# cgmb/euler

Hardware: AMD Instinct MI355X
Metric: cells*steps/sec of sim_step() (frames incl. the PCG pressure projection) + pressure-solve HBM GB/s vs roofline (higher is better)
Workload: dtype f64

## Files before the change

euler_amd/__init__.py:

```python
import ctypes as C
import os

import numpy as np

_HERE = os.path.dirname(os.path.abspath(__file__))
LIB_PATH = os.path.join(_HERE, "lib", "libeuler_hip.so")

DOT_AUTO, DOT_SEQUENTIAL, DOT_TREE = 0, 1, 2
PRECOND_IC0, PRECOND_JACOBI, PRECOND_IC0_TILE, PRECOND_IC0_TILE2, PRECOND_IC0_TILE_MG = 0, 1, 2, 3, 4
(OPT_P_STEPS, OPT_TILE_STORE_AS, OPT_TILE_REVERSE, OPT_RESIDENT_CAP, OPT_GRID4_MIN_CELLS, OPT_SLAB_FUSION, OPT_RCCL_SMALL, OPT_RCCL_NO_EXCHANGE, OPT_MARKERS_ROWMAJOR,
 OPT_SA_RUN, OPT_NO_INTERIOR, OPT_BUILD_GATHER, OPT_RESIDENT_FORCE_TIMEOUT, OPT_MG_SPLIT_LEVEL, OPT_MG_SPLIT_ACTIVE, OPT_MARKERS_TWO_PASS, OPT_BUILD_TWO_PASS,
 OPT_VELOCITY_TWO_PASS, OPT_NO_TILE_MAP, OPT_PROFILE_STRIDE) = range(1, 21)
SWEEP_AUTO, SWEEP_BAND, SWEEP_SIMPLE = 0, 1, 2
PCG_F64, PCG_F32 = 0, 1
RESIDENT_AUTO, RESIDENT_OFF = 0, 1
(F_U, F_V, F_UTMP, F_VTMP, F_SOLID, F_SOURCE, F_SINK, F_COUNT, F_PREV_COUNT, F_MARKERS, F_PRECON,
 F_PRESSURE, F_PCG_B, F_PCG_R, F_PCG_Z, F_PCG_S, F_PCG_Q, F_CELLMASK,
 F_DYE_R, F_DYE_G, F_DYE_B, F_DYE_RTMP, F_DYE_GTMP, F_DYE_BTMP, F_MARKER_KEYS) = range(25)
(STAGE_ADVECT_MARKERS, STAGE_REFRESH_COUNTS, STAGE_SOURCES, STAGE_EXTRAPOLATE, STAGE_ADVECT_VELOCITY,
 STAGE_PROJECT) = range(6)
(OP_BUILD_SYSTEM, OP_PRECON_FACTOR, OP_FORWARD_SOLVE, OP_BACKWARD_SOLVE, OP_APPLY_A, OP_DOT_ZR, OP_DOT_ZS,
 OP_INF_NORM_R, OP_UPDATE_PR, OP_UPDATE_SEARCH) = range(10)

_FIELD_DTYPE = {
    F_U: np.float32, F_V: np.float32, F_UTMP: np.float32, F_VTMP: np.float32,
    F_SOLID: np.uint8, F_SOURCE: np.uint8, F_SINK: np.uint8, F_COUNT: np.uint8, F_PREV_COUNT: np.uint8,
    F_MARKERS: np.float32, F_PRECON: np.float64, F_PRESSURE: np.float64, F_PCG_B: np.float64,
    F_PCG_R: np.float64, F_PCG_Z: np.float64, F_PCG_S: np.float64, F_PCG_Q: np.float64, F_CELLMASK: np.uint8,
    F_DYE_R: np.float32, F_DYE_G: np.float32, F_DYE_B: np.float32,
    F_DYE_RTMP: np.float32, F_DYE_GTMP: np.float32, F_DYE_BTMP: np.float32, F_MARKER_KEYS: np.uint32,
}


class EulerError(RuntimeError):
    def __init__(self, code, msg):
        super().__init__("libeuler_hip error %d: %s" % (code, msg))
        self.code = code


class Config(C.Structure):
    _fields_ = [
        ("abi_version", C.c_int32), ("X", C.c_int32), ("Y", C.c_int32), ("device", C.c_int32),
        ("max_iterations", C.c_int32), ("tol", C.c_double), ("dot_mode", C.c_int32), ("precond", C.c_int32),
        ("sweep_mode", C.c_int32), ("max_substeps", C.c_int32), ("frame_time", C.c_float),
        ("viscosity", C.c_float), ("pcg_poll_interval", C.c_int32), ("rainbow", C.c_int32),
        ("precond_tile_records", C.c_int32), ("slab_rank", C.c_int32), ("slab_nranks", C.c_int32),
        ("slab_band_lo", C.c_int32), ("slab_band_hi", C.c_int32), ("pcg_precision", C.c_int32), ("resident", C.c_int32),
    ]


class Stats(C.Structure):
    _fields_ = [
        ("frames", C.c_uint64), ("total_substeps", C.c_uint64), ("total_pcg_iterations", C.c_uint64),
        ("last_substeps", C.c_int32), ("last_pcg_iterations", C.c_int32), ("last_residual", C.c_double),
        ("last_dt", C.c_float), ("n_markers", C.c_uint64), ("source_exhausted", C.c_int32),
        ("rng_state", C.c_uint64), ("marker_dt_events", C.c_uint64), ("marker_multi_events", C.c_uint64),
        ("fluid_cells", C.c_uint64),
    ]


_lib = None

EXPORTS = [
    "euler_config_default", "euler_create", "euler_destroy", "euler_last_error", "euler_abi_version",
    "euler_load_scenario_mem", "euler_load_scenario_file", "euler_load_half_tank", "euler_load_half_tanks", "euler_parse_scenario",
    "euler_seed_markers", "euler_step", "euler_timestep", "euler_substep", "euler_stage", "euler_pcg_op", "euler_set_precond", "euler_set_solver",
    "euler_get_field", "euler_set_field", "euler_set_markers", "euler_set_rng", "euler_get_stats",
    "euler_field_bytes", "euler_render", "euler_render_grids", "euler_render_grids_rgb", "euler_colorize", "euler_profile_enable",
    "euler_profile_class_count", "euler_profile_class_name", "euler_profile_get", "euler_profile_reset",
    "euler_measure_copy_bandwidth", "euler_measure_exchange", "euler_device_name", "euler_hbm_bytes", "euler_sweep_timeline", "euler_save_state", "euler_load_state", "euler_set_comm", "euler_set_stream", "euler_slab_info",
    "euler_rccl_unique_id", "euler_rccl_version", "euler_set_comm_rccl", "euler_comm_calls",
    "euler_p2p_export", "euler_p2p_connect", "euler_p2p_disconnect", "euler_p2p_calls", "euler_resident_info",
    "euler_set_option", "euler_get_option",
]


def load_library():
    global _lib
    if _lib is not None:
        return _lib
    path = os.environ.get("EULER_HIP_LIB", LIB_PATH)
    if not os.path.exists(path):
        raise ImportError(
            "euler_amd: %s is missing. Build it with `python -c 'import __graft_entry__ as g; g.build()'` "
            "or `make -C euler_amd/csrc`. There is no CPU fallback." % LIB_PATH)
    L = C.CDLL(path)
    vp, i32, u64, f32, f64 = C.c_void_p, C.c_int32, C.c_uint64, C.c_float, C.c_double
    sig = {
        "euler_config_default": (C.c_int, [C.POINTER(Config)]),
        "euler_create": (C.c_int, [C.POINTER(Config), C.POINTER(vp)]),
        "euler_destroy": (None, [vp]),
        "euler_last_error": (C.c_char_p, []),
        "euler_abi_version": (C.c_int, []),
        "euler_load_scenario_mem": (C.c_int, [vp, C.c_char_p, i32, i32]),
        "euler_load_scenario_file": (C.c_int, [vp, C.c_char_p, i32]),
        "euler_load_half_tank": (C.c_int, [vp]),
        "euler_load_half_tanks": (C.c_int, [vp, i32]),
        "euler_parse_scenario": (C.c_int, [C.c_char_p, i32, i32, i32, i32, vp, vp, vp, vp]),
        "euler_seed_markers": (C.c_int, [vp, i32, i32, C.POINTER(u64), vp, C.POINTER(u64)]),
        "euler_step": (C.c_int, [vp]),
        "euler_timestep": (C.c_int, [vp, f32, C.POINTER(f32)]),
        "euler_substep": (C.c_int, [vp, f32]),
        "euler_stage": (C.c_int, [vp, i32, f32]),
        "euler_pcg_op": (C.c_int, [vp, i32, f32, f64, C.POINTER(f64)]),
        "euler_set_precond": (C.c_int, [vp, i32, i32]),
        "euler_set_solver": (C.c_int, [vp, i32, f64]),
        "euler_get_field": (C.c_int, [vp, i32, vp, C.c_size_t]),
        "euler_set_field": (C.c_int, [vp, i32, vp, C.c_size_t]),
        "euler_set_markers": (C.c_int, [vp, vp, u64]),
        "euler_set_rng": (C.c_int, [vp, u64, i32]),
        "euler_get_stats": (C.c_int, [vp, C.POINTER(Stats)]),
        "euler_field_bytes": (C.c_size_t, [vp, i32]),
        "euler_render": (C.c_int, [vp, i32, i32, C.c_char_p, i32, C.POINTER(i32)]),
        "euler_render_grids": (C.c_int, [vp, vp, vp, i32, i32, i32, i32, C.c_char_p, i32, C.POINTER(i32)]),
        "euler_render_grids_rgb": (C.c_int, [vp, vp, vp, vp, vp, vp, i32, i32, i32, i32, C.c_char_p, i32, C.POINTER(i32)]),
        "euler_colorize": (C.c_int, [vp]),
        "euler_profile_enable": (C.c_int, [vp, u64]),
        "euler_profile_class_count": (C.c_int, []),
        "euler_profile_class_name": (C.c_char_p, [i32]),
        "euler_profile_get": (C.c_int, [vp, i32, C.POINTER(f64), C.POINTER(u64)]),
        "euler_profile_reset": (C.c_int, [vp]),
        "euler_resident_info": (C.c_int, [vp, C.POINTER(u64)]),
        "euler_measure_copy_bandwidth": (C.c_int, [vp, C.c_size_t, i32, C.POINTER(f64)]),
        "euler_measure_exchange": (C.c_int, [vp, i32, i32, i32, C.POINTER(f64)]),
        "euler_device_name": (C.c_int, [vp, C.c_char_p, i32]),
        "euler_hbm_bytes": (u64, [vp]),
        "euler_sweep_timeline": (C.c_int, [vp, C.POINTER(C.c_uint64), i32]),
        "euler_save_state": (C.c_int, [vp, C.c_char_p]),
        "euler_load_state": (C.c_int, [vp, C.c_char_p]),
        "euler_set_comm": (C.c_int, [vp, vp, i32]),
        "euler_set_stream": (C.c_int, [vp, vp]),
        "euler_slab_info": (C.c_int, [vp, C.POINTER(i32), C.POINTER(i32), C.POINTER(i32)]),
        "euler_rccl_unique_id": (C.c_int, [vp, i32]),
        "euler_rccl_version": (C.c_int, []),
        "euler_set_comm_rccl": (C.c_int, [vp, vp, i32, i32, i32, i32]),
        "euler_comm_calls": (C.c_int, [vp, C.POINTER(u64)]),
        "euler_p2p_export": (C.c_int, [vp, vp, i32]),
        "euler_p2p_connect": (C.c_int, [vp, vp, i32]),
        "euler_p2p_disconnect": (C.c_int, [vp]),
        "euler_p2p_calls": (C.c_int, [vp, C.POINTER(u64)]),
        "euler_set_option": (C.c_int, [vp, i32, C.c_int64]),
        "euler_get_option": (C.c_int, [vp, i32, C.POINTER(C.c_int64)]),
    }
    for name, (res, args) in sig.items():
        fn = getattr(L, name)
        fn.restype = res
        fn.argtypes = args
    _lib = L
    return L


def _check(rc):
    if rc != 0:
        raise EulerError(rc, load_library().euler_last_error().decode(errors="replace"))


def parse_scenario(text, X, Y, upscale=False):
    if isinstance(text, str):
        text = text.encode()
    out = [np.zeros((Y, X), np.uint8) for _ in range(4)]
    _check(load_library().euler_parse_scenario(text, len(text), X, Y, int(upscale), *[a.ctypes.data for a in out]))
    return tuple(out)


def seed_markers(fluid, rng_state=0x9bd185c449534b91):
# ... 284 lines not shown
```

euler_amd/csrc/driver.hip:

```cpp
#include "euler_dev.h"
#include "k_mg.h"

#include <math.h>
#include <stdarg.h>
#include <stdlib.h>
#include <string.h>

#include <vector>

int eu_launch_build_system(euler_sim* S, float dt);
int eu_launch_velocity_update(euler_sim* S, float dt, int finish);
int eu_pressure_current(euler_sim* S);
int eu_unskew(euler_sim* S, const void* skew, void* rowmajor, int elem_bytes);
int eu_unskew_fluid(euler_sim* S, const double* skew, double* rowmajor);
double* eu_current_search_direction(euler_sim* S);
int eu_launch_tile_table(euler_sim* S);
int eu_skew(euler_sim* S, const void* rowmajor, void* skew, int elem_bytes);

static thread_local char g_err[512] = "";

void eu_set_error(const char* fmt, ...) {
  va_list ap;
  va_start(ap, fmt);
  vsnprintf(g_err, sizeof(g_err), fmt, ap);
// ... 69 lines not shown
  if (ms) *ms = S->prof_ms[cls];
  if (launches) *launches = S->prof_launches[cls];
  return rc;
}
extern "C" int euler_profile_reset(euler_sim* S) {
  if (!S) return EULER_EINVAL;
  int rc = eu_prof_flush(S);
  memset(S->prof_ms, 0, sizeof(S->prof_ms));
  memset(S->prof_launches, 0, sizeof(S->prof_launches));
  memset(S->prof_idle, 0, sizeof(S->prof_idle));
  return rc;
}

extern "C" int euler_config_default(euler_config* c) {
  if (!c) return EULER_EINVAL;
  memset(c, 0, sizeof(*c));
  c->abi_version = EULER_ABI_VERSION;
  c->X = 100; c->Y = 40;
  c->device = 0;
  c->max_iterations = 100;
  c->tol = (double)1e-6f;
  c->dot_mode = EULER_DOT_AUTO;
  c->precond = EULER_PRECOND_IC0;
  c->sweep_mode = EULER_SWEEP_AUTO;
  c->max_substeps = 8;
  c->frame_time = 0.1f;
  c->viscosity = 0.f;
  c->pcg_poll_interval = 8;
  return EULER_OK;
}

static int eu_set_tiles(euler_sim* S, int w) {
  if (w <= 0) w = 16;
  if (w != 8 && w != 16 && w != 32) { eu_set_error("precond_tile_records = %d: 8, 16 or 32 (0 = 16)", w); return EULER_EINVAL; }
  S->cfg.precond_tile_records = w;
  S->tile_w = w;
  return EULER_OK;
}

bool eu_resident_eligible(const euler_sim* S) {
  if (S->res_disabled || S->cfg.resident == EULER_RESIDENT_OFF) return false;
  if (S->cfg.precond != EULER_PRECOND_IC0_TILE || S->tile_w != 16 || S->cfg.sweep_mode == EULER_SWEEP_SIMPLE || S->cfg.dot_mode != EULER_DOT_TREE) return false;
  if (S->has_comm || S->slab_on || S->p2p_on) return false;
  const int cap = eu_resident_capacity(const_cast<euler_sim*>(S), S->cfg.pcg_precision == EULER_PCG_F32);
  if (S->cfg.pcg_precision == EULER_PCG_F32) return cap > 0 && S->geom.nbands * (S->geom.T / 16) <= 4 * cap;
  return cap > 0;
}
extern "C" int euler_resident_info(euler_sim* S, uint64_t out[3]) {
  if (!S || !out) return EULER_EINVAL;
  out[0] = eu_resident_eligible(S) ? 1 : 0; out[1] = S->res_solves; out[2] = S->res_fallbacks;
  return EULER_OK;
}

extern "C" int euler_set_option(euler_sim* S, int32_t key, int64_t value) {
  if (!S || key <= 0 || key >= EULER_OPT__COUNT) { eu_set_error("euler_set_option: unknown key %d", (int)key); return EULER_EINVAL; }
  bool ok = true;
  const char* when = nullptr;
  switch (key) {
    case EULER_OPT_P_STEPS: ok = value == 2 || value == 4 || value == 8; break;
    case EULER_OPT_SA_RUN: ok = value == 8 || value == 16 || value == 32;
      if (ok && value != 8 && (S->has_comm || eu_is_two_level(S))) when = "on a handle without a communicator, in the parity or the plain tile-local mode (the others run runs of 8)";
      break;
    case EULER_OPT_RCCL_SMALL: ok = value >= 0 && value <= 2; if (S->rccl) when = "before euler_set_comm_rccl"; break;
    case EULER_OPT_RCCL_NO_EXCHANGE: ok = value == 0 || value == 1; if (S->rccl) when = "before euler_set_comm_rccl"; break;
    case EULER_OPT_SLAB_FUSION: ok = value == 0 || value == 1; if (S->p2p_on) when = "before euler_p2p_connect"; break;
    case EULER_OPT_RESIDENT_CAP: case EULER_OPT_GRID4_MIN_CELLS: case EULER_OPT_RESIDENT_FORCE_TIMEOUT: ok = value >= 0; break;
    case EULER_OPT_MG_SPLIT_LEVEL: ok = value >= -1 && value < 12; break;
    case EULER_OPT_PROFILE_STRIDE: ok = value >= 1 && value <= 1024; break;
    case EULER_OPT_MG_SPLIT_ACTIVE: ok = false; break;
    default: ok = value == 0 || value == 1; break;
  }
  if (!ok) { eu_set_error("euler_set_option: key %d does not take the value %lld", (int)key, (long long)value); return EULER_EINVAL; }
  if (when) { eu_set_error("euler_set_option: key %d must be set %s", (int)key, when); return EULER_ESTATE; }
  HIPCHK(hipStreamSynchronize(S->stream));
  if (key == EULER_OPT_P_STEPS || key == EULER_OPT_SA_RUN) {
    int rcp = eu_pressure_current(S);
    if (rcp) return rcp;
  }
  S->opt[key] = value;
  if (key == EULER_OPT_P_STEPS || key == EULER_OPT_SA_RUN) S->s_ring_n = 0;
  if (key == EULER_OPT_MG_SPLIT_LEVEL) { eu_mg_split_release(S); S->opt[EULER_OPT_MG_SPLIT_ACTIVE] = 0; }
  return EULER_OK;
}
extern "C" int euler_get_option(euler_sim* S, int32_t key, int64_t* value) {
  if (!S || !value || key <= 0 || key >= EULER_OPT__COUNT) { eu_set_error("euler_get_option: unknown key %d", (int)key); return EULER_EINVAL; }
  *value = S->opt[key];
  return EULER_OK;
}

static const char* eu_precond_combination(const euler_sim* S, int precond, int tile_w, int has_comm, int slab_on, int p2p_on) {
  const bool coarse = precond == EULER_PRECOND_IC0_TILE2 || precond == EULER_PRECOND_IC0_TILE_MG;
  if (!coarse) return nullptr;
  if (tile_w != 16 || S->cfg.sweep_mode == EULER_SWEEP_SIMPLE) return "the coarse-correction preconditioners run on tiles of 16 records with the band schedule";
  if (precond == EULER_PRECOND_IC0_TILE2 && (has_comm || slab_on)) return "EULER_PRECOND_IC0_TILE2 runs on one GPU (row slabs: EULER_PRECOND_IC0_TILE_MG)";
  if (precond == EULER_PRECOND_IC0_TILE_MG && has_comm && (!slab_on || p2p_on)) return "EULER_PRECOND_IC0_TILE_MG with several ranks: row-slab handles without mailboxes only";
  return nullptr;
}

extern "C" int euler_set_precond(euler_sim* S, int32_t precond, int32_t tile_records) {
  if (!S || precond < EULER_PRECOND_IC0 || precond > EULER_PRECOND_IC0_TILE_MG) { eu_set_error("euler_set_precond: bad argument"); return EULER_EINVAL; }
  const int w = tile_records <= 0 ? 16 : tile_records;
  if (w != 8 && w != 16 && w != 32) { eu_set_error("precond_tile_records = %d: 8, 16 or 32 (0 = 16)", tile_records); return EULER_EINVAL; }
  if (const char* why = eu_precond_combination(S, precond, w, S->has_comm, S->slab_on, S->p2p_on)) { eu_set_error("euler_set_precond: %s", why); return EULER_EINVAL; }
  if (S->cfg.pcg_precision == EULER_PCG_F32 && (precond != EULER_PRECOND_IC0_TILE || w != 16)) { eu_set_error("euler_set_precond: an EULER_PCG_F32 handle runs EULER_PRECOND_IC0_TILE with tiles of 16 records only"); return EULER_EINVAL; }
  HIPCHK(hipStreamSynchronize(S->stream));
  const bool coarse = precond == EULER_PRECOND_IC0_TILE2 || precond == EULER_PRECOND_IC0_TILE_MG;
  if (coarse) { int rc = eu_coarse_alloc(S, precond == EULER_PRECOND_IC0_TILE_MG); if (rc) return rc; }
  (void)eu_set_tiles(S, w);
  S->cfg.dot_mode = coarse ? EULER_DOT_TREE : S->dot_mode_user;
  if (S->has_comm && S->cfg.dot_mode == EULER_DOT_SEQUENTIAL) S->cfg.dot_mode = EULER_DOT_TREE;
  S->cfg.precond = precond;
  S->lean_ok = 0;
  return EULER_OK;
}

extern "C" int euler_set_solver(euler_sim* S, int32_t max_iterations, double tol) {
  if (!S) return EULER_EINVAL;
  HIPCHK(hipStreamSynchronize(S->stream));
  if (max_iterations > 0) S->cfg.max_iterations = max_iterations;
  if (tol >= 0.0) S->cfg.tol = tol;
  return EULER_OK;
}

static thread_local size_t g_alloc_bytes = 0;
template <typename T>
static int dalloc(T** p, size_t n) {
  HIPCHK(hipMalloc((void**)p, n * sizeof(T)));
  g_alloc_bytes += n * sizeof(T);
  HIPCHK(hipMemset(*p, 0, n * sizeof(T)));
  return EULER_OK;
}
#define DALLOC(p, n) do { int _rc = dalloc(&(p), (n)); if (_rc) { euler_destroy(S); return _rc; } } while (0)

extern "C" void euler_destroy(euler_sim* S) {
  if (!S) return;
  if (S->stream) (void)hipStreamSynchronize(S->stream);
  eu_p2p_release(S);
  eu_rccl_release(S);
  eu_slab_release(S);
  eu_coarse_release(S);
  const size_t wo = S->shifted ? S->win_off : 0;
  for (float* f : {S->u, S->v, S->utmp, S->vtmp}) if (f) (void)hipFree(f + wo);
  for (uint8_t* g : {S->solid, S->source, S->sink, S->count, S->prev_count}) if (g) (void)hipFree(g + wo);
  if (S->count32) (void)hipFree(S->count32);
  if (S->blockedT) (void)hipFree(S->blockedT);
  if (S->tmap) (void)hipFree(S->tmap);
  if (S->uT) (void)hipFree(S->uT);
  if (S->vT) (void)hipFree(S->vT);
  if (S->countT) (void)hipFree(S->countT);
  if (S->solidT) (void)hipFree(S->solidT);
  if (S->sys_m) (void)hipFree(S->sys_m);
  if (S->sys_div) (void)hipFree(S->sys_div);
  void* dev[] = {S->markers[0], S->markers[1], S->keys[0], S->keys[1], S->ms, S->evmask, S->delmask, S->ev_theta, S->ev_delta, S->sel_idx, S->act_idx,
                 S->act_dt, S->cellmask64, S->draws, S->sel.block_sums, S->sc, S->partial, S->red_counter, S->granules, S->ticket, S->sweep_timeline, S->halo_buf, S->band_ranges, S->partial2, S->pair_buf, S->xrows, S->alpha_buf, S->rng_jump, S->chunk_flag, S->chunk_prev, S->chunk_part, S->tile_table, S->chunk_bits, S->chunk_list,
                 S->rowmajor_tmp};
  for (void* p : dev) if (p) (void)hipFree(p);
  for (float* d : S->dye) if (d) (void)hipFree(d + wo);
  const size_t so = S->shifted ? S->skew_off : 0, sl = S->shifted ? (size_t)EU_SKEW_SLACK : 0;
  (void)so; (void)sl;
  for (void* d : S->s_ring_alloc) if (d) (void)hipFree(d);
  for (void* d : S->skew_alloc) if (d) (void)hipFree(d);
  const size_t fb_off = S->shifted ? (size_t)S->ab_lo * S->fb_stride * 64 : 0;
  if (S->fbits_fwd) (void)hipFree(S->fbits_fwd + fb_off);
  if (S->fbits_bwd) (void)hipFree(S->fbits_bwd + fb_off);
  if (S->ms_host) (void)hipHostFree(S->ms_host);
  if (S->sc_host) (void)hipHostFree(S->sc_host);
  if (S->poll_host) (void)hipHostFree(S->poll_host);
  if (S->res_err) (void)hipHostFree(S->res_err);
  if (S->res_gran) (void)hipFree(S->res_gran);
  for (hipEvent_t e : S->poll_event) if (e) (void)hipEventDestroy(e);
  if (S->ev_pool) { for (int k = 0; k < S->ev_cap; ++k) if (S->ev_pool[k]) (void)hipEventDestroy(S->ev_pool[k]); free(S->ev_pool); }
  free(S->ev_cls); free(S->ev_solve); free(S->ev_iter);
  if (S->stream && S->own_stream) (void)hipStreamDestroy(S->stream);
  free(S);
}

extern "C" int euler_create(const euler_config* cfg, euler_sim** out) {
  if (!cfg || !out) { eu_set_error("euler_create: null argument"); return EULER_EINVAL; }
  if (cfg->abi_version != EULER_ABI_VERSION) { eu_set_error("euler_create: ABI version %d != %d", cfg->abi_version, EULER_ABI_VERSION); return EULER_EINVAL; }
  if (cfg->X < 8 || cfg->Y < 8 || (size_t)cfg->X * cfg->Y > (size_t)1 << 30) { eu_set_error("euler_create: grid %dx%d out of range", cfg->X, cfg->Y); return EULER_EINVAL; }
  int ndev = 0;
  hipError_t e = hipGetDeviceCount(&ndev);
  if (e != hipSuccess || ndev == 0) {
    eu_set_error("euler_create: no HIP device (%s); libeuler_hip has no CPU path", e == hipSuccess ? "device count 0" : hipGetErrorString(e));
    return EULER_EHIP;
  }
  if (cfg->device < 0 || cfg->device >= ndev) { eu_set_error("euler_create: device %d of %d", cfg->device, ndev); return EULER_EINVAL; }
  HIPCHK(hipSetDevice(cfg->device));
  hipDeviceProp_t prop;
  HIPCHK(hipGetDeviceProperties(&prop, cfg->device));
  if (strncmp(prop.gcnArchName, "gfx950", 6) != 0) {
    eu_set_error("euler_create: device is %s; this library carries gfx950 code only", prop.gcnArchName);
    return EULER_EHIP;
  }

  euler_sim* S = (euler_sim*)calloc(1, sizeof(euler_sim));
  if (S) { S->opt[EULER_OPT_P_STEPS] = 8; S->opt[EULER_OPT_TILE_REVERSE] = 1; S->opt[EULER_OPT_GRID4_MIN_CELLS] = 1ll << 22; S->opt[EULER_OPT_SA_RUN] = 8; S->opt[EULER_OPT_PROFILE_STRIDE] = 1; }
  if (!S) return EULER_ENOMEM;
  g_alloc_bytes = 0;
  S->cfg = *cfg;
  if (S->cfg.max_iterations <= 0) S->cfg.max_iterations = 100;
  if (S->cfg.max_substeps <= 0) S->cfg.max_substeps = 8;
  if (S->cfg.frame_time <= 0.f) S->cfg.frame_time = 0.1f;
  S->X = cfg->X; S->Y = cfg->Y;
  const size_t C = S->C = (size_t)cfg->X * cfg->Y;
  if (S->cfg.dot_mode == EULER_DOT_AUTO) S->cfg.dot_mode = C <= 65536 ? EULER_DOT_SEQUENTIAL : EULER_DOT_TREE;
  S->dot_mode_user = S->cfg.dot_mode;
  if (S->cfg.sweep_mode == EULER_SWEEP_AUTO) S->cfg.sweep_mode = EULER_SWEEP_BAND;
  S->geom.X = S->X; S->geom.Y = S->Y;
  S->geom.nbands = (S->Y + 63) / 64;
  S->geom.T = (S->X + 63 + 95) / 96 * 96;
  S->geom.TS = (S->geom.T + 31) / 32 * 32 + 64;
  S->geom.S = (size_t)S->geom.nbands * S->geom.TS * 64;
  const int nbands = S->geom.nbands;
  S->slab_on = cfg->slab_nranks >= 1;
  if (S->slab_on) {
    if (cfg->slab_rank < 0 || cfg->slab_rank >= cfg->slab_nranks || cfg->slab_nranks > nbands) {
      eu_set_error("euler_create: slab rank %d of %d for %d bands of 64 rows", cfg->slab_rank, cfg->slab_nranks, nbands);
      free(S); return EULER_EINVAL;
    }
    if (S->cfg.sweep_mode == EULER_SWEEP_SIMPLE) {
      eu_set_error("euler_create: row slabs do not run EULER_SWEEP_SIMPLE");
      free(S); return EULER_EINVAL;
    }
    S->band_lo = (int)((int64_t)nbands * cfg->slab_rank / cfg->slab_nranks);
    S->band_hi = (int)((int64_t)nbands * (cfg->slab_rank + 1) / cfg->slab_nranks);
    if (cfg->slab_band_hi > cfg->slab_band_lo || cfg->slab_band_lo != 0) {
      const int lo = cfg->slab_band_lo, hi = cfg->slab_band_hi;
      const bool first = cfg->slab_rank == 0, last = cfg->slab_rank + 1 == cfg->slab_nranks;
      if (lo < 0 || hi <= lo || hi > nbands || (first && lo != 0) || (last && hi != nbands) || (!first && lo < cfg->slab_rank) ||
          (!last && nbands - hi < cfg->slab_nranks - 1 - cfg->slab_rank)) {
        eu_set_error("euler_create: slab rank %d of %d cannot own bands [%d, %d) of %d (every rank needs a band; the ranges tile the grid in rank order)",
                     cfg->slab_rank, cfg->slab_nranks, lo, hi, nbands);
        free(S); return EULER_EINVAL;
      }
      S->band_lo = lo; S->band_hi = hi;
    }
    if (S->cfg.dot_mode == EULER_DOT_SEQUENTIAL) S->cfg.dot_mode = EULER_DOT_TREE;
  } else { S->band_lo = 0; S->band_hi = nbands; }
  S->row_lo = 64 * S->band_lo; S->row_hi = 64 * S->band_hi < S->Y ? 64 * S->band_hi : S->Y;
  S->win_lo = S->row_lo - EU_GHOST_LO > 0 ? S->row_lo - EU_GHOST_LO : 0;
  S->win_hi = S->row_hi + EU_GHOST_HI < S->Y ? S->row_hi + EU_GHOST_HI : S->Y;
  S->win_off = (size_t)S->win_lo * S->X;
  S->Cw = (size_t)(S->win_hi - S->win_lo) * S->X;
  S->ab_lo = S->band_lo > 0 ? S->band_lo - 1 : 0; S->ab_hi = S->band_hi < nbands ? S->band_hi + 1 : nbands;
  S->skew_off = (size_t)S->ab_lo * S->geom.TS * 64;
  S->Sw = (size_t)(S->ab_hi - S->ab_lo) * S->geom.TS * 64;
  S->e_lo = (size_t)S->band_lo * S->geom.TS * 64; S->e_cnt = (size_t)(S->band_hi - S->band_lo) * S->geom.TS * 64;
  const size_t SS = S->Sw;
  const size_t Cw = S->Cw;
  if (C > ((size_t)1 << 29) || Cw > ((size_t)1 << 28) || (SS + EU_SKEW_SLACK) * 8 >= ((size_t)1 << 32)) {
    eu_set_error("grid %d x %d is larger than the supported maximum (2^28 cells per GPU, 2^29 in all)", cfg->X, cfg->Y);
    free(S);
    return EULER_EINVAL;
  }
#define CREATECHK(call) do { hipError_t _e = (call); if (_e != hipSuccess) { int _rc = eu_hip_fail(_e, #call, __FILE__, __LINE__); euler_destroy(S); return _rc; } } while (0)
  CREATECHK(hipStreamCreateWithFlags(&S->stream, hipStreamNonBlocking));
  S->own_stream = 1;

  DALLOC(S->u, Cw); DALLOC(S->v, Cw); DALLOC(S->utmp, Cw); DALLOC(S->vtmp, Cw);
  DALLOC(S->solid, Cw); DALLOC(S->source, Cw); DALLOC(S->sink, Cw); DALLOC(S->count, Cw); DALLOC(S->prev_count, Cw);
  DALLOC(S->count32, Cw);
  if (!S->slab_on) { DALLOC(S->blockedT, Cw); DALLOC(S->uT, Cw); DALLOC(S->vT, Cw); DALLOC(S->countT, Cw); DALLOC(S->solidT, Cw); }
  eu_state_replaced(S);
  DALLOC(S->sys_m, Cw); DALLOC(S->sys_div, Cw);
  if (S->cfg.rainbow) for (float*& d : S->dye) DALLOC(d, Cw);
  S->max_markers = 4 * C;
  if (S->slab_on) { const size_t cap = 6 * (size_t)(S->row_hi - S->row_lo) * S->X + 65536; if (cap < S->max_markers) S->max_markers = cap; }
  DALLOC(S->markers[0], S->max_markers); DALLOC(S->markers[1], S->max_markers);
  if (S->slab_on) { DALLOC(S->keys[0], S->max_markers); DALLOC(S->keys[1], S->max_markers); }
  DALLOC(S->ms, 1);
  const size_t mwords = (S->max_markers + 63) / 64;
  DALLOC(S->evmask, mwords);
  if (!S->slab_on) DALLOC(S->delmask, mwords);
  if (!S->slab_on) {
    S->tmap_nx = (S->X + 63) / 64 + 1; S->tmap_n = S->tmap_nx * ((S->Y + 63) / 64 + 2);
    DALLOC(S->tmap, 3 * (size_t)S->tmap_n);
  }
  DALLOC(S->ev_theta, S->max_markers); DALLOC(S->ev_delta, S->max_markers);
  S->sel_cap = S->max_markers;
  DALLOC(S->sel_idx, S->sel_cap);
  DALLOC(S->act_idx, S->max_markers); DALLOC(S->act_dt, S->max_markers);
  DALLOC(S->cellmask64, (Cw + 63) / 64 + 1);
  S->sel.capacity_blocks = (mwords + 2047) / 2048 + 1;
  DALLOC(S->sel.block_sums, S->sel.capacity_blocks);
  {
    const size_t stagger = (size_t)EU_ARRAY_STAGGER / 8 * 8;
    int k = 0;
    for (double** d : {&S->b, &S->p, &S->r, &S->z, &S->s, &S->s2, &S->q, &S->precon}) {
      DALLOC(*d, SS + EU_SKEW_SLACK + 8 * stagger / 8);
      S->skew_alloc[k] = *d;
      *d += (size_t)k * stagger / 8;
      ++k;
    }
    DALLOC(S->cellmask, SS + EU_SKEW_SLACK);
    S->skew_alloc[8] = S->cellmask;
  }
  S->fb_stride = 12 * (((S->geom.T + 7) / 8 + 11) / 12) + 4;
  DALLOC(S->fbits_fwd, (size_t)(S->ab_hi - S->ab_lo) * S->fb_stride * 64);
  DALLOC(S->fbits_bwd, (size_t)(S->ab_hi - S->ab_lo) * S->fb_stride * 64);
  DALLOC(S->sc, 1);
  DALLOC(S->band_ranges, (size_t)S->geom.nbands);
  { int rc = eu_set_tiles(S, S->cfg.precond_tile_records); if (rc) { euler_destroy(S); return rc; } }
  S->red_blocks = (int)eu_blocks(S->e_cnt, EU_RED_ELEMS, 2048);
  DALLOC(S->partial, (size_t)S->red_blocks > 2048 ? (size_t)S->red_blocks : 2048);
  DALLOC(S->partial2, 2048);
  DALLOC(S->pair_buf, 2 * 64);
// ... 704 lines not shown
```

euler_amd/csrc/euler_dev.h:

```cpp
#pragma once

#include <hip/hip_runtime.h>
#include <stdint.h>
#include <stdio.h>

#include "euler.h"
#include "euler_host.h"

#define EU_H 1.0f
#define EU_RHO 1.0f
#define EU_G (-10.0f)

#define CM_FLUID 0x01
#define CM_RIGHT 0x02
#define CM_UP    0x04
#define CM_LEFT  0x08
#define CM_DOWN  0x10
#define CM_DIAG_SHIFT 5
#define CM_INTERIOR 0x9F
#define EU_CHUNK_INTERIOR 0x80000000u

enum {
  KC_TIMESTEP = 0, KC_MARKER_ADVECT, KC_MARKER_EVENTS, KC_MARKER_BIN, KC_MARKER_COMPACT, KC_SOURCES,
  KC_SELECT, KC_EXTRAPOLATE, KC_ADVECT_VELOCITY, KC_BUILD_SYSTEM, KC_PRECON_FACTOR,
  KC_FORWARD_SOLVE, KC_BACKWARD_SOLVE, KC_APPLY_A, KC_DOT, KC_UPDATE_PR, KC_UPDATE_SEARCH,
  KC_REDUCE_FINAL, KC_VELOCITY_UPDATE, KC_JACOBI, KC_MISC, KC_PRECOND_TILE, KC_COARSE_CYCLE, KC_RESIDENT, KC__COUNT
};

struct PcgScalars {
  double sigma, zs, sigma_new, alpha, beta, rnorm;
  double tol;
  double comm_val;
  double comm_val2;
  double* comm_slot;
  double alpha_prev;
  double alpha_hist[8];
  int nonzero;
  int done;
  int iters;
  int max_iters;
  unsigned int n_chunks, pad_;
  void** p2p_boxes;
  int* p2p_error;
  int p2p_rank, p2p_n;
  unsigned int p2p_seq, p2p_halo_seq;
};

struct MarkerState {
  unsigned long long n;
  unsigned long long max_markers;
  unsigned long long rng_state;
  int exhausted;
  unsigned int n_events;
  unsigned int n_actual;
  unsigned int n_deleted;
  unsigned int n_append;
  unsigned long long n0_append;
  unsigned long long total_dt_events, multi_events;
  float dt_final;
  float dt;
  unsigned int max_u2_bits, max_v2_bits;
  unsigned int dt_ticket;
  int error;
  unsigned long long n_loc;
  unsigned int n_rm;
  unsigned int n_del_glob;
  unsigned int n_recv;
  unsigned int src_k_lo;
  unsigned long long rng0;
};

#define EU_SKEW_SLACK (64 * 64)
#ifndef EU_ARRAY_STAGGER
#define EU_ARRAY_STAGGER 0
#endif
#ifndef EU_RED_ELEMS
#define EU_RED_ELEMS (256 * 16)
#endif
struct SkewGeom {
  int X, Y, nbands, T, TS;
  size_t S;
};
static inline __host__ __device__ size_t skew_index(const SkewGeom& g, int x, int y) {
  const int l = y & 63, t = x + l;
  return ((size_t)(y >> 6) * g.TS + (size_t)(t & ~1)) * 64 + 2 * l + (t & 1);
}
static inline __host__ __device__ void skew_decode(const SkewGeom& g, size_t e, int& band, int& t, int& l) {
  const size_t per_band = (size_t)g.TS * 64;
  band = (int)(e / per_band);
  const size_t r = e % per_band;
  l = (int)((r & 127) >> 1);
  t = (int)((r >> 7) << 1) + (int)(r & 1);
}

struct SelectScratch {
  unsigned int* block_sums;
  unsigned int* total;
  size_t capacity_blocks;
};

struct euler_sim {
  euler_config cfg;
  int X, Y;
  size_t C;
  hipStream_t stream;
  int loaded;
  long long opt[32];
  int dot_mode_user;

  float *u, *v, *utmp, *vtmp;
  uint8_t *solid, *source, *sink, *count, *prev_count;
  unsigned int* count32;
  int p_pending;
  int maxsq_state;
  int uv_clean;
  int uv_zb;
  int count32_dirty;
  int prebin_valid;
  unsigned long long* delmask;
  uint8_t* tmap;
  int tmap_nx, tmap_n;
  int tmap_valid;
  int utmp_clean;
  int countT_clean;
  uint8_t* blockedT;
  int blocked_dirty;
  float *uT, *vT; uint8_t *countT, *solidT;
  int solidT_dirty;
  float* dye[6];
  float2* markers[2];
  int cur;
  size_t max_markers;
  unsigned long long n_markers_host;
  size_t n_source_cells;
  MarkerState* ms;
  MarkerState* ms_host;
  unsigned long long* evmask;
  float* ev_theta;
  float* ev_delta;
  unsigned int* sel_idx;
  size_t sel_cap;
  unsigned int* act_idx; float* act_dt;
  unsigned long long* cellmask64;
  float* draws;
  SelectScratch sel;

  SkewGeom geom;
  double *b, *p, *r, *z, *s, *q, *precon;
  double* s2;
  void* skew_alloc[9];
  uint8_t* cellmask;
  uint8_t* sys_m; float* sys_div;
  unsigned int* fbits_fwd; unsigned int* fbits_bwd;
  int fb_stride;
  int4* band_ranges;
  int coarse_m, coarse_shift, coarse_nx, coarse_ny, coarse_n;
  int *cc_diag, *cc_right, *cc_up;
  int* cc_pinned;
  double* cc_sten;
  int cc_n;
  double* cc_fac;
  double* cc_inv;
  double* cc_part;
  double* cc_y;
  double* cc_null;
  int mg_levels, mg_nx[12], mg_ny[12];
  size_t mg_off[12], mg_cells;
  double* mg_a;
  unsigned long long* mg_a0i;
  double *mg_rhs, *mg_x;
  double* mg_wd;
  uint8_t* mg_inner0; double mg_ic[9];
  double* mg_part;
  double* mg_dot;
  double* mg_null0;
  double* mg_m0;
  void* mg_split;
  double* mg_xbuf; int mg_xslot;
  unsigned long long* res_gran;
  unsigned long long res_tag;
  int* res_err;
  int res_disabled;
  unsigned int res_last_chunks;
  int res_have_last, res_skip_once;
  unsigned long long res_solves, res_fallbacks;
  int pcg_fields_resident;
  int tile_w;
  double* s_ring[8];
  void* s_ring_alloc[8];
  double* s_base[2];
  int s_ring_n;
  int s_launched;
  int s_none;
  int s_stale;
  const double* tile_as_override;
  double* partial2;
  struct RngJump* rng_jump;
  uint8_t* chunk_flag;
  uint8_t* chunk_prev;
  uint8_t* chunk_part;
  size_t hbm_bytes;
  int lean_ok;
  double* tile_table;
  unsigned long long* chunk_bits;
  unsigned int* chunk_list;
  size_t chunk_words, chunk_cap;
  double* xrows;
  size_t xrow_len;
  int gs_cur;
  double* alpha_buf;
  double* pair_buf;
  double* rowmajor_tmp;
  PcgScalars* sc;
  PcgScalars* sc_host;
  PcgScalars* poll_host;
  hipEvent_t poll_event[2];
  double* partial;
  unsigned int* red_counter;
  int red_blocks;
  unsigned long long* granules;
  int gran_stride;
  unsigned int* ticket;
  unsigned int ticket_base;
  unsigned int epoch;
  unsigned long long* sweep_timeline;

  float interp_lim[4];

  euler_stats stats;

  euler_comm_ops comm;
  int has_comm, couple;
  int band_lo, band_hi;
  size_t e_lo, e_cnt;
  double* halo_buf;
  int own_stream;
  int slab_on, shifted;
  int row_lo, row_hi, win_lo, win_hi;
  size_t win_off, Cw, skew_off, Sw;
  int ab_lo, ab_hi;
  unsigned int* keys[2];
  euler_comm_ops bulk;
  struct SlabScratch* slab;
  int part_lo[64], part_hi[64];
  void* rccl;
  void* p2p;
  int p2p_on;

  uint64_t prof_mask;
  uint64_t prof_open;
  unsigned int prof_seq[32];
  double prof_ms[KC__COUNT];
  uint64_t prof_launches[KC__COUNT];
  uint64_t prof_idle[KC__COUNT];
  hipEvent_t* ev_pool; int* ev_cls; int* ev_solve; int* ev_iter; int ev_used, ev_cap;
  int solve_seq;
  int prof_iter;
  int solve_iters[256];
};

void eu_set_error(const char* fmt, ...);
int eu_hip_fail(hipError_t e, const char* what, const char* file, int line);
#define HIPCHK(call) do { hipError_t _e = (call); if (_e != hipSuccess) return eu_hip_fail(_e, #call, __FILE__, __LINE__); } while (0)

void eu_prof_begin(euler_sim* S, int cls);
void eu_prof_end(euler_sim* S, int cls);
int  eu_prof_flush(euler_sim* S);

#define LAUNCH(S, CLS, KERNEL, GRID, BLOCK, ...)                                   \
  do {                                                                             \
    eu_prof_begin((S), (CLS));                                                     \
    hipLaunchKernelGGL(KERNEL, GRID, BLOCK, 0, (S)->stream, __VA_ARGS__);          \
    eu_prof_end((S), (CLS));                                                       \
  } while (0)

static inline unsigned eu_blocks(size_t n, unsigned per_block, unsigned cap = 0x7fffffffu) {
  size_t b = (n + per_block - 1) / per_block;
  if (b < 1) b = 1;
  if (b > cap) b = cap;
  return (unsigned)b;
}

__device__ __forceinline__ size_t eu_xcd_block() {
  const unsigned int b = blockIdx.x, full = gridDim.x & ~7u;
  return b < full ? (size_t)(b & 7) * (full >> 3) + (b >> 3) : (size_t)b;
}

#define EU_GHOST_LO 1
#define EU_GHOST_HI 2
int  eu_slab_alloc(euler_sim* S);
size_t eu_slab_bytes(const euler_sim* S);
void eu_slab_release(euler_sim* S);
int  eu_slab_substep(euler_sim* S, float dt);
int  eu_slab_stage(euler_sim* S, int stage, float dt);
int  eu_slab_timestep(euler_sim* S, float frame_time_left);
int  eu_slab_after_load(euler_sim* S);
int  eu_slab_check_partition(euler_sim* S);
int  eu_slab_exchange_uv(euler_sim* S);
int  eu_slab_exchange_dye(euler_sim* S);
int  eu_slab_render(euler_sim* S, int wx, int wy, char* out, int cap, int* len);
int  eu_slab_after_restore(euler_sim* S);
int  eu_slab_error_sync(euler_sim* S);
int  eu_slab_same_everywhere(euler_sim* S, const double* vals, int n, int* same);
int  eu_slab_status_sync(euler_sim* S, int local_rc, int* worst);
static inline void eu_state_replaced(euler_sim* S) {
  S->blocked_dirty = 1; S->solidT_dirty = 1;
  S->prebin_valid = 0;
  if (S->maxsq_state == 2) S->maxsq_state = 1;
  S->p_pending = 0;
  S->uv_clean = 0; S->uv_zb = 0;
  S->tmap_valid = 0; S->utmp_clean = 0; S->countT_clean = 0;
}
static inline bool eu_tile_map_on(const euler_sim* S) { return S->tmap && S->tmap_valid && !S->slab_on && S->opt[EULER_OPT_NO_TILE_MAP] == 0; }
int eu_launch_timestep(euler_sim* S, float frame_time_left);
int eu_launch_advect_markers(euler_sim* S, float dt);
int eu_launch_refresh_counts(euler_sim* S);
int eu_launch_sources(euler_sim* S);
int eu_launch_extrapolate(euler_sim* S);
int eu_launch_advect_velocity(euler_sim* S, float dt);
int eu_launch_diffuse(euler_sim* S, float dt);
int eu_launch_project(euler_sim* S, float dt);
int eu_resident_capacity(euler_sim* S, int f32);
int eu_launch_resident(euler_sim* S, unsigned int n_chunks);
bool eu_resident_eligible(const euler_sim* S);
int eu_launch_colorize(euler_sim* S);
int eu_launch_dye_extrapolate(euler_sim* S);
int eu_launch_dye_sources(euler_sim* S);
int eu_launch_dye_advect(euler_sim* S, float dt);
int eu_launch_pcg_op(euler_sim* S, int op, float dt, double a, double* out);
int eu_ordered_select(euler_sim* S, const unsigned long long* mask, size_t nwords, unsigned int* out_idx,
                      unsigned int* out_total);
int eu_sync_marker_state(euler_sim* S);
void eu_rccl_release(euler_sim* S);
void eu_p2p_release(euler_sim* S);
int eu_p2p_halo_skewed(euler_sim* S, double* s_skewed);
void eu_p2p_xgran(euler_sim* S, int backward, const unsigned long long** in, unsigned long long** out);
int  eu_p2p_has_neighbour_arrays(const euler_sim* S);
void eu_p2p_neighbour_arrays(euler_sim* S, const double** z_dn, const double** s_dn, const double** z_up, const double** s_up);
int eu_install_comm(euler_sim* S, const euler_comm_ops* ops, int32_t coupling, int allow_single);
static inline bool eu_is_tile(const euler_sim* S) { return S->cfg.precond == EULER_PRECOND_IC0_TILE || S->cfg.precond == EULER_PRECOND_IC0_TILE2 || S->cfg.precond == EULER_PRECOND_IC0_TILE_MG; }
static inline bool eu_is_two_level(const euler_sim* S) { return S->cfg.precond == EULER_PRECOND_IC0_TILE2 || S->cfg.precond == EULER_PRECOND_IC0_TILE_MG; }
static inline bool eu_is_mg(const euler_sim* S) { return S->cfg.precond == EULER_PRECOND_IC0_TILE_MG; }
int  eu_coarse_alloc(euler_sim* S, bool mg);
void eu_coarse_release(euler_sim* S);
int  eu_launch_coarse_setup(euler_sim* S);
int  eu_launch_coarse_consistent(euler_sim* S);
int  eu_launch_coarse_solve(euler_sim* S, int fin_op, int force);
int  eu_launch_coarse_search_init(euler_sim* S);
int  eu_coarse_comm_slots(euler_sim* S);
int  eu_launch_coarse_pre(euler_sim* S, int force);
int  eu_launch_coarse_scatter(euler_sim* S);
int  eu_launch_coarse_add_row(euler_sim* S, double* row, int yrow);

#ifdef __HIPCC__

// ... 186 lines not shown
```

euler_amd/csrc/k_pcg.hip:

```cpp
#include "euler_dev.h"
#include "k_mg.h"

#include <stdlib.h>
#include <cmath>
#include <type_traits>
#include <vector>

#define RED_THREADS 1024
typedef double sw_d2 __attribute__((ext_vector_type(2)));

__device__ __forceinline__ bool pcg_idle(const PcgScalars* sc) { return sc->done || !sc->nonzero; }

#define DPP_WAVE_SHL1 0x130
#define DPP_WAVE_SHR1 0x138

template <int CTRL>
__device__ __forceinline__ double wave_shift_inject(double v, double edge) {
  const int lo = __builtin_amdgcn_update_dpp(__double2loint(edge), __double2loint(v), CTRL, 0xf, 0xf, false);
  const int hi = __builtin_amdgcn_update_dpp(__double2hiint(edge), __double2hiint(v), CTRL, 0xf, 0xf, false);
  return __hiloint2double(hi, lo);
}

enum { FIN_SIGMA_INIT = 0, FIN_ALPHA, FIN_RNORM, FIN_BETA, FIN_STORE_ONLY, FIN_TO_COMM };
#define FIN_VIA_P2P 0x100
// ... 80 lines not shown
  return l == 0 ? ((edges & 1) && band == 0) : ((edges & 2) && band == nb_local - 1);
}

template <bool EDGES>
__global__ __launch_bounds__(RED_THREADS) void k_dot_partial(const double* __restrict__ a, const double* __restrict__ b,
                                                             const uint8_t* __restrict__ mask, size_t S,
                                                             double* __restrict__ partial, PcgScalars* sc, int force,
                                                             unsigned int* counter, int fin_op, int TS, int nb_local, int edges) {
  if (!force && pcg_idle(sc)) return;
  const size_t chunk = (((S + gridDim.x - 1) / gridDim.x) + 1) & ~(size_t)1;
  const size_t lo = (size_t)blockIdx.x * chunk, hi = lo + chunk < S ? lo + chunk : S;
  double t = 0.0;
  for (size_t i = lo + 2 * (size_t)threadIdx.x; i < hi; i += 2 * RED_THREADS) {
    const unsigned int mm = *reinterpret_cast<const unsigned short*>(mask + i);
    if (!((mm | (mm >> 8)) & CM_FLUID)) continue;
    const sw_d2 av = *reinterpret_cast<const sw_d2*>(a + i), bv = *reinterpret_cast<const sw_d2*>(b + i);
    if (mm & CM_FLUID) t += av.x * bv.x;
    if ((mm >> 8) & CM_FLUID) t += av.y * bv.y;
    if (EDGES && slab_edge_row(i, (int)((i & 127) >> 1), TS, nb_local, edges)) {
      if (mm & CM_FLUID) st_system(a + i, av.x);
      if ((mm >> 8) & CM_FLUID) st_system(a + i + 1, av.y);
    }
  }
  if (EDGES) asm volatile("s_waitcnt vmcnt(0)" ::: "memory");
  t = block_sum(t);
  block_finish<false>(t, partial, counter, sc, fin_op);
}

#define SEQ_TILE 4096
__global__ __launch_bounds__(256) void k_dot_sequential(const double* __restrict__ a, const double* __restrict__ b,
                                                        const uint8_t* __restrict__ mask, SkewGeom g, PcgScalars* sc,
                                                        int op, int force) {
  if (!force && pcg_idle(sc)) return;
  __shared__ double prod[2][SEQ_TILE];
  __shared__ unsigned long long any[2][SEQ_TILE / 64];
  const size_t C = (size_t)g.X * g.Y;
  const int ntiles = (int)((C + SEQ_TILE - 1) / SEQ_TILE);
  const int wave = threadIdx.x >> 6, lane = threadIdx.x & 63;
  double total = 0.0;
  for (int tile = -1; tile < ntiles; ++tile) {
    if (wave > 0 && tile + 1 < ntiles) {
      const int buf = (tile + 1) & 1;
      const size_t base = (size_t)(tile + 1) * SEQ_TILE;
      for (int grp = wave - 1; grp < SEQ_TILE / 64; grp += 3) {
        const size_t c = base + (size_t)grp * 64 + lane;
        bool f = false;
        double pr = 0.0;
        if (c < C) {
          const size_t i = skew_index(g, (int)(c % g.X), (int)(c / g.X));
          f = (mask[i] & CM_FLUID) != 0;
          if (f) pr = a[i] * b[i];
        }
        prod[buf][grp * 64 + lane] = pr;
        const unsigned long long bal = __ballot(f);
        if (lane == 0) any[buf][grp] = bal;
      }
    }
    if (threadIdx.x == 0 && tile >= 0) {
      const int buf = tile & 1;
      for (int grp = 0; grp < SEQ_TILE / 64; ++grp) {
        if (any[buf][grp] == 0ull) continue;
        const double* pp = &prod[buf][grp * 64];
        double v[64];
#pragma unroll
        for (int k = 0; k < 64; ++k) v[k] = pp[k];
#pragma unroll
        for (int k = 0; k < 64; ++k) total += v[k];
      }
    }
    __syncthreads();
  }
  if (threadIdx.x == 0) pcg_scalar_step(sc, op, total);
}

__global__ __launch_bounds__(RED_THREADS) void k_apply_a(const double* __restrict__ s, double* __restrict__ z,
                                                         const uint8_t* __restrict__ mask, SkewGeom g,
                                                         double* __restrict__ partial, PcgScalars* sc, int force,
                                                         unsigned int* counter, int fin_op) {
  if (!force && pcg_idle(sc)) return;
  const size_t S = g.S;
  const size_t chunk = (((S + gridDim.x - 1) / gridDim.x) + 127) & ~(size_t)127;
  const size_t lo = (size_t)blockIdx.x * chunk, hi = lo + chunk < S ? lo + chunk : S;
  double t = 0.0;
  for (size_t i = lo + 2 * (size_t)threadIdx.x; i < hi; i += 2 * RED_THREADS) {
    const unsigned int mm = *reinterpret_cast<const unsigned short*>(mask + i);
    const unsigned int m0 = mm & 0xff, m1 = mm >> 8;
    if (!((m0 | m1) & CM_FLUID)) continue;
    const sw_d2 c = *reinterpret_cast<const sw_d2*>(s + i);
    const int l = (int)((i & 127) >> 1);
    sw_d2 o = {0.0, 0.0};
    if (m0 & CM_FLUID) {
      double v = (double)(int)(m0 >> CM_DIAG_SHIFT) * c.x;
      v = v - ((m0 & CM_RIGHT) ? c.y : 0.0);
      if (m0 & CM_UP) {
        size_t up = i + 3;
        if (l == 63) { int band, tt, ll; skew_decode(g, i, band, tt, ll); up = skew_index(g, tt - 63, 64 * (band + 1)); }
        v = v - s[up];
      } else {
        v = v - 0.0;
      }
      v = v - ((m0 & CM_LEFT) ? s[i - 127] : 0.0);
      if (m0 & CM_DOWN) {
        size_t dn = i - 129;
        if (l == 0) { int band, tt, ll; skew_decode(g, i, band, tt, ll); dn = skew_index(g, tt, 64 * band - 1); }
        v = v - s[dn];
      } else {
        v = v - 0.0;
      }
      o.x = v;
      t += v * c.x;
    }
    if (m1 & CM_FLUID) {
      double v = (double)(int)(m1 >> CM_DIAG_SHIFT) * c.y;
      v = v - ((m1 & CM_RIGHT) ? s[i + 128] : 0.0);
      if (m1 & CM_UP) {
        size_t up = i + 130;
        if (l == 63) { int band, tt, ll; skew_decode(g, i + 1, band, tt, ll); up = skew_index(g, tt - 63, 64 * (band + 1)); }
        v = v - s[up];
      } else {
        v = v - 0.0;
      }
      v = v - ((m1 & CM_LEFT) ? c.x : 0.0);
      if (m1 & CM_DOWN) {
        size_t dn = i - 2;
        if (l == 0) { int band, tt, ll; skew_decode(g, i + 1, band, tt, ll); dn = skew_index(g, tt, 64 * band - 1); }
        v = v - s[dn];
      } else {
        v = v - 0.0;
      }
      o.y = v;
      t += v * c.y;
    }
    if ((m0 & m1) & CM_FLUID) *reinterpret_cast<sw_d2*>(z + i) = o;
    else if (m0 & CM_FLUID) z[i] = o.x;
    else z[i + 1] = o.y;
  }
  t = block_sum(t);
  if (fin_op >= 0) block_finish<false>(t, partial, counter, sc, fin_op);
}

struct SlabNeighbours {
  const double *z_dn, *s_dn, *z_up, *s_up;
  int nb_local;
  const double *zrow_dn, *srow_dn, *zrow_up, *srow_up;
  double *snew_dn, *snew_up;
};
__device__ __forceinline__ double ld_system(const double* p) {
  double v;
  asm volatile("global_load_dwordx2 %0, %1, off sc0 sc1\n\ts_waitcnt vmcnt(0)" : "=v"(v) : "v"(p) : "memory");
  return v;
}

#define SA_THREADS 256
struct SaPair { sw_d2 z, so; double ez0, es0, ez1, es1; };

__device__ __forceinline__ double pick3(int t, int tb1, int tb2, double v0, double v1, double v2) {
  double v = v0;
  v = t >= tb1 ? v1 : v;
  v = t >= tb2 ? v2 : v;
  return v;
}
struct CoarseRef { const double* y; int shift, nx, ny, band0; };
__device__ __forceinline__ double pick4(int q, double v0, double v1, double v2, double v3) {
  double v = v0;
  v = q >= 1 ? v1 : v;
  v = q >= 2 ? v2 : v;
  v = q >= 3 ? v3 : v;
  return v;
}
struct SaHist { const double* s[6]; };
template <int SLAB, int PMODE, int SA_RUN, int COARSE = 0, bool STORE = true>
__global__ __launch_bounds__(SA_THREADS, (COARSE == 2 && PMODE == 1 && SLAB == 0) ? 4 : 1) void k_search_apply(const double* __restrict__ s_old, const double* __restrict__ z,
                                                             double* __restrict__ s_new, double* __restrict__ out,
                                                             const uint8_t* __restrict__ mask, SkewGeom g,
                                                             double* __restrict__ partial, PcgScalars* sc, int force,
                                                             unsigned int* counter, int fin_op, SlabNeighbours nbr,
                                                             double* __restrict__ p, double* s_new_base, double* s_old_base,
                                                             const unsigned int* __restrict__ chunk_list,
                                                             CoarseRef cref, SaHist hist) {
  __shared__ double s_cy[COARSE == 2 ? SA_THREADS / 64 : 1][COARSE == 2 ? MG_NI + 1 : 1][64];
  __shared__ double s_ce[COARSE == 2 ? SA_THREADS / 64 : 1][COARSE == 2 ? MG_NI + 1 : 1][64];
  if (!force && pcg_idle(sc)) return;
  const double beta = sc->beta;
  (void)s_new_base; (void)s_old_base;
  constexpr int NPA = PMODE >= 2 ? PMODE : 2;
  double al[NPA] = {};
  if (PMODE >= 2) {
    const int k = sc->iters;
#pragma unroll
    for (int j = 0; j < NPA; ++j) al[j] = sc->alpha_hist[(k - NPA + j) & 7];
  }
  const int lane = threadIdx.x & 63;
  const int TS = g.TS, npairs = TS / 2;
  const int nb_local = (int)(g.S / ((size_t)TS * 64));
  const int cpb = (npairs + SA_RUN - 1) / SA_RUN, total = nb_local * cpb;
  const int n_waves = gridDim.x * (SA_THREADS / 64);
  const bool edge_lane = lane == 0 || lane == 63;
  double t = 0.0;
  const bool listed = chunk_list != nullptr;
  const int ntb16 = g.T / 16;
  const int todo = listed ? (int)sc->n_chunks : total;
  typedef std::integral_constant<bool, true> yes_t;
  typedef std::integral_constant<bool, false> no_t;
  for (int i = blockIdx.x * (SA_THREADS / 64) + (threadIdx.x >> 6); i < todo; i += n_waves) {
    int c = i, per = cpb;
    bool interior = false;
    if (listed) { const unsigned int ent = chunk_list[i]; interior = (ent & EU_CHUNK_INTERIOR) != 0; c = (int)(ent & ~EU_CHUNK_INTERIOR); per = ntb16; }
    const int lb = c / per, P0 = (c % per) * SA_RUN, P1 = P0 + SA_RUN < npairs ? P0 + SA_RUN : npairs;
    const size_t bbase = (size_t)lb * TS * 64 + 2 * lane;
    auto run = [&](auto full_tag) {
      constexpr bool FULL = decltype(full_tag)::value;
      unsigned int mm[SA_RUN];
      unsigned int any = 0;
#pragma unroll
      for (int j = 0; j < SA_RUN; ++j) {
        if (FULL) mm[j] = CM_INTERIOR | (CM_INTERIOR << 8);
        else mm[j] = P0 + j < P1 ? (unsigned int)*reinterpret_cast<const unsigned short*>(mask + bbase + (size_t)(P0 + j) * 128) : 0u;
        any |= mm[j];
      }
      if (!FULL && !listed && !__ballot(((any | (any >> 8)) & CM_FLUID) != 0)) return;
      const bool up_remote = SLAB == 1 && nbr.z_up && lb + 1 == nb_local, dn_remote = SLAB == 1 && nbr.z_dn && lb == 0;
      const double* ez = lane == 0 ? (dn_remote ? nbr.z_dn : z) : (up_remote ? nbr.z_up : z);
      const double* es = lane == 0 ? (dn_remote ? nbr.s_dn : s_old) : (up_remote ? nbr.s_up : s_old);
      const bool remote = lane == 0 ? dn_remote : up_remote;
      const long long e0_base = lane == 0 ? ((long long)(lb - 1) * TS + 62) * 64 + 127 : ((long long)(lb + 1) * TS - 64) * 64 + 1;
      const long long e1_base = lane == 0 ? ((long long)(lb - 1) * TS + 64) * 64 + 126 : ((long long)(lb + 1) * TS - 62) * 64;
      const unsigned int vbit = lane == 0 ? CM_DOWN : CM_UP;
      const bool ghost = SLAB == 2 && (lane == 0 ? (nbr.zrow_dn != nullptr && lb == 0) : (nbr.zrow_up != nullptr && lb + 1 == nb_local));
      const double* gz = lane == 0 ? nbr.zrow_dn : nbr.zrow_up;
      const double* gs = lane == 0 ? nbr.srow_dn : nbr.srow_up;
      double* gsn = lane == 0 ? nbr.snew_dn : nbr.snew_up;
      const int gcol = lane == 0 ? 0 : -63;
      double cy0 = 0.0, cy1 = 0.0, cy2 = 0.0, ce0 = 0.0, ce1 = 0.0, ce2 = 0.0;
      double (*cyv)[64] = s_cy[COARSE == 2 ? threadIdx.x >> 6 : 0];
      double (*cev)[64] = s_ce[COARSE == 2 ? threadIdx.x >> 6 : 0];
      int ctb1 = 0x7fffffff, ctb2 = 0x7fffffff, cJb = 0;
      (void)cJb;
      if (COARSE == 2) {
        cJb = (2 * (P0 - 1) - lane - MG_G0 / 2) >> MG_LOG;
        ctb1 = MG_G0 * (cJb + 1) + lane + MG_G0 / 2;
        const int row = (cref.band0 + lb) * 64 + lane;
        const int hi_ = cref.nx - 1;
        int i0, i1;
        double fy;
        mg_cell_w(row, cref.ny, i0, i1, fy);
        const double* y0 = cref.y + (size_t)i0 * cref.nx;
        const double* y1 = cref.y + (size_t)i1 * cref.nx;
#pragma unroll
        for (int q = 0; q <= MG_NI; ++q) { const int c = cJb + q < 0 ? 0 : (cJb + q < hi_ ? cJb + q : hi_); cyv[q][lane] = mg_rows(y0[c], y1[c], fy); }
#pragma unroll
        for (int q = 0; q <= MG_NI; ++q) cev[q][lane] = 0.0;
        if (edge_lane) {
          const int re = row + (lane == 0 ? -1 : 1);
          if (re >= 0 && re < MG_G0 * cref.ny) {
            mg_cell_w(re, cref.ny, i0, i1, fy);
            y0 = cref.y + (size_t)i0 * cref.nx; y1 = cref.y + (size_t)i1 * cref.nx;
#pragma unroll
            for (int q = 0; q <= MG_NI; ++q) { const int c = cJb + q < 0 ? 0 : (cJb + q < hi_ ? cJb + q : hi_); cev[q][lane] = mg_rows(y0[c], y1[c], fy); }
          }
        }
      }
      auto p0y = [&](int t, double (*av)[64]) __attribute__((always_inline)) {
        const double f = (double)((t - lane - MG_G0 / 2) & (MG_G0 - 1)) * (1.0 / MG_G0);
        int m = t >= ctb1 ? ((t - ctb1) >> MG_LOG) + 1 : 0;
        m = m < MG_NI - 1 ? m : MG_NI - 1;
        return mg_lerp_x(av[m][lane], av[m + 1][lane], f);
      };
      if (COARSE == 1) {
        const int xa = 2 * (P0 - 1) - lane, Ja = (xa > 0 ? xa : 0) >> cref.shift;
        const int row = (cref.band0 + lb) * 64 + lane;
        const size_t I = (size_t)(row >> cref.shift) * cref.nx;
        ctb1 = ((Ja + 1) << cref.shift) + lane;
        ctb2 = ((Ja + 2) << cref.shift) + lane;
        cy0 = Ja < cref.nx ? cref.y[I + Ja] : 0.0;
        cy1 = Ja + 1 < cref.nx ? cref.y[I + Ja + 1] : 0.0;
        cy2 = Ja + 2 < cref.nx ? cref.y[I + Ja + 2] : 0.0;
        if (edge_lane) {
          const int re = row + (lane == 0 ? -1 : 1);
          const bool inside = re >= 0 && (re >> cref.shift) < cref.ny;
          const size_t Ie = (size_t)((inside ? re : row) >> cref.shift) * cref.nx;
          ce0 = (inside && Ja < cref.nx) ? cref.y[Ie + Ja] : 0.0;
          ce1 = (inside && Ja + 1 < cref.nx) ? cref.y[Ie + Ja + 1] : 0.0;
          ce2 = (inside && Ja + 2 < cref.nx) ? cref.y[Ie + Ja + 2] : 0.0;
        }
      }
      auto load_pair = [&](int P, SaPair& d, unsigned int m) __attribute__((always_inline)) {
        d.ez0 = d.es0 = d.ez1 = d.es1 = 0.0;
        if (P < 0 || P >= npairs) { d.z = sw_d2{0.0, 0.0}; d.so = sw_d2{0.0, 0.0}; return; }
        d.z = *reinterpret_cast<const sw_d2*>(z + bbase + (size_t)P * 128);
        d.so = *reinterpret_cast<const sw_d2*>(s_old + bbase + (size_t)P * 128);
        if (edge_lane) {
          if ((m & CM_FLUID) && (m & vbit)) {
            const long long k = e0_base + (long long)P * 128;
            if (SLAB == 2 && ghost) { d.ez0 = gz[2 * P + gcol]; d.es0 = gs[2 * P + gcol]; }
            else if (SLAB == 1 && remote) { d.ez0 = ld_system(ez + k); d.es0 = ld_system(es + k); } else { d.ez0 = ez[k]; d.es0 = es[k]; }
          }
          if (((m >> 8) & CM_FLUID) && ((m >> 8) & vbit)) {
            const long long k = e1_base + (long long)P * 128;
            if (SLAB == 2 && ghost) { d.ez1 = gz[2 * P + 1 + gcol]; d.es1 = gs[2 * P + 1 + gcol]; }
            else if (SLAB == 1 && remote) { d.ez1 = ld_system(ez + k); d.es1 = ld_system(es + k); } else { d.ez1 = ez[k]; d.es1 = es[k]; }
          }
          if (COARSE == 1) {
            d.ez0 = d.ez0 + pick3(2 * P, ctb1, ctb2, ce0, ce1, ce2);
            d.ez1 = d.ez1 + pick3(2 * P + 1, ctb1, ctb2, ce0, ce1, ce2);
          }
          if (COARSE == 2) {
            d.ez0 = d.ez0 + p0y(2 * P, cev);
            d.ez1 = d.ez1 + p0y(2 * P + 1, cev);
          }
        }
        if (COARSE == 1) {
          d.z.x = d.z.x + pick3(2 * P, ctb1, ctb2, cy0, cy1, cy2);
          d.z.y = d.z.y + pick3(2 * P + 1, ctb1, ctb2, cy0, cy1, cy2);
        }
        if (COARSE == 2) {
          d.z.x = d.z.x + p0y(2 * P, cyv);
          d.z.y = d.z.y + p0y(2 * P + 1, cyv);
        }
      };
      auto sprime = [&](const SaPair& d) __attribute__((always_inline)) { return sw_d2{d.z.x + beta * d.so.x, d.z.y + beta * d.so.y}; };
      SaPair A, B, Cn;
      load_pair(P0 - 1, A, 0u);
      load_pair(P0, B, mm[0]);
      load_pair(P0 + 1, Cn, SA_RUN > 1 ? mm[1] : 0u);
      double prev_y = sprime(A).y;
      sw_d2 cur = sprime(B);
#pragma unroll
      for (int j = 0; j < SA_RUN; ++j) {
        const int P = P0 + j;
        if (P < P1) {
          SaPair D;
          load_pair(P + 2 <= P1 ? P + 2 : -1, D, j + 2 < SA_RUN ? mm[j + 2] : 0u);
          const unsigned int m0 = mm[j] & 0xff, m1 = mm[j] >> 8;
          const sw_d2 nxt = sprime(Cn);
          const double e0 = B.ez0 + beta * B.es0, e1 = B.ez1 + beta * B.es1;
          if (SLAB == 2 && ghost && edge_lane) {
            if ((mm[j] & CM_FLUID) && (mm[j] & vbit)) gsn[2 * P + gcol] = e0;
            if (((mm[j] >> 8) & CM_FLUID) && ((mm[j] >> 8) & vbit)) gsn[2 * P + 1 + gcol] = e1;
          }
          const double dn0 = wave_shift_inject<DPP_WAVE_SHR1>(prev_y, e0), up0 = wave_shift_inject<DPP_WAVE_SHL1>(cur.y, e0);
          const double dn1 = wave_shift_inject<DPP_WAVE_SHR1>(cur.x, e1), up1 = wave_shift_inject<DPP_WAVE_SHL1>(nxt.x, e1);
          if ((m0 | m1) & CM_FLUID) {
            const size_t i = bbase + (size_t)P * 128;
            sw_d2 cc = B.so, o = {0.0, 0.0};
            if (PMODE >= 2) {
              sw_d2 pv = *reinterpret_cast<const sw_d2*>(p + i);
              constexpr int NP = PMODE >= 2 ? PMODE : 2;
              sw_d2 sv[NP];
              sv[0] = *reinterpret_cast<const sw_d2*>(s_new + i);
#pragma unroll
              for (int j = 1; j < NP - 1; ++j) sv[j] = *reinterpret_cast<const sw_d2*>(hist.s[j - 1] + i);
              sv[NP - 1] = B.so;
#pragma unroll
              for (int j = 0; j < NP; ++j) {
                if (m0 & CM_FLUID) pv.x = pv.x + sv[j].x * al[j];
                if (m1 & CM_FLUID) pv.y = pv.y + sv[j].y * al[j];
              }
              *reinterpret_cast<sw_d2*>(p + i) = pv;
            }
            if (m0 & CM_FLUID) cc.x = cur.x;
            if (m1 & CM_FLUID) cc.y = cur.y;
            if (m0 & CM_FLUID) {
              double v = (double)(int)(m0 >> CM_DIAG_SHIFT) * cc.x;
              v = v - ((m0 & CM_RIGHT) ? cc.y : 0.0);
              v = v - ((m0 & CM_UP) ? up0 : 0.0);
              v = v - ((m0 & CM_LEFT) ? prev_y : 0.0);
              v = v - ((m0 & CM_DOWN) ? dn0 : 0.0);
              o.x = v;
              t += v * cc.x;
            }
            if (m1 & CM_FLUID) {
              double v = (double)(int)(m1 >> CM_DIAG_SHIFT) * cc.y;
              v = v - ((m1 & CM_RIGHT) ? nxt.x : 0.0);
              v = v - ((m1 & CM_UP) ? up1 : 0.0);
              v = v - ((m1 & CM_LEFT) ? cc.x : 0.0);
              v = v - ((m1 & CM_DOWN) ? dn1 : 0.0);
              o.y = v;
              t += v * cc.y;
            }
            if ((m0 & m1) & CM_FLUID) *reinterpret_cast<sw_d2*>(s_new + i) = cc;
            else if (m0 & CM_FLUID) s_new[i] = cc.x;
            else s_new[i + 1] = cc.y;
            if (STORE) {
              if ((m0 & m1) & CM_FLUID) *reinterpret_cast<sw_d2*>(out + i) = o;
              else if (m0 & CM_FLUID) out[i] = o.x;
              else out[i + 1] = o.y;
            }
            if (SLAB == 1 && slab_edge_row(i, lane, TS, nb_local, (nbr.z_dn ? 1 : 0) | (nbr.z_up ? 2 : 0))) {
              if (m0 & CM_FLUID) st_system(s_new + i, cc.x);
              if (m1 & CM_FLUID) st_system(s_new + i + 1, cc.y);
            }
          }
          prev_y = cur.y; cur = nxt;
          B = Cn; Cn = D;
        }
      }
    };
    if (SA_RUN == 8 && interior) run(yes_t()); else run(no_t());
  }
  if (SLAB == 1) asm volatile("s_waitcnt vmcnt(0)" ::: "memory");
  t = block_sum<SA_THREADS>(t);
  if (fin_op >= 0) block_finish<false, SA_THREADS>(t, partial, counter, sc, fin_op);
}

__global__ __launch_bounds__(RED_THREADS) void k_update_pr(double* __restrict__ p, double* __restrict__ r,
                                                           const double* __restrict__ s, const double* __restrict__ z,
                                                           const uint8_t* __restrict__ mask, size_t S,
                                                           double* __restrict__ partial, PcgScalars* sc, int force,
                                                           double alpha_arg, unsigned int* counter, int fin_op) {
  if (!force && pcg_idle(sc)) return;
  const double alpha = force ? alpha_arg : sc->alpha;
  const double nalpha = -alpha;
  const size_t chunk = (((S + gridDim.x - 1) / gridDim.x) + 1) & ~(size_t)1;
  const size_t lo = (size_t)blockIdx.x * chunk, hi = lo + chunk < S ? lo + chunk : S;
  double mx = 0.0;
  for (size_t i = lo + 2 * (size_t)threadIdx.x; i < hi; i += 2 * RED_THREADS) {
    const unsigned int mm = *reinterpret_cast<const unsigned short*>(mask + i);
    const bool f0 = (mm & CM_FLUID) != 0, f1 = ((mm >> 8) & CM_FLUID) != 0;
    if (!(f0 | f1)) continue;
    const sw_d2 sv = *reinterpret_cast<const sw_d2*>(s + i), zv = *reinterpret_cast<const sw_d2*>(z + i);
    sw_d2 pv = *reinterpret_cast<const sw_d2*>(p + i), rv = *reinterpret_cast<const sw_d2*>(r + i);
    if (f0) { pv.x = pv.x + sv.x * alpha; rv.x = rv.x + zv.x * nalpha; const double a = fabs(rv.x); if (a > mx) mx = a; }
    if (f1) { pv.y = pv.y + sv.y * alpha; rv.y = rv.y + zv.y * nalpha; const double a = fabs(rv.y); if (a > mx) mx = a; }
    *reinterpret_cast<sw_d2*>(p + i) = pv;
    *reinterpret_cast<sw_d2*>(r + i) = rv;
  }
  mx = block_max(mx);
  if (fin_op >= 0) block_finish<true>(mx, partial, counter, sc, fin_op);
}

__global__ __launch_bounds__(RED_THREADS) void k_inf_norm(const double* __restrict__ r, const uint8_t* __restrict__ mask,
                                                          size_t S, double* __restrict__ partial) {
  const size_t chunk = (S + gridDim.x - 1) / gridDim.x;
  const size_t lo = (size_t)blockIdx.x * chunk, hi = lo + chunk < S ? lo + chunk : S;
  double mx = 0.0;
  for (size_t i = lo + threadIdx.x; i < hi; i += RED_THREADS)
    if (mask[i] & CM_FLUID) { const double a = fabs(r[i]); if (a > mx) mx = a; }
  mx = block_max(mx);
  if (threadIdx.x == 0) partial[blockIdx.x] = mx;
}

template <bool COPY>
__global__ __launch_bounds__(256) void k_update_search(double* __restrict__ s, const double* __restrict__ z,
                                                       const uint8_t* __restrict__ mask, size_t S, const PcgScalars* sc,
                                                       int force, double beta_arg) {
  if (!force && pcg_idle(sc)) return;
  const double beta = force ? beta_arg : sc->beta;
  for (size_t i = 2 * ((size_t)blockIdx.x * blockDim.x + threadIdx.x); i < S; i += 2 * (size_t)gridDim.x * blockDim.x) {
    const sw_d2 zv = *reinterpret_cast<const sw_d2*>(z + i);
    if (COPY) { *reinterpret_cast<sw_d2*>(s + i) = zv; continue; }
    const unsigned int mm = *reinterpret_cast<const unsigned short*>(mask + i);
    const bool f0 = (mm & CM_FLUID) != 0, f1 = ((mm >> 8) & CM_FLUID) != 0;
// ... 340 lines not shown
  };

  auto await = [&](const unsigned int* cnt, int target) {
    ++stalls;
    for (unsigned int spins = 0; (int)lds_get(cnt) < target;) {
      if (lds_get(&sh.abort)) break;
      if (++spins > SW_SPIN_LIMIT) { if (lane == 0) atomicExch(a.error, 2); lds_put(&sh.abort, 1u); break; }
      __builtin_amdgcn_s_sleep(1);
    }
    SW_COMPILER_FENCE();
  };

  unsigned long long t_first = 0;
  double qq = 0.0;
  auto sweep = [&](auto hp_c, auto pb_c) {
    constexpr bool HP = decltype(hp_c)::value;
    constexpr bool PB = decltype(pb_c)::value;
    fetch_block(opA);
    if (DIST >= 2) fetch_block(opB);
    if (DIST >= 3) fetch_block(opC);
    double own = CONST;
    qq = 0.0;
    double out = CONST;
    double beA[SW_BLK], beB[SW_BLK];
    auto read_boundary = [&](int rel, double (&be)[SW_BLK]) {
      const double* slot = sh.bnd[rel & (SW_BND_RING - 1)];
#pragma unroll
      for (int j = 0; j < SW_BLK; ++j) be[j] = HP ? slot[j] : CONST;
    };
    if (PB) sh.pub[(SW_BLK * B0 - 1) & (SW_RING - 1)][lane] = CONST;
    if (HP) await(&sh.dep_done, 1);
    read_boundary(0, beA);
    t_first = wall_clock64();

    auto run_block = [&](int blk, Operands& cur, Operands& nxt, double (&be)[SW_BLK], double (&be_next)[SW_BLK]) {
      const int rel = blk - B0;
      fetch_block(nxt);
      unsigned long long prog = 0;
      if (HP || PB) prog = __hip_atomic_load(reinterpret_cast<const unsigned long long*>(&sh.dep_done), __ATOMIC_RELAXED, __HIP_MEMORY_SCOPE_WORKGROUP);
      __builtin_amdgcn_sched_barrier(0);
      double* ring = &sh.pub[(SW_BLK * blk) & (SW_RING - 1)][lane];
      double prev_carry = CONST, prev_res = 0.0;
      auto step = [&](auto jc) {
        constexpr int j = decltype(jc)::value;
        constexpr int P = j >> 1;
        constexpr bool ODD = ((j & 1) != 0) != BWD;
        if constexpr (OP != SW_FACTOR && (j & 1) == 0) {
          constexpr int N0 = (3 - P) * LOADS_PER_PAIR + DIST * LOADS + P, N = N0 < 63 ? N0 : 63;
          asm volatile("s_waitcnt vmcnt(%3)" : "+v"(cur.in[P]), "+v"(cur.pre[P]), "+v"(cur.fb) : "n"(N) : "memory");
        }
        const double nbv = wave_shift_inject<CTRL>(out, be[j]);
        const double cin = ODD ? cur.in[P].y : cur.in[P].x, cpre = ODD ? cur.pre[P].y : cur.pre[P].x;
        const int cm = OP == SW_FACTOR ? ((cur.m[P] >> (ODD ? 8 : 0)) & 0xff) : ((int)(cur.fb << (31 - j)) >> 31);
        double res, carry;
        if (OP == SW_FACTOR) {
          const double aa = (double)(cm >> CM_DIAG_SHIFT);
          const double cl = -1.0 * own, cb = -1.0 * nbv;
          double e = aa - cl * cl - cb * cb;
          if (e < 0.25 * aa) e = (aa != 0.0) ? aa : 1.0;
          res = (cm & CM_FLUID) ? 1.0 / sqrt(e) : cpre;
          carry = res;
        } else if (OP == SW_FORWARD) {
          const double t = cin - own - nbv;
          const double qv = t * cpre;
          res = __hiloint2double(__double2hiint(qv) & cm, __double2loint(qv) & cm);
          carry = -1.0 * cpre * res;
          qq = __builtin_fma(res, res, qq);
        } else {
          const int fr = (int)(cur.fb << (23 - j)) >> 31, fu = (int)(cur.fb << (15 - j)) >> 31;
          const double kr = __hiloint2double((int)0xBFF00000 & fr, 0) * cpre, ku = __hiloint2double((int)0xBFF00000 & fu, 0) * cpre;
          const double t = cin - kr * own - ku * nbv;
          const double zv = t * cpre;
          res = __hiloint2double(__double2hiint(zv) & cm, __double2loint(zv) & cm);
          carry = res;
        }
        if (j & 1) *reinterpret_cast<sw_d2*>(p_out + P * PSTEP) = BWD ? sw_d2{res, prev_res} : sw_d2{prev_res, res};
        prev_res = res;
        own = carry;
        out = carry;
        if (PB && (j & 1)) { ring[(j - 1) * 64] = prev_carry; ring[j * 64] = carry; }
        prev_carry = carry;
      };
      step(std::integral_constant<int, 0>()); step(std::integral_constant<int, 1>()); step(std::integral_constant<int, 2>());
      step(std::integral_constant<int, 3>());
      step(std::integral_constant<int, 4>()); step(std::integral_constant<int, 5>());
      if (HP) {
        if (__builtin_expect(rel + 1 < NBLK && (int)(unsigned int)prog < rel + 2, 0)) await(&sh.dep_done, rel + 2);
        read_boundary(rel + 1, be_next);
        if (SW_TRACE_HANDOFF && blk + 1 == SW_TRACE_CB && lane == 0) a.timeline[(size_t)ord * 8 + 7] = wall_clock64();
      }
      step(std::integral_constant<int, 6>()); step(std::integral_constant<int, 7>());
      __builtin_amdgcn_sched_barrier(0);
      p_out += 4 * PSTEP;
      if (HP || PB) { SW_COMPILER_FENCE(); lds_put(&sh.comp_done, (unsigned int)(rel + 1)); }
      if (SW_TRACE_HANDOFF && blk == SW_TRACE_CB + 8 && lane == 0) a.timeline[(size_t)ord * 8 + 4] = wall_clock64();
      if (PB && __builtin_expect(rel + 1 < NBLK && (int)(unsigned int)(prog >> 32) < rel - 5, 0)) await(&sh.pub_done, rel - 5);
    };

    for (int blk = B0; blk < B1; blk += 4) {
      if (DIST == 3) {
        run_block(blk, opA, opD, beA, beB);
        run_block(blk + 1, opB, opA, beB, beA);
        run_block(blk + 2, opC, opB, beA, beB);
        run_block(blk + 3, opD, opC, beB, beA);
      } else {
        run_block(blk, opA, opB, beA, beB);
        run_block(blk + 1, opB, opA, beB, beA);
        run_block(blk + 2, opA, opB, beA, beB);
        run_block(blk + 3, opB, opA, beB, beA);
      }
    }
    asm volatile("s_waitcnt vmcnt(0)" ::: "memory");
  };
  typedef std::integral_constant<bool, true> yes_t;
  typedef std::integral_constant<bool, false> no_t;
  if (has_prev) { if (publish) sweep(yes_t(), yes_t()); else sweep(yes_t(), no_t()); }
  else          { if (publish) sweep(no_t(), yes_t()); else sweep(no_t(), no_t()); }
  if (OP == SW_FORWARD && a.fin_qq >= 0) sweep_qq_arrive(a, ord, qq);
  if (lane == 0) {
    unsigned long long* tl = a.timeline + (size_t)ord * 8;
    tl[0] = t_entry; tl[1] = t_first; tl[2] = wall_clock64(); tl[3] = ((unsigned long long)(B1 - B0) << 32) | stalls;
  }
}


#define PT_THREADS 256
struct TileArgs {
  SkewGeom g;
  const uint8_t* mask;
  double* pre;
  double* r;
  const double* as;
  double* z;
  int band_lo, nb_local;
  int rupd;
  int sweeps;
  int fin_dot;
  int via;
  double* part_max; double* part_dot;
  unsigned int* counter;
  const unsigned int* list;
  const double* table;
  PcgScalars* sc;
  int force;
  double alpha_arg;
  double* pair_slot;
  double *zsend_lo, *zsend_hi;
  int edge_lo, edge_hi;
  int reverse;
  double* cpart;
  int cshift;
  int cmode, cnx, cny;
  const double *gs_lo, *gs_hi;
};

__device__ __forceinline__ void tile_block_reduce(double& mx, double& sm) {
  __shared__ double s_mx[PT_THREADS / 64], s_sm[PT_THREADS / 64];
  mx = eu_wave_max(mx);
  sm = eu_wave_sum(sm);
  __syncthreads();
  if ((threadIdx.x & 63) == 0) { s_mx[threadIdx.x >> 6] = mx; s_sm[threadIdx.x >> 6] = sm; }
  __syncthreads();
  if (threadIdx.x == 0) {
    mx = s_mx[0]; sm = s_sm[0];
    for (int k = 1; k < PT_THREADS / 64; ++k) { mx = s_mx[k] > mx ? s_mx[k] : mx; sm += s_sm[k]; }
  }
}

__device__ __forceinline__ double factor_step(double aa, double own, double nbv) {
  const double cl = -1.0 * own, cb = -1.0 * nbv;
  double e = aa - cl * cl - cb * cb;
  if (e < 0.25 * aa) e = (aa != 0.0) ? aa : 1.0;
  return 1.0 / sqrt(e);
}

__global__ __launch_bounds__(64) void k_tile_table(double* __restrict__ tab) {
  const int lane = threadIdx.x & 63;
  double own = 0.0, out = 0.0;
  sw_d2 pp[8];
#pragma unroll
  for (int j = 0; j < 16; ++j) {
    const double nbv = wave_shift_inject<DPP_WAVE_SHR1>(out, 0.0);
    const double res = factor_step(4.0, own, nbv);
    own = res; out = res;
    if (j & 1) pp[j >> 1].y = res; else pp[j >> 1].x = res;
  }
#pragma unroll
  for (int P = 0; P < 8; ++P) reinterpret_cast<sw_d2*>(tab)[P * 64 + lane] = pp[P];
}
int eu_launch_tile_table(euler_sim* S) {
  hipLaunchKernelGGL(k_tile_table, dim3(1), dim3(64), 0, S->stream, S->tile_table);
  return EULER_OK;
}

template <int CTRL>
__device__ __forceinline__ double dpp_move(double v) {
  const int lo = __builtin_amdgcn_update_dpp(0, __double2loint(v), CTRL, 0xf, 0xf, true);
  const int hi = __builtin_amdgcn_update_dpp(0, __double2hiint(v), CTRL, 0xf, 0xf, true);
  return __hiloint2double(hi, lo);
}
__device__ __forceinline__ double group_sum(double v) {
  v = v + dpp_move<0xB1>(v);
  v = v + dpp_move<0x4E>(v);
  if (MG_LG == 8) v = v + dpp_move<0x141>(v);
  return v;
}

template <int W>
__global__ __launch_bounds__(PT_THREADS) void k_factor_tile(TileArgs a) {
  if (!a.force && pcg_idle(a.sc)) return;
  const int lane = threadIdx.x & 63;
  const int ntb = a.g.T / W, total = a.nb_local * ntb;
  const int n_waves = gridDim.x * (PT_THREADS / 64);
  for (int tile = blockIdx.x * (PT_THREADS / 64) + (threadIdx.x >> 6); tile < total; tile += n_waves) {
    const int band = a.band_lo + tile / ntb, k = tile % ntb;
    const size_t base = ((size_t)band * a.g.TS + (size_t)k * W) * 64 + 2 * lane;
    unsigned int mm[W / 2];
    unsigned int any = 0;
#pragma unroll
    for (int P = 0; P < W / 2; ++P) { mm[P] = *reinterpret_cast<const unsigned short*>(a.mask + base + P * 128); any |= mm[P]; }
    if (!__ballot(((any | (any >> 8)) & CM_FLUID) != 0)) continue;
    sw_d2 pp[W / 2];
#pragma unroll
    for (int P = 0; P < W / 2; ++P) pp[P] = *reinterpret_cast<const sw_d2*>(a.pre + base + P * 128);
    double own = 0.0, out = 0.0;
#pragma unroll
    for (int j = 0; j < W; ++j) {
      const int cm = (int)((mm[j >> 1] >> ((j & 1) * 8)) & 0xff);
      const double cpre = (j & 1) ? pp[j >> 1].y : pp[j >> 1].x;
      const double nbv = wave_shift_inject<DPP_WAVE_SHR1>(out, 0.0);
      const double aa = (double)(cm >> CM_DIAG_SHIFT);
      const double res = (cm & CM_FLUID) ? factor_step(aa, own, nbv) : cpre;
      own = res; out = res;
      if (j & 1) pp[j >> 1].y = res; else pp[j >> 1].x = res;
    }
#pragma unroll
    for (int P = 0; P < W / 2; ++P) *reinterpret_cast<sw_d2*>(a.pre + base + P * 128) = pp[P];
  }
}

#ifndef PT_RECOMP_BLOCKS
#define PT_RECOMP_BLOCKS 1
#endif
template <int W, bool RECOMP = false, int CMODE = 0>
__global__ __launch_bounds__(PT_THREADS, RECOMP ? PT_RECOMP_BLOCKS : 1) void k_precond_tile(TileArgs a) {
  if (!a.force && pcg_idle(a.sc)) return;
  const int lane = threadIdx.x & 63;
  const int ntb = a.g.T / W, total = a.nb_local * ntb;
  const int n_waves = gridDim.x * (PT_THREADS / 64);
  const double nalpha = -(a.force ? a.alpha_arg : a.sc->alpha);
  double mx = 0.0, dsum = 0.0;
  const bool listed = W == 16 && a.list != nullptr;
  const int todo = listed ? (int)a.sc->n_chunks : total;
  constexpr int TABP = W == 16 ? 8 : 1;
  __shared__ sw_d2 s_tab[TABP][64];
  __shared__ double s_cpart[CMODE == 2 ? PT_THREADS / 64 : 1][CMODE == 2 ? 16 * 2 * MG_NSLOT : 1];
  (void)s_cpart;
  const bool have_tab = W == 16 && listed && a.table != nullptr;
  if (have_tab) {
    for (int k = threadIdx.x; k < TABP * 64; k += PT_THREADS) (&s_tab[0][0])[k] = reinterpret_cast<const sw_d2*>(a.table)[k];
    __syncthreads();
  }
  typedef std::integral_constant<bool, true> yes_t;
  typedef std::integral_constant<bool, false> no_t;
  for (int i = blockIdx.x * (PT_THREADS / 64) + (threadIdx.x >> 6); i < todo; i += n_waves) {
    const int ii = a.reverse ? todo - 1 - i : i;
    const unsigned int ent = listed ? a.list[ii] : (unsigned int)ii;
    const bool interior = have_tab && (ent & EU_CHUNK_INTERIOR) != 0;
    const int tile = (int)(listed ? ent & ~EU_CHUNK_INTERIOR : ent);
    const int band = a.band_lo + tile / ntb, k = tile % ntb;
    const size_t base = ((size_t)band * a.g.TS + (size_t)k * W) * 64 + 2 * lane;
    auto run = [&](auto full_tag) {
      constexpr bool FULL = decltype(full_tag)::value;
      unsigned int mm[W / 2];
      unsigned int any = 0;
#pragma unroll
      for (int P = 0; P < W / 2; ++P) {
        mm[P] = FULL ? (unsigned int)(CM_INTERIOR | (CM_INTERIOR << 8)) : (unsigned int)*reinterpret_cast<const unsigned short*>(a.mask + base + P * 128);
        any |= mm[P];
      }
      if (!FULL && !listed && !__ballot(((any | (any >> 8)) & CM_FLUID) != 0)) return;
      sw_d2 rr[W / 2], qq[W / 2], pp[W / 2];
#pragma unroll
      for (int P = 0; P < W / 2; ++P) {
        rr[P] = *reinterpret_cast<const sw_d2*>(a.r + base + P * 128);
        if (RECOMP && a.rupd) continue;
        if (!a.sweeps) pp[P] = sw_d2{0.0, 0.0};
        else if (FULL) pp[P] = s_tab[P < TABP ? P : 0][lane];
        else pp[P] = *reinterpret_cast<const sw_d2*>(a.pre + base + P * 128);
        if (!RECOMP && a.rupd) qq[P] = *reinterpret_cast<const sw_d2*>(a.as + base + P * 128);
      }
      if (RECOMP && a.rupd) {
        const int npairs = a.g.TS / 2, P0 = k * (W / 2);
        sw_d2 ss[W / 2 + 2];
#pragma unroll
        for (int P = -1; P <= W / 2; ++P)
          ss[P + 1] = (P0 + P >= 0 && P0 + P < npairs) ? *reinterpret_cast<const sw_d2*>(a.as + base + (long long)P * 128) : sw_d2{0.0, 0.0};
        double ev = 0.0;
        if (lane < 16) {
          const int x = k * W + lane;
          if (x < a.g.X) {
            if (a.gs_lo && band == a.band_lo) ev = a.gs_lo[x];
            else if (band > 0) ev = a.as[skew_index(a.g, x, 64 * band - 1)];
          }
        } else if (lane >= 48) {
          const int x = k * W + lane - 48 - 63;
          if (x >= 0 && x < a.g.X) {
            if (a.gs_hi && band == a.band_lo + a.nb_local - 1) ev = a.gs_hi[x];
            else if (band + 1 < a.g.nbands) ev = a.as[skew_index(a.g, x, 64 * (band + 1))];
          }
        }
        const int ev_lo = __double2loint(ev), ev_hi = __double2hiint(ev);
#pragma unroll
        for (int P = 0; P < W / 2; ++P) {
          const unsigned int m0 = mm[P] & 0xff, m1 = mm[P] >> 8;
          const sw_d2 cc = ss[P + 1];
          const double prev_y = ss[P].y, nxt_x = ss[P + 2].x;
          const double d0 = __hiloint2double(__builtin_amdgcn_readlane(ev_hi, 2 * P), __builtin_amdgcn_readlane(ev_lo, 2 * P));
          const double d1 = __hiloint2double(__builtin_amdgcn_readlane(ev_hi, 2 * P + 1), __builtin_amdgcn_readlane(ev_lo, 2 * P + 1));
          const double u0 = __hiloint2double(__builtin_amdgcn_readlane(ev_hi, 48 + 2 * P), __builtin_amdgcn_readlane(ev_lo, 48 + 2 * P));
          const double u1 = __hiloint2double(__builtin_amdgcn_readlane(ev_hi, 49 + 2 * P), __builtin_amdgcn_readlane(ev_lo, 49 + 2 * P));
          const double dn0 = wave_shift_inject<DPP_WAVE_SHR1>(prev_y, d0), up0 = wave_shift_inject<DPP_WAVE_SHL1>(cc.y, u0);
          const double dn1 = wave_shift_inject<DPP_WAVE_SHR1>(cc.x, d1), up1 = wave_shift_inject<DPP_WAVE_SHL1>(nxt_x, u1);
          double v = (double)(int)(m0 >> CM_DIAG_SHIFT) * cc.x;
          v = v - ((m0 & CM_RIGHT) ? cc.y : 0.0);
          v = v - ((m0 & CM_UP) ? up0 : 0.0);
          v = v - ((m0 & CM_LEFT) ? prev_y : 0.0);
          v = v - ((m0 & CM_DOWN) ? dn0 : 0.0);
          if (m0 & CM_FLUID) { rr[P].x = rr[P].x + v * nalpha; const double w = fabs(rr[P].x); if (w > mx) mx = w; }
          v = (double)(int)(m1 >> CM_DIAG_SHIFT) * cc.y;
          v = v - ((m1 & CM_RIGHT) ? nxt_x : 0.0);
          v = v - ((m1 & CM_UP) ? up1 : 0.0);
          v = v - ((m1 & CM_LEFT) ? cc.x : 0.0);
          v = v - ((m1 & CM_DOWN) ? dn1 : 0.0);
          if (m1 & CM_FLUID) { rr[P].y = rr[P].y + v * nalpha; const double w = fabs(rr[P].y); if (w > mx) mx = w; }
          *reinterpret_cast<sw_d2*>(a.r + base + P * 128) = rr[P];
        }
      }
      if (!RECOMP && a.rupd) {
#pragma unroll
        for (int P = 0; P < W / 2; ++P) {
          if (mm[P] & CM_FLUID) { rr[P].x = rr[P].x + qq[P].x * nalpha; const double v = fabs(rr[P].x); if (v > mx) mx = v; }
          if ((mm[P] >> 8) & CM_FLUID) { rr[P].y = rr[P].y + qq[P].y * nalpha; const double v = fabs(rr[P].y); if (v > mx) mx = v; }
          *reinterpret_cast<sw_d2*>(a.r + base + P * 128) = rr[P];
        }
      }
      if (!a.sweeps) return;
      if (W == 16 && CMODE == 2) {
        const int quad = lane >> 2, G = (lane + 4) >> 3;
        const int uy = 64 * band + lane - MG_G0 / 2, I0 = uy >> MG_LOG;
        double wy1 = (double)(uy & (MG_G0 - 1)), wy0 = (double)MG_G0 - wy1;
        if (I0 < 0) { wy0 = 0.0; wy1 = (double)MG_G0; }
        if (I0 >= a.cny - 1) { wy0 = (double)MG_G0; wy1 = 0.0; }
        const int x0 = 16 * k - lane - MG_G0 / 2, Jb = x0 >> MG_LOG, tbase = MG_G0 * Jb - x0;
        const int Jq = 2 * k - G - 1;
        double sg_s[MG_NSEG], sg_t[MG_NSEG];
#pragma unroll
        for (int m = 0; m < MG_NSEG; ++m) { sg_s[m] = 0.0; sg_t[m] = 0.0; }
#pragma unroll
        for (int j = 0; j < W; ++j) {
          const int cm = (int)((mm[j >> 1] >> ((j & 1) * 8)) & 0xff);
          const double rv = (cm & CM_FLUID) ? ((j & 1) ? rr[j >> 1].y : rr[j >> 1].x) : 0.0;
          const double jv = rv * (double)j;
#pragma unroll
          for (int m = 0; m < MG_NSEG; ++m) {
            const bool in = (m == 0 || j >= tbase + MG_G0 * m) && (m == MG_NSEG - 1 || j < tbase + MG_G0 * (m + 1));
            sg_s[m] += in ? rv : 0.0; sg_t[m] += in ? jv : 0.0;
          }
        }
        double cn[MG_NSEG + 1];
#pragma unroll
        for (int m = 0; m <= MG_NSEG; ++m) cn[m] = 0.0;
#pragma unroll
        for (int m = 0; m < MG_NSEG; ++m) {
          double u1 = sg_t[m] + (double)(-tbase - MG_G0 * m) * sg_s[m], u0 = (double)MG_G0 * sg_s[m] - u1;
          if (Jb + m < 0) { u0 = 0.0; u1 = (double)MG_G0 * sg_s[m]; }
          if (Jb + m >= a.cnx - 1) { u0 = (double)MG_G0 * sg_s[m]; u1 = 0.0; }
          cn[m] += u0; cn[m + 1] += u1;
        }
        const bool shifted = Jb != Jq;
        wy0 *= 1.0 / (MG_G0 * MG_G0); wy1 *= 1.0 / (MG_G0 * MG_G0);
        double* sp = s_cpart[threadIdx.x >> 6];
#pragma unroll
        for (int q = 0; q < MG_NSLOT; ++q) {
          const double lo = cn[q], hi = q >= 1 ? cn[q - 1] : 0.0;
          const double cs = shifted ? hi : lo;
          const double p0 = group_sum(wy0 * cs), p1 = group_sum(wy1 * cs);
          if ((lane & 3) == 0) { sp[quad * 2 * MG_NSLOT + q] = p0; sp[quad * 2 * MG_NSLOT + MG_NSLOT + q] = p1; }
        }
        __builtin_amdgcn_fence(__ATOMIC_RELEASE, "wavefront");
        __builtin_amdgcn_wave_barrier();
        {
          double* cp = a.cpart + ((size_t)(tile / ntb) * MG_NGRP * ntb + (size_t)k) * (2 * MG_NSLOT);
#pragma unroll
          for (int u = 0; u < (MG_PART + 63) / 64; ++u) {
            const int e = lane + 64 * u;
            if (e < MG_PART) {
              const int g = e / (2 * MG_NSLOT), w = e % (2 * MG_NSLOT);
              const double va = g > 0 ? sp[(2 * g - 1) * 2 * MG_NSLOT + w] : 0.0, vb = g < 8 ? sp[(2 * g) * 2 * MG_NSLOT + w] : 0.0;
              cp[((size_t)g * ntb) * (2 * MG_NSLOT) + w] = va + vb;
            }
          }
        }
        __builtin_amdgcn_fence(__ATOMIC_ACQUIRE, "wavefront");
        __builtin_amdgcn_wave_barrier();
      } else if (W == 16 && CMODE == 1) {
        const int xl = k * W - 63, J0 = (xl > 0 ? xl : 0) >> a.cshift;
        double c0 = 0.0, c1 = 0.0, c2 = 0.0;
#pragma unroll
        for (int j = 0; j < W; ++j) {
          const int cm = (int)((mm[j >> 1] >> ((j & 1) * 8)) & 0xff);
          const double rv = (cm & CM_FLUID) ? ((j & 1) ? rr[j >> 1].y : rr[j >> 1].x) : 0.0;
          const int x = k * W + j - lane;
          const int b = ((x > 0 ? x : 0) >> a.cshift) - J0;
          c0 += b == 0 ? rv : 0.0; c1 += b == 1 ? rv : 0.0; c2 += b == 2 ? rv : 0.0;
        }
        c0 = eu_wave_sum(c0); c1 = eu_wave_sum(c1); c2 = eu_wave_sum(c2);
        if (lane == 0) { double* cp = a.cpart + (size_t)tile * 3; cp[0] = c0; cp[1] = c1; cp[2] = c2; }
      }
      if (RECOMP && a.rupd) {
        asm volatile("" ::: "memory");
#pragma unroll
        for (int P = 0; P < W / 2; ++P) pp[P] = FULL ? s_tab[P < TABP ? P : 0][lane] : *reinterpret_cast<const sw_d2*>(a.pre + base + P * 128);
      }
      double own = -0.0, out = -0.0;
#pragma unroll
      for (int j = 0; j < W; ++j) {
        const int cm = (int)((mm[j >> 1] >> ((j & 1) * 8)) & 0xff);
        const double cin = (j & 1) ? rr[j >> 1].y : rr[j >> 1].x, cpre = (j & 1) ? pp[j >> 1].y : pp[j >> 1].x;
        const double nbv = wave_shift_inject<DPP_WAVE_SHR1>(out, -0.0);
        const double t = cin - own - nbv;
        const double qv = t * cpre;
        const double res = (cm & CM_FLUID) ? qv : 0.0;
        const double carry = -1.0 * cpre * res;
        own = carry; out = carry;
        if (j & 1) qq[j >> 1].y = res; else qq[j >> 1].x = res;
      }
      own = 0.0; out = 0.0;
#pragma unroll
      for (int j = W - 1; j >= 0; --j) {
        const int cm = (int)((mm[j >> 1] >> ((j & 1) * 8)) & 0xff);
        const double cin = (j & 1) ? qq[j >> 1].y : qq[j >> 1].x, cpre = (j & 1) ? pp[j >> 1].y : pp[j >> 1].x;
        const double crr = (j & 1) ? rr[j >> 1].y : rr[j >> 1].x;
        const double nbv = wave_shift_inject<DPP_WAVE_SHL1>(out, 0.0);
        const double kr = ((cm & CM_RIGHT) ? -1.0 : 0.0) * cpre, ku = ((cm & CM_UP) ? -1.0 : 0.0) * cpre;
        const double t = cin - kr * own - ku * nbv;
        const double zv = t * cpre;
        const double res = (cm & CM_FLUID) ? zv : 0.0;
        own = res; out = res;
        if (cm & CM_FLUID) dsum += res * crr;
        if (j & 1) qq[j >> 1].y = res; else qq[j >> 1].x = res;
      }
#pragma unroll
      for (int P = 0; P < W / 2; ++P) *reinterpret_cast<sw_d2*>(a.z + base + P * 128) = qq[P];
      if (band == a.edge_lo || band == a.edge_hi) {
        const bool lo = band == a.edge_lo && lane == 0, hi = band == a.edge_hi && lane == 63;
#pragma unroll
        for (int j = 0; j < W; ++j) {
          const double zv = (j & 1) ? qq[j >> 1].y : qq[j >> 1].x;
          const int x_lo = k * W + j, x_hi = k * W + j - 63;
          if (lo && x_lo < a.g.X) a.zsend_lo[x_lo] = zv;
          if (hi && x_hi >= 0 && x_hi < a.g.X) a.zsend_hi[x_hi] = zv;
        }
      }
    };
    if (W == 16 && interior) run(yes_t()); else run(no_t());
  }
  tile_block_reduce(mx, dsum);
  __shared__ int am_last;
  if (threadIdx.x == 0) {
    __hip_atomic_store(reinterpret_cast<unsigned long long*>(&a.part_max[blockIdx.x]), (unsigned long long)__double_as_longlong(mx), __ATOMIC_RELAXED, __HIP_MEMORY_SCOPE_AGENT);
    __hip_atomic_store(reinterpret_cast<unsigned long long*>(&a.part_dot[blockIdx.x]), (unsigned long long)__double_as_longlong(dsum), __ATOMIC_RELAXED, __HIP_MEMORY_SCOPE_AGENT);
    asm volatile("s_waitcnt vmcnt(0)" ::: "memory");
    const unsigned int t = __hip_atomic_fetch_add(a.counter, 1u, __ATOMIC_RELAXED, __HIP_MEMORY_SCOPE_AGENT);
    am_last = t == gridDim.x - 1;
  }
  __syncthreads();
  if (!am_last) return;
  double vmax = 0.0, vsum = 0.0;
  for (unsigned int i = threadIdx.x; i < gridDim.x; i += PT_THREADS) {
    const double m = __longlong_as_double((long long)__hip_atomic_load(reinterpret_cast<unsigned long long*>(&a.part_max[i]), __ATOMIC_RELAXED, __HIP_MEMORY_SCOPE_AGENT));
    const double d = __longlong_as_double((long long)__hip_atomic_load(reinterpret_cast<unsigned long long*>(&a.part_dot[i]), __ATOMIC_RELAXED, __HIP_MEMORY_SCOPE_AGENT));
    vmax = m > vmax ? m : vmax; vsum += d;
  }
  tile_block_reduce(vmax, vsum);
  if (a.via == FIN_VIA_P2P) {
    if (a.rupd) vmax = p2p_allreduce_block<true>(a.sc, vmax);
    if (a.fin_dot >= 0) vsum = p2p_allreduce_block<false>(a.sc, vsum);
  }
  if (threadIdx.x == 0) {
    if (a.via == FIN_TO_COMM) { a.pair_slot[0] = vmax; a.pair_slot[1] = vsum; }
    else {
      if (a.rupd) pcg_scalar_step(a.sc, FIN_RNORM, vmax);
      if (a.fin_dot >= 0 && !(a.rupd && a.sc->done)) pcg_scalar_step(a.sc, a.fin_dot, vsum);
    }
    __hip_atomic_store(a.counter, 0u, __ATOMIC_RELAXED, __HIP_MEMORY_SCOPE_AGENT);
  }
}

struct SRing { const double* s[8]; int n, steps; };
__global__ __launch_bounds__(256) void k_finish_p(double* __restrict__ p, const uint8_t* __restrict__ mask, size_t e_lo, size_t S,
                                                  const PcgScalars* sc, SRing ring) {
  if (!sc->nonzero || sc->iters == 0) return;
  const int n_it = sc->iters;
  const int from = n_it - 1 >= ring.steps ? (n_it - 1) / ring.steps * ring.steps : 0;
  const int cnt = n_it - from;
  double al[8];
  const double* sp[8];
#pragma unroll
  for (int j = 0; j < 8; ++j) { const int it = from + (j < cnt ? j : 0); al[j] = sc->alpha_hist[it & 7]; sp[j] = ring.s[it % ring.n] + e_lo; }
  for (size_t i = 2 * ((size_t)blockIdx.x * blockDim.x + threadIdx.x); i < S; i += 2 * (size_t)gridDim.x * blockDim.x) {
    const unsigned int mm = *reinterpret_cast<const unsigned short*>(mask + i);
    const bool f0 = (mm & CM_FLUID) != 0, f1 = ((mm >> 8) & CM_FLUID) != 0;
    if (!(f0 | f1)) continue;
    sw_d2 pv = *reinterpret_cast<const sw_d2*>(p + i);
#pragma unroll
    for (int j = 0; j < 8; ++j) {
      if (j < cnt) {
        const sw_d2 sv = *reinterpret_cast<const sw_d2*>(sp[j] + i);
        if (f0) pv.x = pv.x + sv.x * al[j];
        if (f1) pv.y = pv.y + sv.y * al[j];
      }
    }
    *reinterpret_cast<sw_d2*>(p + i) = pv;
  }
}

int eu_launch_finish_p(euler_sim* S) {
  if (S->s_ring_n <= 0) return EULER_OK;
  SRing ring;
  for (int k = 0; k < 8; ++k) ring.s[k] = S->s_ring[k < S->s_ring_n ? k : 0];
  ring.n = S->s_ring_n; ring.steps = S->s_ring_n;
  LAUNCH(S, KC_UPDATE_PR, k_finish_p, dim3(eu_blocks(S->e_cnt, 256 * 4, 4096)), dim3(256), S->p + S->e_lo, S->cellmask + S->e_lo, S->e_lo, S->e_cnt, S->sc, ring);
  return EULER_OK;
}

static SweepArgs make_sweep_args(euler_sim* S, int op, int force) {
  SweepArgs a;
  a.g = S->geom;
  a.mask = S->cellmask; a.fbits_fwd = S->fbits_fwd; a.fbits_bwd = S->fbits_bwd; a.fb_stride = S->fb_stride; a.pre = S->precon;
  a.in = op == SW_FORWARD ? S->r : S->q;
  a.out = op == SW_FORWARD ? S->q : S->z;
  a.granules = S->granules; a.gran_stride = S->gran_stride; a.ticket = S->ticket;
  a.xg_in = nullptr; a.xg_out = nullptr;
  a.ranges = S->band_ranges;
  a.band_lo = S->band_lo; a.nb_local = S->band_hi - S->band_lo; a.couple = S->has_comm && S->couple;
  a.ticket_base = S->ticket_base; a.epoch = S->epoch;
  a.sc = S->sc; a.force = force; a.error = &S->ms->error;
  a.timeline = S->sweep_timeline;
  a.tile_w = eu_is_tile(S) ? S->tile_w : 0;
  a.fin_qq = -1; a.qq_partial = S->partial; a.qq_counter = S->red_counter; a.sc_w = S->sc;
  return a;
}

__global__ __launch_bounds__(1024) void k_band_ranges(const uint8_t* __restrict__ count, int X, int Y, int T, int4* __restrict__ ranges, int band0) {
  __shared__ int s_lo, s_hi;
  const int band = band0 + blockIdx.x;
  if (threadIdx.x == 0) { s_lo = 0x7fffffff; s_hi = -1; }
  __syncthreads();
  int lo = 0x7fffffff, hi = -1;
  const int rows = Y - band * 64 < 64 ? Y - band * 64 : 64;
  for (int x = threadIdx.x; x < X; x += 1024) {
    for (int l0 = 0; l0 < rows; l0 += 8) {
      uint8_t c[8];
#pragma unroll
      for (int k = 0; k < 8; ++k) c[k] = l0 + k < rows ? count[(size_t)(band * 64 + l0 + k) * X + x] : (uint8_t)0;
#pragma unroll
      for (int k = 0; k < 8; ++k)
        if (c[k]) { const int t = x + l0 + k; lo = t < lo ? t : lo; hi = t > hi ? t : hi; }
    }
  }
  if (hi >= 0) { atomicMin(&s_lo, lo); atomicMax(&s_hi, hi); }
  __syncthreads();
  if (threadIdx.x == 0) {
    int4 r = make_int4(0, 0, 0, 0);
    if (s_hi >= 0) {
      const int f0 = s_lo / 32 * 32, f1 = (s_hi + 2 + 31) / 32 * 32;
      const int b0 = (T - 1 - s_hi) / 32 * 32, b1 = (T - 1 - s_lo + 2 + 31) / 32 * 32;
      r = make_int4(f0 / 8, f1 / 8, b0 / 8, b1 / 8);
    }
    ranges[band] = r;
  }
}
__global__ __launch_bounds__(256) void k_pack_fbits(const uint8_t* __restrict__ cellmask, SkewGeom g, unsigned int* __restrict__ fwd,
                                                    unsigned int* __restrict__ bwd, int fb_stride, int band_lo, int nb_local) {
  const size_t i = (size_t)blockIdx.x * 256 + threadIdx.x;
  if (i >= (size_t)nb_local * fb_stride * 64) return;
  const int lane = (int)(i & 63);
  const int gi = (int)((i >> 6) % fb_stride), band = band_lo + (int)((i >> 6) / fb_stride);
  const uint8_t* base = cellmask + (size_t)band * g.TS * 64 + 2 * lane;
  unsigned int wf = 0, wb = 0;
#pragma unroll
  for (int j = 0; j < 8; ++j) {
    const int tf = 8 * gi + j, tb = g.T - 1 - 8 * gi - j;
    if (tf < g.T && (base[(size_t)(tf & ~1) * 64 + (tf & 1)] & CM_FLUID)) wf |= 1u << j;
    if (tb >= 0) {
      const unsigned int m = base[(size_t)(tb & ~1) * 64 + (tb & 1)];
      if (m & CM_FLUID) wb |= 1u << j;
      if (m & CM_RIGHT) wb |= 1u << (8 + j);
      if (m & CM_UP) wb |= 1u << (16 + j);
    }
  }
  const size_t o = ((size_t)band * fb_stride + gi) * 64 + lane;
  fwd[o] = wf; bwd[o] = wb;
}
int eu_launch_band_ranges(euler_sim* S) {
  if (eu_is_tile(S)) return EULER_OK;
  const bool nbrs = S->has_comm && S->couple && !S->slab_on;
  const int b0 = nbrs && S->band_lo > 0 ? S->band_lo - 1 : S->band_lo, b1 = nbrs && S->band_hi < S->geom.nbands ? S->band_hi + 1 : S->band_hi;
  LAUNCH(S, KC_BUILD_SYSTEM, k_band_ranges, dim3(b1 - b0), dim3(1024), S->count, S->X, S->Y, S->geom.T, S->band_ranges, b0);
  const int nbl = S->band_hi - S->band_lo;
  const size_t n = (size_t)nbl * S->fb_stride * 64;
  LAUNCH(S, KC_BUILD_SYSTEM, k_pack_fbits, dim3((unsigned)((n + 255) / 256)), dim3(256), S->cellmask, S->geom, S->fbits_fwd, S->fbits_bwd,
         S->fb_stride, S->band_lo, nbl);
  return EULER_OK;
}

__global__ void k_scalar_epilogue(PcgScalars* sc, int op, int force) {
  if (!force && pcg_idle(sc)) return;
  pcg_scalar_step(sc, op, sc->comm_val);
}
__global__ void k_nonzero_to_comm(PcgScalars* sc) { sc->comm_val = sc->nonzero ? 1.0 : 0.0; }
__global__ void k_nonzero_from_comm(PcgScalars* sc) { sc->nonzero = sc->comm_val != 0.0; }

__global__ __launch_bounds__(256) void k_pack_row(const double* __restrict__ skew, double* __restrict__ row, SkewGeom g, int band, int lane) {
  const int x = blockIdx.x * 256 + threadIdx.x;
  if (x < g.X) row[x] = skew[skew_index(g, x, band * 64 + lane)];
}
__global__ __launch_bounds__(256) void k_unpack_row(double* __restrict__ skew, const double* __restrict__ row, SkewGeom g, int band, int lane) {
  const int x = blockIdx.x * 256 + threadIdx.x;
  if (x < g.X) skew[skew_index(g, x, band * 64 + lane)] = row[x];
}

template <bool PACK>
__global__ __launch_bounds__(256) void k_halo_rows2(double* a, double* b, double* lo, double* hi, SkewGeom g, int band_lo, int band_hi,
                                                    int has_lo, int has_hi) {
  const int x = blockIdx.x * 256 + threadIdx.x;
  if (x >= g.X) return;
  const int side = blockIdx.y >> 1, vec = blockIdx.y & 1;
  if (side == 0 ? !has_lo : !has_hi) return;
  double* arr = vec ? b : a;
  double* buf = (side ? hi : lo) + (size_t)vec * g.X;
  const int y = PACK ? (side ? 64 * band_hi - 1 : 64 * band_lo) : (side ? 64 * band_hi : 64 * band_lo - 1);
  double* e = arr + skew_index(g, x, y);
  if (PACK) buf[x] = *e; else *e = buf[x];
}

#define COMM_CALL(expr) do { if ((expr) != 0) { eu_set_error("communicator callback failed: %s", #expr); return EULER_ECOMM; } } while (0)

static inline bool tile_fused(const euler_sim* S);
static inline bool ghost_mode(const euler_sim* S) { return S->has_comm && !S->p2p_on && tile_fused(S); }
enum { XR_ZSEND_LO = 0, XR_ZSEND_HI, XR_ZRECV_LO, XR_ZRECV_HI, XR_GS_LO0, XR_GS_LO1, XR_GS_HI0, XR_GS_HI1 };
static inline double* xrow(const euler_sim* S, int k) { return S->xrows + (size_t)k * S->xrow_len; }
static int comm_exchange(euler_sim* S, double* send_lo, double* send_hi, double* recv_lo, double* recv_hi, int count, double* small, int nsmall) {
  if (S->bulk.exchange) {
    COMM_CALL(S->bulk.exchange(S->bulk.ctx, send_lo, send_hi, recv_lo, recv_hi, count, small, nsmall));
    return EULER_OK;
  }
  if (count > 0) COMM_CALL(S->bulk.halo(S->bulk.ctx, send_lo, send_hi, recv_lo, recv_hi, count));
  if (nsmall > 0) {
    int64_t off[64], cnt[64];
    for (int r = 0; r < S->bulk.nranks && r < 64; ++r) { off[r] = (int64_t)8 * nsmall * r; cnt[r] = (int64_t)8 * nsmall; }
    COMM_CALL(S->bulk.allgather(S->bulk.ctx, small, off, cnt));
  }
  return EULER_OK;
}
__global__ void k_alpha_fold(PcgScalars* sc, const double* __restrict__ vals, int R, int force) {
  if (!force && pcg_idle(sc)) return;
  double v = 0.0;
  for (int r = 0; r < R; ++r) v += vals[r];
  pcg_scalar_step(sc, FIN_ALPHA, v);
}

static int comm_allreduce_scalar(euler_sim* S, int is_max) {
  COMM_CALL(S->comm.allreduce(S->comm.ctx, &S->sc->comm_val, 1, is_max));
  return EULER_OK;
}
static int comm_finish(euler_sim* S, int fin_op, int is_max, int force) {
  if (S->p2p_on) return EULER_OK;
  if (fin_op == FIN_ALPHA && ghost_mode(S)) {
    int rc = comm_exchange(S, nullptr, nullptr, nullptr, nullptr, 0, S->alpha_buf, 1);
    if (rc) return rc;
    hipLaunchKernelGGL(k_alpha_fold, dim3(1), dim3(1), 0, S->stream, S->sc, S->alpha_buf, S->comm.nranks, force);
    return EULER_OK;
  }
  int rc = comm_allreduce_scalar(S, is_max);
  if (rc) return rc;
  hipLaunchKernelGGL(k_scalar_epilogue, dim3(1), dim3(1), 0, S->stream, S->sc, fin_op, force);
  return EULER_OK;
}
static inline int fin_or_comm(const euler_sim* S, int fin_op) {
  return S->has_comm ? (S->p2p_on ? (fin_op | FIN_VIA_P2P) : (int)FIN_TO_COMM) : fin_op;
}

static int comm_halo_s(euler_sim* S) {
  if (S->p2p_on) return eu_p2p_halo_skewed(S, S->s);
  const int X = S->X, nbk = (X + 255) / 256;
  double *send_lo = S->halo_buf, *send_hi = S->halo_buf + X, *recv_lo = S->halo_buf + 2 * X, *recv_hi = S->halo_buf + 3 * X;
  const bool has_lo = S->band_lo > 0, has_hi = S->band_hi < S->geom.nbands;
  if (has_lo) hipLaunchKernelGGL(k_pack_row, dim3(nbk), dim3(256), 0, S->stream, S->s, send_lo, S->geom, S->band_lo, 0);
  if (has_hi) hipLaunchKernelGGL(k_pack_row, dim3(nbk), dim3(256), 0, S->stream, S->s, send_hi, S->geom, S->band_hi - 1, 63);
  COMM_CALL(S->comm.halo(S->comm.ctx, send_lo, send_hi, recv_lo, recv_hi, X));
  if (has_lo) hipLaunchKernelGGL(k_unpack_row, dim3(nbk), dim3(256), 0, S->stream, S->s, recv_lo, S->geom, S->band_lo - 1, 63);
  if (has_hi) hipLaunchKernelGGL(k_unpack_row, dim3(nbk), dim3(256), 0, S->stream, S->s, recv_hi, S->geom, S->band_hi, 0);
  return EULER_OK;
}

template <int OP>
static int launch_sweep(euler_sim* S, int cls, int force, int fin_qq = -1) {
  if (S->cfg.sweep_mode != EULER_SWEEP_SIMPLE) {
    constexpr bool BWD = OP == SW_BACKWARD;
    const int nb = S->geom.nbands, nbl = S->band_hi - S->band_lo;
    const bool chain = S->has_comm && S->couple;
    const int64_t row_bytes = (int64_t)S->gran_stride * 2 * 8;
    const int g_first = BWD ? nb - S->band_hi : S->band_lo, g_last = g_first + nbl - 1;
    const int r = S->comm.rank, prev_rank = BWD ? r + 1 : r - 1, next_rank = BWD ? r - 1 : r + 1;
    S->epoch += 1;
    if (chain && S->p2p_on) {
      SweepArgs a = make_sweep_args(S, OP, force);
      eu_p2p_xgran(S, BWD ? 1 : 0, &a.xg_in, &a.xg_out);
      LAUNCH(S, cls, (k_sweep_skew<OP, true>), dim3(nbl), dim3(192), a);
      S->ticket_base += (unsigned)nbl;
      return EULER_OK;
    }
    if (chain && g_first > 0)
      COMM_CALL(S->comm.chain(S->comm.ctx, S->granules + (size_t)(g_first - 1) * S->gran_stride * 2, row_bytes, prev_rank, r));
    SweepArgs a = make_sweep_args(S, OP, force);
    a.fin_qq = fin_qq;
    LAUNCH(S, cls, k_sweep_skew<OP>, dim3(nbl), dim3(192), a);
    S->ticket_base += (unsigned)nbl;
    if (chain && g_last + 1 < nb)
      COMM_CALL(S->comm.chain(S->comm.ctx, S->granules + (size_t)g_last * S->gran_stride * 2, row_bytes, r, next_rank));
  } else {
    SweepArgs a = make_sweep_args(S, OP, force);
    LAUNCH(S, cls, k_sweep_simple<OP>, dim3(1), dim3(1024), a);
  }
  return EULER_OK;
}

#define LOC(ptr) ((ptr) + S->e_lo)
static inline int loc_red_blocks(const euler_sim* S) { return (int)eu_blocks(S->e_cnt, EU_RED_ELEMS, 2048); }

static int launch_dot(euler_sim* S, const double* a, const double* b, int fin_op, int force) {
  if (S->cfg.dot_mode == EULER_DOT_SEQUENTIAL && !S->has_comm) {
    LAUNCH(S, KC_DOT, k_dot_sequential, dim3(1), dim3(256), a, b, S->cellmask, S->geom, S->sc, fin_op, force);
  } else {
    const int edges = (a == S->z && S->has_comm && eu_p2p_has_neighbour_arrays(S)) ? ((S->band_lo > 0 ? 1 : 0) | (S->band_hi < S->geom.nbands ? 2 : 0)) : 0;
    if (edges)
      LAUNCH(S, KC_DOT, k_dot_partial<true>, dim3(loc_red_blocks(S)), dim3(RED_THREADS), LOC(a), LOC(b), LOC(S->cellmask), S->e_cnt,
             S->partial, S->sc, force, S->red_counter, fin_or_comm(S, fin_op), S->geom.TS, S->band_hi - S->band_lo, edges);
    else
      LAUNCH(S, KC_DOT, k_dot_partial<false>, dim3(loc_red_blocks(S)), dim3(RED_THREADS), LOC(a), LOC(b), LOC(S->cellmask), S->e_cnt,
             S->partial, S->sc, force, S->red_counter, fin_or_comm(S, fin_op), 0, 0, 0);
    if (S->has_comm) return comm_finish(S, fin_op, 0, force);
  }
  return EULER_OK;
}

static inline bool tile_fused(const euler_sim* S) { return eu_is_tile(S) && S->cfg.sweep_mode != EULER_SWEEP_SIMPLE; }
static inline int sa_run(const euler_sim* S);
static inline bool tile_recompute(const euler_sim* S) {
  if (S->opt[EULER_OPT_TILE_STORE_AS] || sa_run(S) != 8) return false;
  if (!tile_fused(S)) return !S->has_comm && S->cfg.dot_mode != EULER_DOT_SEQUENTIAL;
  if (S->tile_w != 16) return false;
  if (S->has_comm) return ghost_mode(S);
  return S->cfg.dot_mode != EULER_DOT_SEQUENTIAL;
}
__global__ void k_pair_fold(PcgScalars* sc, const double* __restrict__ pairs, int stride, int R, int rupd, int fin_dot, int force) {
  if (!force && pcg_idle(sc)) return;
  double vmax = 0.0, vsum = 0.0;
  for (int r = 0; r < R; ++r) { vmax = pairs[(size_t)stride * r] > vmax ? pairs[(size_t)stride * r] : vmax; vsum += pairs[(size_t)stride * r + 1]; }
  if (rupd) pcg_scalar_step(sc, FIN_RNORM, vmax);
  if (fin_dot >= 0 && !(rupd && sc->done)) pcg_scalar_step(sc, fin_dot, vsum);
}
static TileArgs make_tile_args(euler_sim* S, int force) {
  TileArgs a;
  a.g = S->geom; a.mask = S->cellmask; a.pre = S->precon; a.r = S->r; a.as = S->tile_as_override ? S->tile_as_override : S->q; a.z = S->z;
  a.band_lo = S->band_lo; a.nb_local = S->band_hi - S->band_lo;
  a.rupd = 0; a.sweeps = 1; a.fin_dot = -1;
  a.via = S->has_comm ? (S->p2p_on ? (int)FIN_VIA_P2P : (int)FIN_TO_COMM) : 0;
  a.part_max = S->partial; a.part_dot = S->partial2; a.counter = S->red_counter; a.sc = S->sc; a.force = force; a.alpha_arg = 0.0;
  a.pair_slot = S->pair_buf + 2 * (S->has_comm ? S->comm.rank : 0);
  a.list = !force ? S->chunk_list : nullptr;
  a.table = S->tile_table;
  a.zsend_lo = a.zsend_hi = nullptr; a.edge_lo = a.edge_hi = -1;
  a.reverse = S->opt[EULER_OPT_TILE_REVERSE] != 0;
  a.cpart = nullptr; a.cshift = 0; a.cmode = 0; a.cnx = a.cny = 0;
  a.gs_lo = a.gs_hi = nullptr;
  if (ghost_mode(S)) {
    if (S->band_lo > 0) { a.zsend_lo = xrow(S, XR_ZSEND_LO); a.edge_lo = S->band_lo; }
    if (S->band_hi < S->geom.nbands) { a.zsend_hi = xrow(S, XR_ZSEND_HI); a.edge_hi = S->band_hi - 1; }
  }
  return a;
}
static inline unsigned tile_blocks(const euler_sim* S) {
  const size_t tiles = (size_t)(S->band_hi - S->band_lo) * (S->geom.T / S->tile_w);
  return eu_blocks(tiles, PT_THREADS / 64, 2048);
}
static int launch_factor_tile(euler_sim* S, int force) {
  const TileArgs a = make_tile_args(S, force);
  switch (S->tile_w) {
    case 8: LAUNCH(S, KC_PRECON_FACTOR, k_factor_tile<8>, dim3(tile_blocks(S)), dim3(PT_THREADS), a); break;
    case 32: LAUNCH(S, KC_PRECON_FACTOR, k_factor_tile<32>, dim3(tile_blocks(S)), dim3(PT_THREADS), a); break;
    default: LAUNCH(S, KC_PRECON_FACTOR, k_factor_tile<16>, dim3(tile_blocks(S)), dim3(PT_THREADS), a); break;
  }
  return EULER_OK;
}
static int launch_precond_tile(euler_sim* S, int rupd, int sweeps, int fin_dot, int force, double alpha, bool r_only = false) {
  const bool seq = S->cfg.dot_mode == EULER_DOT_SEQUENTIAL && !S->has_comm;
  TileArgs a = make_tile_args(S, force);
  a.rupd = rupd; a.sweeps = sweeps; a.fin_dot = (seq || !sweeps) ? -1 : fin_dot; a.alpha_arg = alpha;
  const bool two_level = eu_is_two_level(S) && sweeps && !r_only && !force && a.list != nullptr;
  const int fin_real = a.fin_dot;
  if (two_level) {
    const bool mg = eu_is_mg(S);
    a.cpart = mg ? S->mg_part : S->cc_part; a.cshift = mg ? 0 : S->coarse_shift;
    a.cmode = mg ? 2 : 1; a.cnx = mg ? S->mg_nx[0] : 0; a.cny = mg ? S->mg_ny[0] : 0;
    if (a.fin_dot >= 0) a.fin_dot = FIN_STORE_ONLY;
  }
  double* xsmall = S->pair_buf;
  int nsmall = 2;
  bool split = false;
  if (two_level && a.via == FIN_TO_COMM) {
    split = eu_is_mg(S) && ghost_mode(S) && eu_mg_split(S);
    nsmall = eu_coarse_comm_slots(S);
    if (nsmall < 0) return EULER_ENOMEM;
    xsmall = S->mg_xbuf;
    a.pair_slot = xsmall + (size_t)S->comm.rank * nsmall;
    if (split) {
      if (a.zsend_lo) a.zsend_lo = eu_mg_split_msg(S, 0);
      if (a.zsend_hi) a.zsend_hi = eu_mg_split_msg(S, 1);
    }
  }
  const int w = r_only ? 16 : S->tile_w, cls = r_only ? KC_UPDATE_PR : KC_PRECOND_TILE;
  const unsigned nblk = eu_blocks((size_t)(S->band_hi - S->band_lo) * (S->geom.T / w), PT_THREADS / 64, 2048);
  const bool recomp = rupd && !force && tile_recompute(S) && (r_only ? S->tile_as_override == S->q : !S->tile_as_override);
  if (recomp) {
    a.as = S->s;
    if (ghost_mode(S)) {
      if (S->band_lo > 0) a.gs_lo = xrow(S, XR_GS_LO0 + S->gs_cur);
      if (S->band_hi < S->geom.nbands) a.gs_hi = xrow(S, XR_GS_HI0 + S->gs_cur);
    }
  }
  switch (w) {
    case 8: LAUNCH(S, cls, k_precond_tile<8>, dim3(nblk), dim3(PT_THREADS), a); break;
    case 32: LAUNCH(S, cls, k_precond_tile<32>, dim3(nblk), dim3(PT_THREADS), a); break;
    default:
      if (a.cmode == 2) { if (recomp) LAUNCH(S, cls, (k_precond_tile<16, true, 2>), dim3(nblk), dim3(PT_THREADS), a); else LAUNCH(S, cls, (k_precond_tile<16, false, 2>), dim3(nblk), dim3(PT_THREADS), a); }
      else if (a.cmode == 1) { if (recomp) LAUNCH(S, cls, (k_precond_tile<16, true, 1>), dim3(nblk), dim3(PT_THREADS), a); else LAUNCH(S, cls, (k_precond_tile<16, false, 1>), dim3(nblk), dim3(PT_THREADS), a); }
      else if (recomp) LAUNCH(S, cls, (k_precond_tile<16, true>), dim3(nblk), dim3(PT_THREADS), a);
      else LAUNCH(S, cls, k_precond_tile<16>, dim3(nblk), dim3(PT_THREADS), a);
      break;
  }
  if (two_level && a.via != FIN_TO_COMM) { int rc = eu_launch_coarse_solve(S, fin_real, force); if (rc) return rc; }
  if (seq && sweeps && fin_dot >= 0)
    LAUNCH(S, KC_DOT, k_dot_sequential, dim3(1), dim3(256), S->z, S->r, S->cellmask, S->geom, S->sc, fin_dot, force);
  if (a.via == FIN_TO_COMM) {
    const int R = S->comm.nranks;
    const bool rows = ghost_mode(S) && !force;
    int rc = !two_level ? EULER_OK : split ? eu_mg_split_pre(S) : eu_launch_coarse_pre(S, force);
    if (rc) return rc;
    if (split) rc = comm_exchange(S, eu_mg_split_msg(S, 0), eu_mg_split_msg(S, 1), eu_mg_split_msg(S, 2), eu_mg_split_msg(S, 3), eu_mg_split_count(S), xsmall, nsmall);
    else rc = comm_exchange(S, xrow(S, XR_ZSEND_LO), xrow(S, XR_ZSEND_HI), xrow(S, XR_ZRECV_LO), xrow(S, XR_ZRECV_HI), rows ? S->X : 0, xsmall, nsmall);
    if (rc) return rc;
    hipLaunchKernelGGL(k_pair_fold, dim3(1), dim3(1), 0, S->stream, S->sc, xsmall, nsmall, R, rupd, a.fin_dot, force);
    if (split) {
      if ((rc = eu_mg_split_mid(S, fin_real, force, xrow(S, XR_ZRECV_LO), xrow(S, XR_ZRECV_HI)))) return rc;
      if ((rc = comm_exchange(S, nullptr, nullptr, nullptr, nullptr, 0, eu_mg_split_gc(S), 1 + MG_NULL_MAX))) return rc;
      return eu_mg_split_fold(S, fin_real, force);
    }
    if (two_level) { rc = eu_launch_coarse_scatter(S); if (rc) return rc; rc = eu_launch_coarse_solve(S, fin_real, force); if (rc) return rc; }
  }
  return EULER_OK;
}

static int comm_halo_two(euler_sim* S, double* a, double* b) {
  if (S->p2p_on) { int rc = eu_p2p_halo_skewed(S, a); return rc ? rc : eu_p2p_halo_skewed(S, b); }
  const int X = S->X, nbk = (X + 255) / 256;
  double *send_lo = S->halo_buf, *send_hi = S->halo_buf + 2 * X, *recv_lo = S->halo_buf + 4 * X, *recv_hi = S->halo_buf + 6 * X;
  const int has_lo = S->band_lo > 0, has_hi = S->band_hi < S->geom.nbands;
  hipLaunchKernelGGL(k_halo_rows2<true>, dim3(nbk, 4), dim3(256), 0, S->stream, a, b, send_lo, send_hi, S->geom, S->band_lo, S->band_hi, has_lo, has_hi);
  COMM_CALL(S->comm.halo(S->comm.ctx, send_lo, send_hi, recv_lo, recv_hi, 2 * X));
  hipLaunchKernelGGL(k_halo_rows2<false>, dim3(nbk, 4), dim3(256), 0, S->stream, a, b, recv_lo, recv_hi, S->geom, S->band_lo, S->band_hi, has_lo, has_hi);
  return EULER_OK;
}

static inline bool dot_rides_in_sweep(const euler_sim* S) {
  return S->cfg.precond == EULER_PRECOND_IC0 && S->cfg.sweep_mode != EULER_SWEEP_SIMPLE && !S->has_comm && S->cfg.dot_mode != EULER_DOT_SEQUENTIAL;
}
static int launch_precondition(euler_sim* S, int force, int fin_dot = -1) {
  if (S->cfg.precond == EULER_PRECOND_JACOBI) {
    LAUNCH(S, KC_JACOBI, k_jacobi, dim3(eu_blocks(S->e_cnt, 256 * 4, 4096)), dim3(256), LOC(S->r), LOC(S->z), LOC(S->cellmask),
           S->e_cnt, S->sc, force);
    return fin_dot >= 0 ? launch_dot(S, S->z, S->r, fin_dot, force) : EULER_OK;
  }
  const bool ride = fin_dot >= 0 && dot_rides_in_sweep(S);
  int rc = launch_sweep<SW_FORWARD>(S, KC_FORWARD_SOLVE, force, ride ? fin_dot : -1);
  if (rc) return rc;
  if ((rc = launch_sweep<SW_BACKWARD>(S, KC_BACKWARD_SOLVE, force))) return rc;
  return fin_dot >= 0 && !ride ? launch_dot(S, S->z, S->r, fin_dot, force) : EULER_OK;
}

static int launch_apply_a_and_alpha(euler_sim* S, int force) {
  const bool seq = S->cfg.dot_mode == EULER_DOT_SEQUENTIAL && !S->has_comm;
  if (S->has_comm && ghost_mode(S) && !force) {
    const int X = S->X, nbk = (X + 255) / 256;
    const bool coarse = eu_is_two_level(S);
    if (S->band_lo > 0) {
      HIPCHK(hipMemcpyAsync(xrow(S, XR_GS_LO0), xrow(S, XR_ZRECV_LO), (size_t)X * 8, hipMemcpyDeviceToDevice, S->stream));
      if (coarse) { int rc = eu_launch_coarse_add_row(S, xrow(S, XR_GS_LO0), 64 * S->band_lo - 1); if (rc) return rc; }
      hipLaunchKernelGGL(k_unpack_row, dim3(nbk), dim3(256), 0, S->stream, S->s, xrow(S, XR_GS_LO0), S->geom, S->band_lo - 1, 63);
    }
    if (S->band_hi < S->geom.nbands) {
      HIPCHK(hipMemcpyAsync(xrow(S, XR_GS_HI0), xrow(S, XR_ZRECV_HI), (size_t)X * 8, hipMemcpyDeviceToDevice, S->stream));
      if (coarse) { int rc = eu_launch_coarse_add_row(S, xrow(S, XR_GS_HI0), 64 * S->band_hi); if (rc) return rc; }
      hipLaunchKernelGGL(k_unpack_row, dim3(nbk), dim3(256), 0, S->stream, S->s, xrow(S, XR_GS_HI0), S->geom, S->band_hi, 0);
    }
    S->gs_cur = 0;
  } else if (S->has_comm) { int rc = comm_halo_s(S); if (rc) return rc; }
  SkewGeom gl = S->geom;
  gl.S = S->e_cnt;
  double* out = tile_fused(S) ? S->q : S->z;
  LAUNCH(S, KC_APPLY_A, k_apply_a, dim3(loc_red_blocks(S)), dim3(RED_THREADS), LOC(S->s), LOC(out), LOC(S->cellmask), gl,
         S->partial, S->sc, force, S->red_counter, seq ? -1 : fin_or_comm(S, FIN_ALPHA));
  if (seq)
    LAUNCH(S, KC_DOT, k_dot_sequential, dim3(1), dim3(256), out, S->s, S->cellmask, S->geom, S->sc, (int)FIN_ALPHA, force);
  if (S->has_comm) return comm_finish(S, FIN_ALPHA, 0, force);
  return EULER_OK;
}

static inline unsigned sa_blocks(const euler_sim* S, int run) {
  const size_t runs = (size_t)(S->band_hi - S->band_lo) * ((S->geom.TS / 2 + run - 1) / run);
  return eu_blocks(runs, SA_THREADS / 64, 2048);
}
static inline int sa_run(const euler_sim* S) {
  if (S->opt[EULER_OPT_SA_RUN] != 8 && !S->has_comm && !eu_is_two_level(S)) return (int)S->opt[EULER_OPT_SA_RUN];
  return 8;
}
static inline int p_steps(const euler_sim* S) {
  if (S->p2p_on || sa_run(S) != 8) return 2;
  return (int)S->opt[EULER_OPT_P_STEPS];
}
static int ring_begin(euler_sim* S) {
  const int n = p_steps(S);
  if (!S->s_base[0]) { S->s_base[0] = S->s; S->s_base[1] = S->s2; }
  if (n > 2) { S->s = S->s_base[0]; S->s2 = S->s_base[1]; }
  else if (S->s != S->s_base[0] && S->s != S->s_base[1]) { S->s = S->s_base[0]; S->s2 = S->s_base[1]; }
  else if (S->s2 != S->s_base[0] && S->s2 != S->s_base[1]) S->s2 = S->s == S->s_base[0] ? S->s_base[1] : S->s_base[0];
  S->s_ring[0] = S->s; S->s_ring[1] = S->s2;
  for (int k = 2; k < n; ++k) {
    if (!S->s_ring_alloc[k]) {
      const size_t elems = S->Sw + EU_SKEW_SLACK;
      if (hipMalloc(&S->s_ring_alloc[k], elems * sizeof(double)) != hipSuccess) {
        (void)hipGetLastError();
        S->s_ring_alloc[k] = nullptr;
        for (int j = 2; j < k; ++j) if (S->s_ring_alloc[j]) { (void)hipFree(S->s_ring_alloc[j]); S->s_ring_alloc[j] = nullptr; S->hbm_bytes -= elems * sizeof(double); }
        S->opt[EULER_OPT_P_STEPS] = 2;
        return ring_begin(S);
      }
      S->hbm_bytes += elems * sizeof(double);
      HIPCHK(hipMemsetAsync(S->s_ring_alloc[k], 0, elems * sizeof(double), S->stream));
    }
    S->s_ring[k] = static_cast<double*>(S->s_ring_alloc[k]) + EU_SKEW_SLACK - S->skew_off;
  }
  S->s_ring_n = n;
  S->s_launched = 0;
  return EULER_OK;
}
double* eu_current_search_direction(euler_sim* S) {
  if (S->s_ring_n < 2 || S->s_launched <= 0) return S->s;
  (void)hipStreamSynchronize(S->stream);
  const int ran = S->sc_host->nonzero ? S->sc_host->iters : 0;
  if (ran <= 0 || ran > S->s_launched) return S->s;
  return S->s_ring[(ran - 1) % S->s_ring_n];
}
static int launch_search_apply_and_alpha(euler_sim* S, int it) {
  const bool seq = S->cfg.dot_mode == EULER_DOT_SEQUENTIAL && !S->has_comm;
  SlabNeighbours nbr = {nullptr, nullptr, nullptr, nullptr, S->band_hi - S->band_lo, nullptr, nullptr, nullptr, nullptr, nullptr, nullptr};
  const bool direct = S->has_comm && eu_p2p_has_neighbour_arrays(S);
  const bool ghost = ghost_mode(S);
  if (ghost) {
    const int c = S->gs_cur;
    if (S->band_lo > 0) { nbr.zrow_dn = xrow(S, XR_ZRECV_LO); nbr.srow_dn = xrow(S, XR_GS_LO0 + c); nbr.snew_dn = xrow(S, XR_GS_LO0 + (c ^ 1)); }
    if (S->band_hi < S->geom.nbands) { nbr.zrow_up = xrow(S, XR_ZRECV_HI); nbr.srow_up = xrow(S, XR_GS_HI0 + c); nbr.snew_up = xrow(S, XR_GS_HI0 + (c ^ 1)); }
    S->gs_cur = c ^ 1;
  } else if (direct) {
    eu_p2p_neighbour_arrays(S, &nbr.z_dn, &nbr.s_dn, &nbr.z_up, &nbr.s_up);
    if (nbr.z_dn) { nbr.z_dn += S->e_lo; nbr.s_dn += S->e_lo; }
    if (nbr.z_up) { nbr.z_up += S->e_lo; nbr.s_up += S->e_lo; }
  } else if (S->has_comm) {
    int rc = comm_halo_two(S, S->z, S->s);
    if (rc) return rc;
  }
  SkewGeom gl = S->geom;
  gl.S = S->e_cnt;
  const int steps = S->s_ring_n;
  const int pmode = (it >= steps && it % steps == 0) ? steps : 1;
  SaHist hist = {{nullptr, nullptr, nullptr, nullptr, nullptr, nullptr}};
  for (int j = 1; j + 1 < steps; ++j) hist.s[j - 1] = LOC(S->s_ring[j]);
  const int run = sa_run(S);
  const int fin = S->has_comm ? fin_or_comm(S, FIN_ALPHA) : (seq ? -1 : (int)FIN_ALPHA);
  double* pp = LOC(S->p);
  const bool store = !tile_recompute(S);
  const bool mg = eu_is_mg(S);
  const CoarseRef cref = {mg ? S->mg_x : S->cc_y, mg ? 0 : S->coarse_shift, mg ? S->mg_nx[0] : S->coarse_nx, mg ? S->mg_ny[0] : S->coarse_ny, S->band_lo};
#define SA_LAUNCH_CS(SLABF, PM, RUNV, CF, ST)                                                                                                \
  LAUNCH(S, KC_APPLY_A, (k_search_apply<SLABF, PM, RUNV, CF, ST>), dim3(sa_blocks(S, RUNV)), dim3(SA_THREADS), LOC(S->s), LOC(S->z), LOC(S->s2), \
         LOC(S->q), LOC(S->cellmask), gl, S->partial, S->sc, 0, S->red_counter, fin, nbr, pp, S->s2, S->s, (RUNV) == 8 ? S->chunk_list : (const unsigned int*)nullptr, cref, hist)
#define SA_LAUNCH_C(SLABF, PM, RUNV, CF) do { if ((RUNV) == 8 && !store) SA_LAUNCH_CS(SLABF, PM, RUNV, CF, ((RUNV) != 8)); else SA_LAUNCH_CS(SLABF, PM, RUNV, CF, true); } while (0)
#define SA_LAUNCH(SLABF, PM, RUNV) SA_LAUNCH_C(SLABF, PM, RUNV, 0)
#define SA_RUNS(SLABF, PM) do { if (run == 8) SA_LAUNCH(SLABF, PM, 8); else if (run == 16) SA_LAUNCH(SLABF, PM, 16); else SA_LAUNCH(SLABF, PM, 32); } while (0)
  if (eu_is_two_level(S) && tile_fused(S) && ghost) {
    if (pmode == 8) SA_LAUNCH_C(2, 8, 8, 2); else if (pmode == 4) SA_LAUNCH_C(2, 4, 8, 2); else if (pmode == 2) SA_LAUNCH_C(2, 2, 8, 2); else SA_LAUNCH_C(2, 1, 8, 2);
  } else if (eu_is_two_level(S) && tile_fused(S)) {
    if (mg) { if (pmode == 8) SA_LAUNCH_C(0, 8, 8, 2); else if (pmode == 4) SA_LAUNCH_C(0, 4, 8, 2); else if (pmode == 2) SA_LAUNCH_C(0, 2, 8, 2); else SA_LAUNCH_C(0, 1, 8, 2); }
    else { if (pmode == 8) SA_LAUNCH_C(0, 8, 8, 1); else if (pmode == 4) SA_LAUNCH_C(0, 4, 8, 1); else if (pmode == 2) SA_LAUNCH_C(0, 2, 8, 1); else SA_LAUNCH_C(0, 1, 8, 1); }
  } else if (ghost) {
    if (pmode == 8) SA_LAUNCH(2, 8, 8); else if (pmode == 4) SA_LAUNCH(2, 4, 8); else if (pmode == 2) SA_LAUNCH(2, 2, 8); else SA_LAUNCH(2, 1, 8);
  } else if (direct) {
    if (pmode == 2) { if (run == 8) SA_LAUNCH(1, 2, 8); else SA_LAUNCH(1, 2, 32); }
    else if (pmode == 1) { if (run == 8) SA_LAUNCH(1, 1, 8); else SA_LAUNCH(1, 1, 32); }
    else { if (run == 8) SA_LAUNCH(1, 0, 8); else SA_LAUNCH(1, 0, 32); }
  } else {
    if (pmode == 8) SA_LAUNCH(0, 8, 8); else if (pmode == 4) SA_LAUNCH(0, 4, 8); else if (pmode == 2) SA_RUNS(0, 2); else if (pmode == 1) SA_RUNS(0, 1); else SA_RUNS(0, 0);
  }
#undef SA_RUNS
#undef SA_LAUNCH
#undef SA_LAUNCH_C
#undef SA_LAUNCH_CS
  S->s = S->s_ring[it % steps]; S->s2 = S->s_ring[(it + 1) % steps];
  S->s_launched = it + 1;
  if (seq)
    LAUNCH(S, KC_DOT, k_dot_sequential, dim3(1), dim3(256), S->q, S->s, S->cellmask, S->geom, S->sc, (int)FIN_ALPHA, 0);
  if (S->has_comm) return comm_finish(S, FIN_ALPHA, 0, 0);
  return EULER_OK;
}

int eu_launch_build_system(euler_sim* S, float dt);
int eu_launch_velocity_update(euler_sim* S, float dt, int finish);

__global__ void k_pcg_reset(PcgScalars* sc, double tol, int max_iters) {
  sc->sigma = sc->zs = sc->sigma_new = sc->alpha = sc->alpha_prev = sc->beta = sc->rnorm = 0.0;
  sc->tol = tol; sc->nonzero = 0; sc->done = 0; sc->iters = 0; sc->max_iters = max_iters;
}

int eu_launch_project(euler_sim* S, float dt) {
  S->s_launched = 0;
  S->p_pending = 0;
  S->pcg_fields_resident = 0;
  const PcgScalars prev_solve = *S->sc_host;
  S->solve_iters[S->solve_seq & 255] = S->sc_host->nonzero ? S->sc_host->iters : -1;
  if (S->solve_seq > 0) { S->res_last_chunks = S->sc_host->n_chunks; S->res_have_last = 1; }
  S->solve_seq += 1;
  const int pred_iters = (S->sc_host->nonzero && S->sc_host->done && S->sc_host->iters < S->cfg.max_iterations) ? S->sc_host->iters : 0;
  const bool drain_poll = S->p2p_on && !(S->sc_host->nonzero && !S->sc_host->done && S->sc_host->iters >= S->cfg.max_iterations);
  S->prof_iter = -1;
  int rc;
  LAUNCH(S, KC_MISC, k_pcg_reset, dim3(1), dim3(1), S->sc, S->cfg.tol, S->cfg.max_iterations);
  eu_launch_build_system(S, dt);
  if (S->has_comm) {
    hipLaunchKernelGGL(k_nonzero_to_comm, dim3(1), dim3(1), 0, S->stream, S->sc);
    if ((rc = comm_allreduce_scalar(S, 1))) return rc;
    hipLaunchKernelGGL(k_nonzero_from_comm, dim3(1), dim3(1), 0, S->stream, S->sc);
  }
  const bool res_skip = S->res_skip_once != 0;
  S->res_skip_once = 0;
  if (!res_skip && eu_resident_eligible(S)) {
    const unsigned int cap_chunks = 4u * (unsigned int)eu_resident_capacity(S, S->cfg.pcg_precision == EULER_PCG_F32);
    unsigned int guess = S->res_last_chunks;
    if (!S->res_have_last) {
      HIPCHK(hipMemcpyAsync(S->sc_host, S->sc, sizeof(PcgScalars), hipMemcpyDeviceToHost, S->stream));
      HIPCHK(hipStreamSynchronize(S->stream));
      guess = S->sc_host->n_chunks;
    }
    if (guess + guess / 16 + 8 <= cap_chunks || S->cfg.pcg_precision == EULER_PCG_F32) {
      S->prof_iter = -2;
      if ((rc = eu_launch_resident(S, cap_chunks))) return rc;
      HIPCHK(hipMemcpyAsync(S->sc_host, S->sc, sizeof(PcgScalars), hipMemcpyDeviceToHost, S->stream));
      HIPCHK(hipStreamSynchronize(S->stream));
      S->res_last_chunks = S->sc_host->n_chunks; S->res_have_last = 1;
      const int err = *S->res_err;
      if (err == 0) {
        if (S->sc_host->nonzero) { S->res_solves += 1; S->pcg_fields_resident = 1; }
        if ((rc = eu_launch_velocity_update(S, dt, 0))) return rc;
        return EULER_OK;
      }
      *S->res_err = 0;
      if (S->cfg.pcg_precision == EULER_PCG_F32 && err == 2) { eu_set_error("EULER_PCG_F32: the solve's active chunks do not fit the resident solver"); return EULER_EHIP; }
      if (err != 2) { S->res_fallbacks += 1; S->res_disabled = 1; }
      S->solve_seq -= 1;
      S->lean_ok = 0;
      S->res_skip_once = 1;
      *S->sc_host = prev_solve;
      return eu_launch_project(S, dt);
    }
  }
  const bool tile = tile_fused(S);
  const bool two_level = tile && eu_is_two_level(S);
  if (two_level && S->has_comm && !(eu_is_mg(S) && ghost_mode(S) && S->slab_on)) {
    eu_set_error("coarse-correction preconditioners with several ranks: EULER_PRECOND_IC0_TILE_MG on row slabs without mailboxes only");
    return EULER_EINVAL;
  }
  if (two_level && (rc = eu_launch_coarse_setup(S))) return rc;
  if (two_level && (rc = eu_launch_coarse_consistent(S))) return rc;
  if (tile) {
    if ((rc = launch_factor_tile(S, 0))) return rc;
    if ((rc = launch_precond_tile(S, 0, 1, FIN_SIGMA_INIT, 0, 0.0))) return rc;
  } else {
  if (S->cfg.precond != EULER_PRECOND_JACOBI && (rc = launch_sweep<SW_FACTOR>(S, KC_PRECON_FACTOR, 0))) return rc;
  if ((rc = launch_precondition(S, 0, FIN_SIGMA_INIT))) return rc;
  }
  if ((rc = ring_begin(S))) return rc;
  const bool fold0 = two_level && eu_is_mg(S) && !S->has_comm && S->cfg.dot_mode != EULER_DOT_SEQUENTIAL && sa_run(S) == 8;
  if (fold0) {
    const PcgScalars& ps = prev_solve;
    if (ps.nonzero && !(std::isfinite(ps.alpha) && std::isfinite(ps.beta) && std::isfinite(ps.rnorm) && std::isfinite(ps.sigma) && std::isfinite(ps.zs)))
      for (int k = 0; k < S->s_ring_n; ++k) HIPCHK(hipMemsetAsync(S->s_ring[k] + S->skew_off, 0, S->Sw * sizeof(double), S->stream));
  }
  else if (two_level) { if ((rc = eu_launch_coarse_search_init(S))) return rc; }
  else
  LAUNCH(S, KC_UPDATE_SEARCH, k_update_search<true>, dim3(eu_blocks(S->e_cnt, 256 * 4, 4096)), dim3(256), LOC(S->s), LOC(S->z),
         LOC(S->cellmask), S->e_cnt, S->sc, 0, 0.0);
  if (S->has_comm && eu_p2p_has_neighbour_arrays(S)) {
    const int y0 = S->band_lo > 0 ? 64 * S->band_lo : -1, y1 = S->band_hi < S->geom.nbands ? 64 * S->band_hi - 1 : -1;
    LAUNCH(S, KC_UPDATE_SEARCH, k_publish_edge_rows, dim3((S->X + 255) / 256, 2), dim3(256), S->s, S->geom, y0, y1, S->sc);
  }
  if (S->s_ring_n == 2) HIPCHK(hipMemsetAsync(LOC(S->s2), 0, S->e_cnt * sizeof(double), S->stream));
  S->s_stale = 1;
  HIPCHK(hipMemcpyAsync(S->sc_host, S->sc, sizeof(PcgScalars), hipMemcpyDeviceToHost, S->stream));
  HIPCHK(hipStreamSynchronize(S->stream));
  const int poll = S->cfg.pcg_poll_interval > 0 ? S->cfg.pcg_poll_interval : 8;
  const int max_it = S->cfg.max_iterations;
  int it = 0, chunk = 0;
  bool stop = !S->sc_host->nonzero;
  S->s_none = stop ? 1 : 0;
  while (it < max_it && !stop) {
    int chunk_end = it + poll;
    if (!drain_poll && pred_iters > 0 && it < pred_iters + poll && chunk_end > pred_iters - 2) {
      const int lo = pred_iters - 2 < chunk_end ? pred_iters - 2 : chunk_end;
      chunk_end = lo > it + 2 ? lo : it + 2;
    }
    if (chunk_end > max_it) chunk_end = max_it;
    for (; it < chunk_end; ++it) {
      S->prof_iter = it;
      const bool fused = it > 0 || fold0;
      if (it == 0 && fold0) { S->s = S->s_ring[S->s_ring_n - 1]; S->s2 = S->s_ring[0]; }
      if ((rc = fused ? launch_search_apply_and_alpha(S, it) : launch_apply_a_and_alpha(S, 0))) return rc;
      if (tile) {
        S->prof_iter = it;
        if ((rc = launch_precond_tile(S, 1, it + 1 < max_it, FIN_BETA, 0, 0.0))) return rc;
        continue;
      }
      S->tile_as_override = fused ? S->q : S->z;
      rc = launch_precond_tile(S, 1, 0, -1, 0, 0.0, true);
      S->tile_as_override = nullptr;
      if (rc) return rc;
      if (it + 1 < max_it) {
        S->prof_iter = it + 1;
        if ((rc = launch_precondition(S, 0, FIN_BETA))) return rc;
      }
    }
    if (it < max_it && drain_poll) {
      HIPCHK(hipMemcpyAsync(S->sc_host, S->sc, sizeof(PcgScalars), hipMemcpyDeviceToHost, S->stream));
      HIPCHK(hipStreamSynchronize(S->stream));
      stop = S->sc_host->done != 0;
    } else
    if (it < max_it) {
      const int slot = chunk & 1;
      if (chunk > 0) {
        HIPCHK(hipEventSynchronize(S->poll_event[slot ^ 1]));
        stop = S->poll_host[slot ^ 1].done != 0;
      }
      HIPCHK(hipMemcpyAsync(&S->poll_host[slot], S->sc, sizeof(PcgScalars), hipMemcpyDeviceToHost, S->stream));
      HIPCHK(hipEventRecord(S->poll_event[slot], S->stream));
      ++chunk;
    }
  }
  S->prof_iter = -2;
  const bool finish_in_update = !S->has_comm && !S->slab_on && S->opt[EULER_OPT_VELOCITY_TWO_PASS] == 0;
  if (!finish_in_update) { if ((rc = eu_launch_finish_p(S))) return rc; }
  if (S->s_ring_n > 2) { S->s = S->s_base[0]; S->s2 = S->s_base[1]; }
  if (S->has_comm && S->slab_on) {
    const int X = S->X, nbk = (X + 255) / 256;
    double *send_lo = S->halo_buf, *send_hi = S->halo_buf + X, *recv_lo = S->halo_buf + 2 * X, *recv_hi = S->halo_buf + 3 * X;
    if (S->band_lo > 0) hipLaunchKernelGGL(k_pack_row, dim3(nbk), dim3(256), 0, S->stream, S->p, send_lo, S->geom, S->band_lo, 0);
    COMM_CALL(S->bulk.halo(S->bulk.ctx, send_lo, send_hi, recv_lo, recv_hi, X));
    if (S->band_hi < S->geom.nbands) hipLaunchKernelGGL(k_unpack_row, dim3(nbk), dim3(256), 0, S->stream, S->p, recv_hi, S->geom, S->band_hi, 0);
  } else if (S->has_comm) {
    const int n = S->comm.nranks, nb = S->geom.nbands;
    std::vector<int64_t> off(n), cnt(n);
    for (int k = 0; k < n; ++k) {
      const int64_t lo = (int64_t)nb * k / n, hi = (int64_t)nb * (k + 1) / n;
      off[k] = lo * S->geom.TS * 64 * 8;
      cnt[k] = (hi - lo) * S->geom.TS * 64 * 8;
    }
    COMM_CALL(S->comm.allgather(S->comm.ctx, S->p, off.data(), cnt.data()));
  }
  if ((rc = eu_launch_velocity_update(S, dt, finish_in_update ? 1 : 0))) return rc;
  HIPCHK(hipMemcpyAsync(S->sc_host, S->sc, sizeof(PcgScalars), hipMemcpyDeviceToHost, S->stream));
  return EULER_OK;
}

int eu_launch_pcg_op(euler_sim* S, int op, float dt, double a, double* out) {
  S->s_none = 0;
  S->s_launched = 0;
  const bool want_scalar = op == EULER_OP_DOT_ZR || op == EULER_OP_DOT_ZS || op == EULER_OP_INF_NORM_R;
  const size_t SS = S->geom.S;
  if (eu_is_two_level(S) && (op == EULER_OP_PRECON_FACTOR || op == EULER_OP_FORWARD_SOLVE || op == EULER_OP_BACKWARD_SOLVE)) {
    eu_set_error("euler_pcg_op: the preconditioner of EULER_PRECOND_IC0_TILE2 / _MG is not available as a single operation (select EULER_PRECOND_IC0_TILE for its tile level)");
    return EULER_EINVAL;
  }
  switch (op) {
    case EULER_OP_BUILD_SYSTEM:
      LAUNCH(S, KC_MISC, k_pcg_reset, dim3(1), dim3(1), S->sc, S->cfg.tol, S->cfg.max_iterations);
      eu_launch_build_system(S, dt);
      break;
    case EULER_OP_PRECON_FACTOR: if (tile_fused(S)) launch_factor_tile(S, 1); else launch_sweep<SW_FACTOR>(S, KC_PRECON_FACTOR, 1); break;
    case EULER_OP_FORWARD_SOLVE: if (!tile_fused(S)) launch_sweep<SW_FORWARD>(S, KC_FORWARD_SOLVE, 1); break;
    case EULER_OP_BACKWARD_SOLVE:
      if (tile_fused(S)) launch_precond_tile(S, 0, 1, FIN_STORE_ONLY, 1, 0.0); else launch_sweep<SW_BACKWARD>(S, KC_BACKWARD_SOLVE, 1);
      break;
    case EULER_OP_APPLY_A:
      LAUNCH(S, KC_APPLY_A, k_apply_a, dim3(S->red_blocks), dim3(RED_THREADS), S->s, S->z, S->cellmask, S->geom,
             S->partial, S->sc, 1, S->red_counter, -1);
      break;
    case EULER_OP_DOT_ZR: launch_dot(S, S->z, S->r, FIN_STORE_ONLY, 1); break;
    case EULER_OP_DOT_ZS: launch_dot(S, S->z, S->s, FIN_STORE_ONLY, 1); break;
    case EULER_OP_INF_NORM_R:
      LAUNCH(S, KC_UPDATE_PR, k_inf_norm, dim3(S->red_blocks), dim3(RED_THREADS), S->r, S->cellmask, SS, S->partial);
      LAUNCH(S, KC_REDUCE_FINAL, k_reduce_final<true>, dim3(1), dim3(RED_THREADS), S->partial, S->red_blocks, S->sc,
             (int)FIN_STORE_ONLY, 1);
      break;
    case EULER_OP_UPDATE_PR:
      LAUNCH(S, KC_UPDATE_PR, k_update_pr, dim3(S->red_blocks), dim3(RED_THREADS), S->p, S->r, S->s, S->z, S->cellmask,
             SS, S->partial, S->sc, 1, a, S->red_counter, -1);
      break;
    case EULER_OP_UPDATE_SEARCH:
      LAUNCH(S, KC_UPDATE_SEARCH, k_update_search<false>, dim3(eu_blocks(SS, 256 * 4, 4096)), dim3(256), S->s, S->z,
             S->cellmask, SS, S->sc, 1, a);
      break;
    default: eu_set_error("unknown pcg op %d", op); return EULER_EINVAL;
  }
  HIPCHK(hipMemcpyAsync(S->sc_host, S->sc, sizeof(PcgScalars), hipMemcpyDeviceToHost, S->stream));
  HIPCHK(hipStreamSynchronize(S->stream));
  if (want_scalar && out) *out = S->sc_host->sigma_new;
  return EULER_OK;
}
```

include/euler.h:

```cpp
#ifndef EULER_H
#define EULER_H

#include <stddef.h>
#include <stdint.h>

#ifdef __cplusplus
extern "C" {
#endif

#define EULER_ABI_VERSION 2

enum {
  EULER_OK = 0,
  EULER_EINVAL = -1,
  EULER_ENOMEM = -2,
  EULER_EIO = -3,
  EULER_EHIP = -4,
  EULER_ESTATE = -5,
  EULER_ETIMEOUT = -6,
  EULER_ECOMM = -7
};

enum {
  EULER_DOT_AUTO = 0,
// ... 37 lines not shown
} euler_config;

enum { EULER_PCG_F64 = 0, EULER_PCG_F32 = 1 };
enum { EULER_RESIDENT_AUTO = 0, EULER_RESIDENT_OFF = 1 };

typedef struct euler_sim euler_sim;

enum {
  EULER_F_U = 0,
  EULER_F_V,
  EULER_F_UTMP,
  EULER_F_VTMP,
  EULER_F_SOLID,
  EULER_F_SOURCE,
  EULER_F_SINK,
  EULER_F_COUNT,
  EULER_F_PREV_COUNT,
  EULER_F_MARKERS,
  EULER_F_PRECON,
  EULER_F_PRESSURE,
  EULER_F_PCG_B, EULER_F_PCG_R, EULER_F_PCG_Z, EULER_F_PCG_S, EULER_F_PCG_Q,
  EULER_F_CELLMASK,
  EULER_F_DYE_R, EULER_F_DYE_G, EULER_F_DYE_B,
  EULER_F_DYE_RTMP, EULER_F_DYE_GTMP, EULER_F_DYE_BTMP,
  EULER_F_MARKER_KEYS,
  EULER_F__COUNT
};

enum {
  EULER_STAGE_ADVECT_MARKERS = 0,
  EULER_STAGE_REFRESH_COUNTS,
  EULER_STAGE_SOURCES,
  EULER_STAGE_EXTRAPOLATE,
  EULER_STAGE_ADVECT_VELOCITY,
  EULER_STAGE_PROJECT,
  EULER_STAGE__COUNT
};

enum {
  EULER_OP_BUILD_SYSTEM = 0,
  EULER_OP_PRECON_FACTOR,
  EULER_OP_FORWARD_SOLVE,
  EULER_OP_BACKWARD_SOLVE,
  EULER_OP_APPLY_A,
  EULER_OP_DOT_ZR,
  EULER_OP_DOT_ZS,
  EULER_OP_INF_NORM_R,
  EULER_OP_UPDATE_PR,
  EULER_OP_UPDATE_SEARCH,
  EULER_OP__COUNT
};

typedef struct euler_stats {
  uint64_t frames;
  uint64_t total_substeps;
  uint64_t total_pcg_iterations;
  int32_t  last_substeps;
  int32_t  last_pcg_iterations;
  double   last_residual;
  float    last_dt;
  uint64_t n_markers;
  int32_t  source_exhausted;
  uint64_t rng_state;
  uint64_t marker_dt_events;
  uint64_t marker_multi_events;
  uint64_t fluid_cells;
} euler_stats;

int  euler_config_default(euler_config* cfg);
int  euler_create(const euler_config* cfg, euler_sim** out);
void euler_destroy(euler_sim* sim);
const char* euler_last_error(void);
int  euler_abi_version(void);
int  euler_resident_info(euler_sim* sim, uint64_t out[3]);

int euler_load_scenario_mem(euler_sim* sim, const char* text, int32_t len, int32_t upscale);
int euler_load_scenario_file(euler_sim* sim, const char* path, int32_t upscale);
int euler_load_half_tank(euler_sim* sim);
int euler_load_half_tanks(euler_sim* sim, int32_t tanks);

int euler_parse_scenario(const char* text, int32_t len, int32_t X, int32_t Y, int32_t upscale,
                         uint8_t* solid, uint8_t* source, uint8_t* sink, uint8_t* fluid);
int euler_seed_markers(const uint8_t* fluid, int32_t X, int32_t Y, uint64_t* rng_state,
                       float* markers_xy, uint64_t* n_markers);

int euler_step(euler_sim* sim);
int euler_timestep(euler_sim* sim, float frame_time_left, float* dt);
int euler_substep(euler_sim* sim, float dt);
int euler_stage(euler_sim* sim, int32_t stage, float dt);
int euler_pcg_op(euler_sim* sim, int32_t op, float dt, double scalar_in, double* scalar_out);
int euler_set_precond(euler_sim* sim, int32_t precond, int32_t tile_records);
int euler_set_solver(euler_sim* sim, int32_t max_iterations, double tol);

int euler_get_field(euler_sim* sim, int32_t field, void* dst, size_t dst_bytes);
int euler_set_field(euler_sim* sim, int32_t field, const void* src, size_t src_bytes);
int euler_set_markers(euler_sim* sim, const float* xy, uint64_t n);
int euler_set_rng(euler_sim* sim, uint64_t rng_state, int32_t source_exhausted);
int euler_get_stats(euler_sim* sim, euler_stats* out);

int euler_save_state(euler_sim* sim, const char* path);
int euler_load_state(euler_sim* sim, const char* path);
size_t euler_field_bytes(const euler_sim* sim, int32_t field);

int euler_render(euler_sim* sim, int32_t wx, int32_t wy, char* out, int32_t cap, int32_t* len);
int euler_render_grids(const uint8_t* solid, const uint8_t* sink, const uint8_t* count,
                       int32_t X, int32_t Y, int32_t wx, int32_t wy, char* out, int32_t cap, int32_t* len);
int euler_render_grids_rgb(const uint8_t* solid, const uint8_t* sink, const uint8_t* count,
                           const float* r, const float* g, const float* b,
                           int32_t X, int32_t Y, int32_t wx, int32_t wy, char* out, int32_t cap, int32_t* len);
int euler_colorize(euler_sim* sim);

typedef struct euler_comm_ops {
  void*   ctx;
  int32_t rank, nranks;
  int (*allreduce)(void* ctx, void* dev_f64, int32_t count, int32_t is_max);
  int (*halo)(void* ctx, void* send_lo, void* send_hi, void* recv_lo, void* recv_hi, int32_t count);
  int (*chain)(void* ctx, void* dev_ptr, int64_t nbytes, int32_t src, int32_t dst);
  int (*allgather)(void* ctx, void* dev_base, const int64_t* off, const int64_t* cnt);
  int (*exchange)(void* ctx, void* send_lo, void* send_hi, void* recv_lo, void* recv_hi, int32_t count, void* small, int32_t nsmall);
} euler_comm_ops;

enum {
  EULER_SLAB_EXACT = 1,
  EULER_SLAB_LOCAL = 0
};
int euler_set_comm(euler_sim* sim, const euler_comm_ops* ops, int32_t coupling);

#define EULER_RCCL_ID_BYTES 128
int euler_rccl_unique_id(void* id_out, int32_t cap);
int euler_rccl_version(void);
int euler_set_comm_rccl(euler_sim* sim, const void* unique_id, int32_t id_bytes, int32_t rank, int32_t nranks,
                        int32_t coupling);
enum {
  EULER_OPT_P_STEPS = 1,
  EULER_OPT_TILE_STORE_AS = 2,
  EULER_OPT_TILE_REVERSE = 3,
  EULER_OPT_RESIDENT_CAP = 4,
  EULER_OPT_GRID4_MIN_CELLS = 5,
  EULER_OPT_SLAB_FUSION = 6,
  EULER_OPT_RCCL_SMALL = 7,
  EULER_OPT_RCCL_NO_EXCHANGE = 8,
  EULER_OPT_MARKERS_ROWMAJOR = 9,
  EULER_OPT_SA_RUN = 10,
  EULER_OPT_NO_INTERIOR = 11,
  EULER_OPT_BUILD_GATHER = 12,
  EULER_OPT_RESIDENT_FORCE_TIMEOUT = 13,
  EULER_OPT_MG_SPLIT_LEVEL = 14,
  EULER_OPT_MG_SPLIT_ACTIVE = 15,
  EULER_OPT_MARKERS_TWO_PASS = 16,
  EULER_OPT_BUILD_TWO_PASS = 17,
  EULER_OPT_VELOCITY_TWO_PASS = 18,
  EULER_OPT_NO_TILE_MAP = 19,
  EULER_OPT_PROFILE_STRIDE = 20,
  EULER_OPT__COUNT
};
int euler_set_option(euler_sim* sim, int32_t key, int64_t value);
int euler_get_option(euler_sim* sim, int32_t key, int64_t* value);

int euler_comm_calls(euler_sim* sim, uint64_t out[5]);

#define EULER_P2P_HANDLE_BYTES 256
int euler_p2p_export(euler_sim* sim, void* handle_out, int32_t cap);
int euler_p2p_connect(euler_sim* sim, const void* handles, int32_t nranks);
int euler_p2p_disconnect(euler_sim* sim);
int euler_p2p_calls(euler_sim* sim, uint64_t out[2]);
int euler_set_stream(euler_sim* sim, void* hip_stream);
int euler_slab_info(euler_sim* sim, int32_t* band_lo, int32_t* band_hi, int32_t* nbands);

int euler_profile_enable(euler_sim* sim, uint64_t class_mask);
int euler_profile_class_count(void);
const char* euler_profile_class_name(int32_t cls);
int euler_profile_get(euler_sim* sim, int32_t cls, double* total_ms, uint64_t* launches);
int euler_profile_reset(euler_sim* sim);
int euler_measure_copy_bandwidth(euler_sim* sim, size_t bytes, int32_t reps, double* gbps);
int euler_measure_exchange(euler_sim* sim, int32_t reps, int32_t row_doubles, int32_t nsmall, double* us_per_exchange);
int euler_device_name(euler_sim* sim, char* out, int32_t cap);
uint64_t euler_hbm_bytes(const euler_sim* sim);
int euler_sweep_timeline(euler_sim* sim, uint64_t* out, int32_t cap_bands);

#ifdef __cplusplus
}
#endif
#endif
```

Before: 180.2 million.

## Recompute preconditioned z inside search-apply instead of storing full z field

In the tiled IC0 preconditioner path, the precond kernel stops writing the full z vector and only stores tile-boundary halo values and band edge rows. The search-direction/apply-A kernel then re-runs the tile triangular solve from r and the preconditioner to regenerate z in registers, using the halos for cross-tile neighbours. The goal is to save a full f64 write and read of z per PCG iteration on this memory-bound solver. The cost is extra FLOPs and register pressure in search-apply, a fix-up pass that rebuilds z after the loop, and more complex gating on iteration parity.

```diff
diff --git a/euler_amd/__init__.py b/euler_amd/__init__.py
--- a/euler_amd/__init__.py
+++ b/euler_amd/__init__.py
@@ -10,7 +10,7 @@
 PRECOND_IC0, PRECOND_JACOBI, PRECOND_IC0_TILE, PRECOND_IC0_TILE2, PRECOND_IC0_TILE_MG = 0, 1, 2, 3, 4
 (OPT_P_STEPS, OPT_TILE_STORE_AS, OPT_TILE_REVERSE, OPT_RESIDENT_CAP, OPT_GRID4_MIN_CELLS, OPT_SLAB_FUSION, OPT_RCCL_SMALL, OPT_RCCL_NO_EXCHANGE, OPT_MARKERS_ROWMAJOR,
  OPT_SA_RUN, OPT_NO_INTERIOR, OPT_BUILD_GATHER, OPT_RESIDENT_FORCE_TIMEOUT, OPT_MG_SPLIT_LEVEL, OPT_MG_SPLIT_ACTIVE, OPT_MARKERS_TWO_PASS, OPT_BUILD_TWO_PASS,
- OPT_VELOCITY_TWO_PASS, OPT_NO_TILE_MAP, OPT_PROFILE_STRIDE) = range(1, 21)
+ OPT_VELOCITY_TWO_PASS, OPT_NO_TILE_MAP, OPT_PROFILE_STRIDE, OPT_TILE_STORE_Z) = range(1, 22)
 SWEEP_AUTO, SWEEP_BAND, SWEEP_SIMPLE = 0, 1, 2
 PCG_F64, PCG_F32 = 0, 1
 RESIDENT_AUTO, RESIDENT_OFF = 0, 1
diff --git a/euler_amd/csrc/driver.hip b/euler_amd/csrc/driver.hip
--- a/euler_amd/csrc/driver.hip
+++ b/euler_amd/csrc/driver.hip
@@ -245,7 +245,7 @@
   if (S->sys_m) (void)hipFree(S->sys_m);
   if (S->sys_div) (void)hipFree(S->sys_div);
   void* dev[] = {S->markers[0], S->markers[1], S->keys[0], S->keys[1], S->ms, S->evmask, S->delmask, S->ev_theta, S->ev_delta, S->sel_idx, S->act_idx,
-                 S->act_dt, S->cellmask64, S->draws, S->sel.block_sums, S->sc, S->partial, S->red_counter, S->granules, S->ticket, S->sweep_timeline, S->halo_buf, S->band_ranges, S->partial2, S->pair_buf, S->xrows, S->alpha_buf, S->rng_jump, S->chunk_flag, S->chunk_prev, S->chunk_part, S->tile_table, S->chunk_bits, S->chunk_list,
+                 S->act_dt, S->cellmask64, S->draws, S->sel.block_sums, S->sc, S->partial, S->red_counter, S->granules, S->ticket, S->sweep_timeline, S->halo_buf, S->band_ranges, S->partial2, S->pair_buf, S->xrows, S->alpha_buf, S->rng_jump, S->chunk_flag, S->chunk_prev, S->chunk_part, S->tile_table, S->chunk_bits, S->chunk_list, S->zhalo, S->zrows,
                  S->rowmajor_tmp};
   for (void* p : dev) if (p) (void)hipFree(p);
   for (float* d : S->dye) if (d) (void)hipFree(d + wo);
diff --git a/euler_amd/csrc/euler_dev.h b/euler_amd/csrc/euler_dev.h
--- a/euler_amd/csrc/euler_dev.h
+++ b/euler_amd/csrc/euler_dev.h
@@ -39,7 +39,8 @@
   int done;
   int iters;
   int max_iters;
-  unsigned int n_chunks, pad_;
+  unsigned int n_chunks;
+  unsigned int zfix;
   void** p2p_boxes;
   int* p2p_error;
   int p2p_rank, p2p_n;
@@ -201,6 +202,9 @@
   uint8_t* chunk_part;
   size_t hbm_bytes;
   int lean_ok;
+  double* zhalo;
+  double* zrows;
+  int z_halo_last;
   double* tile_table;
   unsigned long long* chunk_bits;
   unsigned int* chunk_list;
diff --git a/euler_amd/csrc/k_pcg.hip b/euler_amd/csrc/k_pcg.hip
--- a/euler_amd/csrc/k_pcg.hip
+++ b/euler_amd/csrc/k_pcg.hip
@@ -256,6 +256,37 @@
 }
 
 #define SA_THREADS 256
+template <int W, bool DOT>
+__device__ __forceinline__ void tile_solve(const unsigned int* mm, const sw_d2* rr, const sw_d2* pp, sw_d2* zz, double& dsum) {
+  double own = -0.0, out = -0.0;
+#pragma unroll
+  for (int j = 0; j < W; ++j) {
+    const int cm = (int)((mm[j >> 1] >> ((j & 1) * 8)) & 0xff);
+    const double cin = (j & 1) ? rr[j >> 1].y : rr[j >> 1].x, cpre = (j & 1) ? pp[j >> 1].y : pp[j >> 1].x;
+    const double nbv = wave_shift_inject<DPP_WAVE_SHR1>(out, -0.0);
+    const double t = cin - own - nbv;
+    const double qv = t * cpre;
+    const double res = (cm & CM_FLUID) ? qv : 0.0;
+    const double carry = -1.0 * cpre * res;
+    own = carry; out = carry;
+    if (j & 1) zz[j >> 1].y = res; else zz[j >> 1].x = res;
+  }
+  own = 0.0; out = 0.0;
+#pragma unroll
+  for (int j = W - 1; j >= 0; --j) {
+    const int cm = (int)((mm[j >> 1] >> ((j & 1) * 8)) & 0xff);
+    const double cin = (j & 1) ? zz[j >> 1].y : zz[j >> 1].x, cpre = (j & 1) ? pp[j >> 1].y : pp[j >> 1].x;
+    const double nbv = wave_shift_inject<DPP_WAVE_SHL1>(out, 0.0);
+    const double kr = ((cm & CM_RIGHT) ? -1.0 : 0.0) * cpre, ku = ((cm & CM_UP) ? -1.0 : 0.0) * cpre;
+    const double t = cin - kr * own - ku * nbv;
+    const double zv = t * cpre;
+    const double res = (cm & CM_FLUID) ? zv : 0.0;
+    own = res; out = res;
+    if (DOT && (cm & CM_FLUID)) dsum += res * ((j & 1) ? rr[j >> 1].y : rr[j >> 1].x);
+    if (j & 1) zz[j >> 1].y = res; else zz[j >> 1].x = res;
+  }
+}
+struct ZrArgs { const double* r; const double* pre; const double* table; const double* halo; const double* rows; int X; };
 struct SaPair { sw_d2 z, so; double ez0, es0, ez1, es1; };
 
 __device__ __forceinline__ double pick3(int t, int tb1, int tb2, double v0, double v1, double v2) {
@@ -273,7 +304,7 @@
   return v;
 }
 struct SaHist { const double* s[6]; };
-template <int SLAB, int PMODE, int SA_RUN, int COARSE = 0, bool STORE = true>
+template <int SLAB, int PMODE, int SA_RUN, int COARSE = 0, bool STORE = true, bool ZR = false>
 __global__ __launch_bounds__(SA_THREADS, (COARSE == 2 && PMODE == 1 && SLAB == 0) ? 4 : 1) void k_search_apply(const double* __restrict__ s_old, const double* __restrict__ z,
                                                              double* __restrict__ s_new, double* __restrict__ out,
                                                              const uint8_t* __restrict__ mask, SkewGeom g,
@@ -281,10 +312,16 @@
                                                              unsigned int* counter, int fin_op, SlabNeighbours nbr,
                                                              double* __restrict__ p, double* s_new_base, double* s_old_base,
                                                              const unsigned int* __restrict__ chunk_list,
-                                                             CoarseRef cref, SaHist hist) {
+                                                             CoarseRef cref, SaHist hist, ZrArgs zr) {
+  static_assert(!ZR || (SLAB == 0 && SA_RUN == 8 && COARSE == 0), "ZR: one GPU, runs of one tile, no coarse part");
   __shared__ double s_cy[COARSE == 2 ? SA_THREADS / 64 : 1][COARSE == 2 ? MG_NI + 1 : 1][64];
   __shared__ double s_ce[COARSE == 2 ? SA_THREADS / 64 : 1][COARSE == 2 ? MG_NI + 1 : 1][64];
   if (!force && pcg_idle(sc)) return;
+  __shared__ sw_d2 s_ztab[ZR ? 8 : 1][64];
+  if (ZR) {
+    for (int k = threadIdx.x; k < 8 * 64; k += SA_THREADS) (&s_ztab[0][0])[k] = reinterpret_cast<const sw_d2*>(zr.table)[k];
+    __syncthreads();
+  }
   const double beta = sc->beta;
   (void)s_new_base; (void)s_old_base;
   constexpr int NPA = PMODE >= 2 ? PMODE : 2;
@@ -310,7 +347,7 @@
     int c = i, per = cpb;
     bool interior = false;
     if (listed) { const unsigned int ent = chunk_list[i]; interior = (ent & EU_CHUNK_INTERIOR) != 0; c = (int)(ent & ~EU_CHUNK_INTERIOR); per = ntb16; }
-    const int lb = c / per, P0 = (c % per) * SA_RUN, P1 = P0 + SA_RUN < npairs ? P0 + SA_RUN : npairs;
+    const int lb = c / per, P0 = (c % per) * SA_RUN, P1 = ZR ? P0 + SA_RUN : (P0 + SA_RUN < npairs ? P0 + SA_RUN : npairs);
     const size_t bbase = (size_t)lb * TS * 64 + 2 * lane;
     auto run = [&](auto full_tag) {
       constexpr bool FULL = decltype(full_tag)::value;
@@ -323,6 +360,18 @@
         any |= mm[j];
       }
       if (!FULL && !listed && !__ballot(((any | (any >> 8)) & CM_FLUID) != 0)) return;
+      sw_d2 zz[ZR ? SA_RUN : 1];
+      if (ZR) {
+        sw_d2 rr[SA_RUN], pp[SA_RUN];
+#pragma unroll
+        for (int j = 0; j < SA_RUN; ++j) {
+          rr[j] = *reinterpret_cast<const sw_d2*>(zr.r + bbase + (size_t)(P0 + j) * 128);
+          pp[j] = FULL ? s_ztab[j][lane] : *reinterpret_cast<const sw_d2*>(zr.pre + bbase + (size_t)(P0 + j) * 128);
+        }
+        double none = 0.0;
+        tile_solve<2 * SA_RUN, false>(mm, rr, pp, zz, none);
+      }
+      const int ztile = P0 / SA_RUN;
       const bool up_remote = SLAB == 1 && nbr.z_up && lb + 1 == nb_local, dn_remote = SLAB == 1 && nbr.z_dn && lb == 0;
       const double* ez = lane == 0 ? (dn_remote ? nbr.z_dn : z) : (up_remote ? nbr.z_up : z);
       const double* es = lane == 0 ? (dn_remote ? nbr.s_dn : s_old) : (up_remote ? nbr.s_up : s_old);
@@ -335,6 +384,7 @@
       const double* gs = lane == 0 ? nbr.srow_dn : nbr.srow_up;
       double* gsn = lane == 0 ? nbr.snew_dn : nbr.snew_up;
       const int gcol = lane == 0 ? 0 : -63;
+      const double* zrow = ZR ? zr.rows + (long long)(lane == 0 ? 2 * lb - 1 : 2 * lb + 2) * zr.X : nullptr;
       double cy0 = 0.0, cy1 = 0.0, cy2 = 0.0, ce0 = 0.0, ce1 = 0.0, ce2 = 0.0;
       double (*cyv)[64] = s_cy[COARSE == 2 ? threadIdx.x >> 6 : 0];
       double (*cev)[64] = s_ce[COARSE == 2 ? threadIdx.x >> 6 : 0];
@@ -391,17 +441,26 @@
       auto load_pair = [&](int P, SaPair& d, unsigned int m) __attribute__((always_inline)) {
         d.ez0 = d.es0 = d.ez1 = d.es1 = 0.0;
         if (P < 0 || P >= npairs) { d.z = sw_d2{0.0, 0.0}; d.so = sw_d2{0.0, 0.0}; return; }
-        d.z = *reinterpret_cast<const sw_d2*>(z + bbase + (size_t)P * 128);
+        if (ZR) {
+          const int j = P - P0;
+          if (j >= 0 && j < SA_RUN) d.z = zz[j >= 0 && j < SA_RUN ? j : 0];
+          else if (j < 0) d.z = sw_d2{0.0, zr.halo[((size_t)lb * ntb16 + ztile - 1) * 128 + 64 + lane]};
+          else d.z = sw_d2{ztile + 1 < ntb16 ? zr.halo[((size_t)lb * ntb16 + ztile + 1) * 128 + lane] : 0.0, 0.0};
+        } else {
+          d.z = *reinterpret_cast<const sw_d2*>(z + bbase + (size_t)P * 128);
+        }
         d.so = *reinterpret_cast<const sw_d2*>(s_old + bbase + (size_t)P * 128);
         if (edge_lane) {
           if ((m & CM_FLUID) && (m & vbit)) {
             const long long k = e0_base + (long long)P * 128;
-            if (SLAB == 2 && ghost) { d.ez0 = gz[2 * P + gcol]; d.es0 = gs[2 * P + gcol]; }
+            if (ZR) { d.ez0 = zrow[2 * P + gcol]; d.es0 = s_old[k]; }
+            else if (SLAB == 2 && ghost) { d.ez0 = gz[2 * P + gcol]; d.es0 = gs[2 * P + gcol]; }
             else if (SLAB == 1 && remote) { d.ez0 = ld_system(ez + k); d.es0 = ld_system(es + k); } else { d.ez0 = ez[k]; d.es0 = es[k]; }
           }
           if (((m >> 8) & CM_FLUID) && ((m >> 8) & vbit)) {
             const long long k = e1_base + (long long)P * 128;
-            if (SLAB == 2 && ghost) { d.ez1 = gz[2 * P + 1 + gcol]; d.es1 = gs[2 * P + 1 + gcol]; }
+            if (ZR) { d.ez1 = zrow[2 * P + 1 + gcol]; d.es1 = s_old[k]; }
+            else if (SLAB == 2 && ghost) { d.ez1 = gz[2 * P + 1 + gcol]; d.es1 = gs[2 * P + 1 + gcol]; }
             else if (SLAB == 1 && remote) { d.ez1 = ld_system(ez + k); d.es1 = ld_system(es + k); } else { d.ez1 = ez[k]; d.es1 = es[k]; }
           }
           if (COARSE == 1) {
@@ -1048,6 +1107,8 @@
   int cshift;
   int cmode, cnx, cny;
   const double *gs_lo, *gs_hi;
+  int zform;
+  double *zhalo, *zrows;
 };
 
 __device__ __forceinline__ void tile_block_reduce(double& mx, double& sm) {
@@ -1140,7 +1201,7 @@
 #endif
 template <int W, bool RECOMP = false, int CMODE = 0>
 __global__ __launch_bounds__(PT_THREADS, RECOMP ? PT_RECOMP_BLOCKS : 1) void k_precond_tile(TileArgs a) {
-  if (!a.force && pcg_idle(a.sc)) return;
+  if (!a.force && (a.zform == 2 ? a.sc->zfix == 0 : pcg_idle(a.sc))) return;
   const int lane = threadIdx.x & 63;
   const int ntb = a.g.T / W, total = a.nb_local * ntb;
   const int n_waves = gridDim.x * (PT_THREADS / 64);
@@ -1319,36 +1380,23 @@
 #pragma unroll
         for (int P = 0; P < W / 2; ++P) pp[P] = FULL ? s_tab[P < TABP ? P : 0][lane] : *reinterpret_cast<const sw_d2*>(a.pre + base + P * 128);
       }
-      double own = -0.0, out = -0.0;
-#pragma unroll
-      for (int j = 0; j < W; ++j) {
-        const int cm = (int)((mm[j >> 1] >> ((j & 1) * 8)) & 0xff);
-        const double cin = (j & 1) ? rr[j >> 1].y : rr[j >> 1].x, cpre = (j & 1) ? pp[j >> 1].y : pp[j >> 1].x;
-        const double nbv = wave_shift_inject<DPP_WAVE_SHR1>(out, -0.0);
-        const double t = cin - own - nbv;
-        const double qv = t * cpre;
-        const double res = (cm & CM_FLUID) ? qv : 0.0;
-        const double carry = -1.0 * cpre * res;
-        own = carry; out = carry;
-        if (j & 1) qq[j >> 1].y = res; else qq[j >> 1].x = res;
-      }
-      own = 0.0; out = 0.0;
-#pragma unroll
-      for (int j = W - 1; j >= 0; --j) {
-        const int cm = (int)((mm[j >> 1] >> ((j & 1) * 8)) & 0xff);
-        const double cin = (j & 1) ? qq[j >> 1].y : qq[j >> 1].x, cpre = (j & 1) ? pp[j >> 1].y : pp[j >> 1].x;
-        const double crr = (j & 1) ? rr[j >> 1].y : rr[j >> 1].x;
-        const double nbv = wave_shift_inject<DPP_WAVE_SHL1>(out, 0.0);
-        const double kr = ((cm & CM_RIGHT) ? -1.0 : 0.0) * cpre, ku = ((cm & CM_UP) ? -1.0 : 0.0) * cpre;
-        const double t = cin - kr * own - ku * nbv;
-        const double zv = t * cpre;
-        const double res = (cm & CM_FLUID) ? zv : 0.0;
-        own = res; out = res;
-        if (cm & CM_FLUID) dsum += res * crr;
-        if (j & 1) qq[j >> 1].y = res; else qq[j >> 1].x = res;
-      }
-#pragma unroll
-      for (int P = 0; P < W / 2; ++P) *reinterpret_cast<sw_d2*>(a.z + base + P * 128) = qq[P];
+      tile_solve<W, true>(mm, rr, pp, qq, dsum);
+      if (W == 16 && a.zform == 1) {
+        double* h = a.zhalo + ((size_t)band * ntb + k) * 128;
+        h[lane] = qq[0].x;
+        h[64 + lane] = qq[W / 2 - 1].y;
+        if (lane == 0 || lane == 63) {
+          double* row = a.zrows + ((size_t)band * 2 + (lane == 63 ? 1 : 0)) * a.g.X;
+#pragma unroll
+          for (int j = 0; j < W; ++j) {
+            const int x = k * W + j - lane;
+            if (x >= 0 && x < a.g.X) row[x] = (j & 1) ? qq[j >> 1].y : qq[j >> 1].x;
+          }
+        }
+      } else {
+#pragma unroll
+        for (int P = 0; P < W / 2; ++P) *reinterpret_cast<sw_d2*>(a.z + base + P * 128) = qq[P];
+      }
       if (band == a.edge_lo || band == a.edge_hi) {
         const bool lo = band == a.edge_lo && lane == 0, hi = band == a.edge_hi && lane == 63;
 #pragma unroll
@@ -1390,6 +1438,7 @@
       if (a.rupd) pcg_scalar_step(a.sc, FIN_RNORM, vmax);
       if (a.fin_dot >= 0 && !(a.rupd && a.sc->done)) pcg_scalar_step(a.sc, a.fin_dot, vsum);
     }
+    if (a.zform >= 0) a.sc->zfix = a.zform == 1 ? 1u : 0u;
     __hip_atomic_store(a.counter, 0u, __ATOMIC_RELAXED, __HIP_MEMORY_SCOPE_AGENT);
   }
 }
@@ -1662,6 +1711,23 @@
   if (S->has_comm) return ghost_mode(S);
   return S->cfg.dot_mode != EULER_DOT_SEQUENTIAL;
 }
+static inline bool tile_z_recompute(const euler_sim* S) {
+  return tile_recompute(S) && tile_fused(S) && !eu_is_two_level(S) && S->tile_w == 16 && !S->has_comm && !S->slab_on && S->band_lo == 0 &&
+         S->opt[EULER_OPT_TILE_STORE_Z] == 0 && S->chunk_list && S->tile_table;
+}
+static bool tile_z_begin(euler_sim* S) {
+  S->z_halo_last = 0;
+  if (!tile_z_recompute(S)) return false;
+  if (!S->zhalo) {
+    const size_t nh = (size_t)S->geom.nbands * (S->geom.T / 16) * 128, nr = (size_t)S->geom.nbands * 2 * S->X;
+    if (hipMalloc(&S->zhalo, nh * sizeof(double)) != hipSuccess) { (void)hipGetLastError(); S->zhalo = nullptr; return false; }
+    if (hipMalloc(&S->zrows, nr * sizeof(double)) != hipSuccess) { (void)hipGetLastError(); (void)hipFree(S->zhalo); S->zhalo = S->zrows = nullptr; return false; }
+    S->hbm_bytes += (nh + nr) * sizeof(double);
+    HIPCHK(hipMemsetAsync(S->zhalo, 0, nh * sizeof(double), S->stream));
+    HIPCHK(hipMemsetAsync(S->zrows, 0, nr * sizeof(double), S->stream));
+  }
+  return true;
+}
 __global__ void k_pair_fold(PcgScalars* sc, const double* __restrict__ pairs, int stride, int R, int rupd, int fin_dot, int force) {
   if (!force && pcg_idle(sc)) return;
   double vmax = 0.0, vsum = 0.0;
@@ -1683,6 +1749,7 @@
   a.reverse = S->opt[EULER_OPT_TILE_REVERSE] != 0;
   a.cpart = nullptr; a.cshift = 0; a.cmode = 0; a.cnx = a.cny = 0;
   a.gs_lo = a.gs_hi = nullptr;
+  a.zform = -1; a.zhalo = S->zhalo; a.zrows = S->zrows;
   if (ghost_mode(S)) {
     if (S->band_lo > 0) { a.zsend_lo = xrow(S, XR_ZSEND_LO); a.edge_lo = S->band_lo; }
     if (S->band_hi < S->geom.nbands) { a.zsend_hi = xrow(S, XR_ZSEND_HI); a.edge_hi = S->band_hi - 1; }
@@ -1702,10 +1769,11 @@
   }
   return EULER_OK;
 }
-static int launch_precond_tile(euler_sim* S, int rupd, int sweeps, int fin_dot, int force, double alpha, bool r_only = false) {
+static int launch_precond_tile(euler_sim* S, int rupd, int sweeps, int fin_dot, int force, double alpha, bool r_only = false, int zform = -1) {
   const bool seq = S->cfg.dot_mode == EULER_DOT_SEQUENTIAL && !S->has_comm;
   TileArgs a = make_tile_args(S, force);
   a.rupd = rupd; a.sweeps = sweeps; a.fin_dot = (seq || !sweeps) ? -1 : fin_dot; a.alpha_arg = alpha;
+  a.zform = zform;
   const bool two_level = eu_is_two_level(S) && sweeps && !r_only && !force && a.list != nullptr;
   const int fin_real = a.fin_dot;
   if (two_level) {
@@ -1728,7 +1796,7 @@
       if (a.zsend_hi) a.zsend_hi = eu_mg_split_msg(S, 1);
     }
   }
-  const int w = r_only ? 16 : S->tile_w, cls = r_only ? KC_UPDATE_PR : KC_PRECOND_TILE;
+  const int w = r_only ? 16 : S->tile_w, cls = r_only ? KC_UPDATE_PR : zform == 2 ? KC_MISC : KC_PRECOND_TILE;
   const unsigned nblk = eu_blocks((size_t)(S->band_hi - S->band_lo) * (S->geom.T / w), PT_THREADS / 64, 2048);
   const bool recomp = rupd && !force && tile_recompute(S) && (r_only ? S->tile_as_override == S->q : !S->tile_as_override);
   if (recomp) {
@@ -1900,13 +1968,17 @@
   const bool store = !tile_recompute(S);
   const bool mg = eu_is_mg(S);
   const CoarseRef cref = {mg ? S->mg_x : S->cc_y, mg ? 0 : S->coarse_shift, mg ? S->mg_nx[0] : S->coarse_nx, mg ? S->mg_ny[0] : S->coarse_ny, S->band_lo};
-#define SA_LAUNCH_CS(SLABF, PM, RUNV, CF, ST)                                                                                                \
-  LAUNCH(S, KC_APPLY_A, (k_search_apply<SLABF, PM, RUNV, CF, ST>), dim3(sa_blocks(S, RUNV)), dim3(SA_THREADS), LOC(S->s), LOC(S->z), LOC(S->s2), \
-         LOC(S->q), LOC(S->cellmask), gl, S->partial, S->sc, 0, S->red_counter, fin, nbr, pp, S->s2, S->s, (RUNV) == 8 ? S->chunk_list : (const unsigned int*)nullptr, cref, hist)
+  const ZrArgs zr = {S->r, S->precon, S->tile_table, S->zhalo, S->zrows, S->X};
+#define SA_LAUNCH_CSZ(SLABF, PM, RUNV, CF, ST, ZRF)                                                                                                \
+  LAUNCH(S, KC_APPLY_A, (k_search_apply<SLABF, PM, RUNV, CF, ST, ZRF>), dim3(sa_blocks(S, RUNV)), dim3(SA_THREADS), LOC(S->s), LOC(S->z), LOC(S->s2), \
+         LOC(S->q), LOC(S->cellmask), gl, S->partial, S->sc, 0, S->red_counter, fin, nbr, pp, S->s2, S->s, (RUNV) == 8 ? S->chunk_list : (const unsigned int*)nullptr, cref, hist, zr)
+#define SA_LAUNCH_CS(SLABF, PM, RUNV, CF, ST) SA_LAUNCH_CSZ(SLABF, PM, RUNV, CF, ST, false)
 #define SA_LAUNCH_C(SLABF, PM, RUNV, CF) do { if ((RUNV) == 8 && !store) SA_LAUNCH_CS(SLABF, PM, RUNV, CF, ((RUNV) != 8)); else SA_LAUNCH_CS(SLABF, PM, RUNV, CF, true); } while (0)
 #define SA_LAUNCH(SLABF, PM, RUNV) SA_LAUNCH_C(SLABF, PM, RUNV, 0)
 #define SA_RUNS(SLABF, PM) do { if (run == 8) SA_LAUNCH(SLABF, PM, 8); else if (run == 16) SA_LAUNCH(SLABF, PM, 16); else SA_LAUNCH(SLABF, PM, 32); } while (0)
-  if (eu_is_two_level(S) && tile_fused(S) && ghost) {
+  if (S->z_halo_last) {
+    SA_LAUNCH_CSZ(0, 1, 8, 0, false, true);
+  } else if (eu_is_two_level(S) && tile_fused(S) && ghost) {
     if (pmode == 8) SA_LAUNCH_C(2, 8, 8, 2); else if (pmode == 4) SA_LAUNCH_C(2, 4, 8, 2); else if (pmode == 2) SA_LAUNCH_C(2, 2, 8, 2); else SA_LAUNCH_C(2, 1, 8, 2);
   } else if (eu_is_two_level(S) && tile_fused(S)) {
     if (mg) { if (pmode == 8) SA_LAUNCH_C(0, 8, 8, 2); else if (pmode == 4) SA_LAUNCH_C(0, 4, 8, 2); else if (pmode == 2) SA_LAUNCH_C(0, 2, 8, 2); else SA_LAUNCH_C(0, 1, 8, 2); }
@@ -1924,6 +1996,7 @@
 #undef SA_LAUNCH
 #undef SA_LAUNCH_C
 #undef SA_LAUNCH_CS
+#undef SA_LAUNCH_CSZ
   S->s = S->s_ring[it % steps]; S->s2 = S->s_ring[(it + 1) % steps];
   S->s_launched = it + 1;
   if (seq)
@@ -1937,11 +2010,12 @@
 
 __global__ void k_pcg_reset(PcgScalars* sc, double tol, int max_iters) {
   sc->sigma = sc->zs = sc->sigma_new = sc->alpha = sc->alpha_prev = sc->beta = sc->rnorm = 0.0;
-  sc->tol = tol; sc->nonzero = 0; sc->done = 0; sc->iters = 0; sc->max_iters = max_iters;
+  sc->tol = tol; sc->nonzero = 0; sc->done = 0; sc->iters = 0; sc->max_iters = max_iters; sc->zfix = 0;
 }
 
 int eu_launch_project(euler_sim* S, float dt) {
   S->s_launched = 0;
+  S->z_halo_last = 0;
   S->p_pending = 0;
   S->pcg_fields_resident = 0;
   const PcgScalars prev_solve = *S->sc_host;
@@ -1999,6 +2073,8 @@
   }
   if (two_level && (rc = eu_launch_coarse_setup(S))) return rc;
   if (two_level && (rc = eu_launch_coarse_consistent(S))) return rc;
+  const bool zr = tile && tile_z_begin(S);
+  bool zr_ran = false;
   if (tile) {
     if ((rc = launch_factor_tile(S, 0))) return rc;
     if ((rc = launch_precond_tile(S, 0, 1, FIN_SIGMA_INIT, 0, 0.0))) return rc;
@@ -2044,7 +2120,12 @@
       if ((rc = fused ? launch_search_apply_and_alpha(S, it) : launch_apply_a_and_alpha(S, 0))) return rc;
       if (tile) {
         S->prof_iter = it;
-        if ((rc = launch_precond_tile(S, 1, it + 1 < max_it, FIN_BETA, 0, 0.0))) return rc;
+        const int nx = it + 1, steps = S->s_ring_n;
+        const bool next_odd = !(nx >= steps && nx % steps == 0);
+        const int zform = zr && it + 1 < max_it ? (it + 2 < max_it && next_odd ? 1 : 0) : -1;
+        if ((rc = launch_precond_tile(S, 1, it + 1 < max_it, FIN_BETA, 0, 0.0, false, zform))) return rc;
+        S->z_halo_last = zform == 1;
+        zr_ran = zr_ran || zform == 1;
         continue;
       }
       S->tile_as_override = fused ? S->q : S->z;
@@ -2073,6 +2154,8 @@
     }
   }
   S->prof_iter = -2;
+  S->z_halo_last = 0;
+  if (zr_ran && (rc = launch_precond_tile(S, 0, 1, -1, 0, 0.0, false, 2))) return rc;
   const bool finish_in_update = !S->has_comm && !S->slab_on && S->opt[EULER_OPT_VELOCITY_TWO_PASS] == 0;
   if (!finish_in_update) { if ((rc = eu_launch_finish_p(S))) return rc; }
   if (S->s_ring_n > 2) { S->s = S->s_base[0]; S->s2 = S->s_base[1]; }
diff --git a/include/euler.h b/include/euler.h
--- a/include/euler.h
+++ b/include/euler.h
@@ -213,6 +213,7 @@
   EULER_OPT_VELOCITY_TWO_PASS = 18,
   EULER_OPT_NO_TILE_MAP = 19,
   EULER_OPT_PROFILE_STRIDE = 20,
+  EULER_OPT_TILE_STORE_Z = 21,
   EULER_OPT__COUNT
 };
 int euler_set_option(euler_sim* sim, int32_t key, int64_t value);
```

Result: faster. 195.3 million (median of 6 runs) (+8.4%).
